# kwea123/nerf_pl

Hardware: AMD Instinct MI355X
Metric: rays/sec (64+128 samples), full training step: render_rays fwd + MSE + bwd + grad all-reduce + Adam (higher is better)
Workload: dtype bf16

## Files before the change

include/nerfhip.h:

```cpp
#ifndef NERFHIP_H
#define NERFHIP_H

#include <stddef.h>
#include <stdint.h>

#ifdef __cplusplus
extern "C" {
#endif

#define NERFHIP_ABI_VERSION 3

#define NERFHIP_E_BADARG (-1)
#define NERFHIP_E_UNSUPPORTED (-2)
#define NERFHIP_E_ALIGN (-3)
#define NERFHIP_E_DATA (-4)

#define NERFHIP_F32 0
#define NERFHIP_BF16 1
#define NERFHIP_BF16_F8 2

typedef void* nerfhip_stream_t;

int nerfhip_abi_version(void);
const char* nerfhip_error_string(int code);

int nerfhip_posenc(const float* x, float* out, int64_t n, int C, int n_freqs, nerfhip_stream_t stream);
int nerfhip_posenc_bwd(const float* x, const float* gout, float* gx, int64_t n, int C, int n_freqs,
                       nerfhip_stream_t stream);

int nerfhip_posenc_bands(const float* x, const float* bands, float* out, int64_t n, int C, int n_freqs,
                         nerfhip_stream_t stream);
int nerfhip_posenc_bands_bwd(const float* x, const float* bands, const float* gout, float* gx, int64_t n, int C, int n_freqs,
                             nerfhip_stream_t stream);

int nerfhip_sample_coarse_z(const float* rays, const float* perturb_rand, float* z, int64_t B, int S,
                            int use_disp, float perturb, nerfhip_stream_t stream);

int nerfhip_searchsorted_right(const float* a, const float* v, int64_t* idx, int64_t B, int M, int K,
                               nerfhip_stream_t stream);
int nerfhip_searchsorted_left(const float* a, const float* v, int64_t* idx, int64_t B, int M, int K,
                              nerfhip_stream_t stream);

int nerfhip_sample_pdf(const float* bins, int64_t bins_stride, const float* weights, int64_t w_stride,
                       const float* u, int64_t u_stride, float* samples, int64_t B, int M, int K, float eps,
                       nerfhip_stream_t stream);

#define NERFHIP_ROW_TOTAL_EXACT 0
#define NERFHIP_ROW_TOTAL_ATEN 1

int nerfhip_sample_pdf_ex(const float* bins, int64_t bins_stride, const float* weights, int64_t w_stride,
                          const float* u, int64_t u_stride, float* samples, int64_t B, int M, int K, float eps,
                          float* cdf_out, int64_t* inds_out, int row_total, nerfhip_stream_t stream);

int nerfhip_fine_z(const float* z_coarse, const float* w_coarse, const float* u, int64_t u_stride,
                   float* z_fine, float* z_new, int64_t B, int S_c, int N_i, float eps,
                   nerfhip_stream_t stream);

int nerfhip_fine_z_ex(const float* z_coarse, const float* w_coarse, const float* u, int64_t u_stride, float* z_fine,
                      float* z_new, int64_t B, int S_c, int N_i, float eps, float* cdf_out, int64_t* inds_out,
                      int row_total, nerfhip_stream_t stream);

int nerfhip_composite_fwd(const float* raw, int raw_ch, const float* z, const float* rays,
                          const float* noise, float noise_std, int white_back, float* weights, float* rgb,
                          float* depth, float* opacity, int64_t B, int S, nerfhip_stream_t stream);
int nerfhip_composite_bwd(const float* raw, int raw_ch, const float* z, const float* rays,
                          const float* noise, float noise_std, int white_back, const float* g_rgb,
                          const float* g_depth, const float* g_opacity, const float* g_weights,
                          float* g_raw, int64_t B, int S, nerfhip_stream_t stream);

int nerfhip_composite_train(const float* raw, const float* z, const float* rays, const float* noise, float noise_std,
                            int white_back, const float* target, float grad_scale, float* weights, float* rgb, float* depth,
                            float* opacity, float* g_raw, int64_t B, int S, nerfhip_stream_t stream);

int nerfhip_composite_train_fine_z(const float* raw, const float* z, const float* rays, const float* noise, float noise_std,
                                   int white_back, const float* target, float grad_scale, float* weights, float* rgb, float* depth,
                                   float* opacity, float* g_raw, int64_t B, int S, const float* u, int64_t u_stride, int N_i,
                                   float eps, float* z_fine, int row_total, nerfhip_stream_t stream);
int nerfhip_composite_train_loss(const float* raw, const float* z, const float* rays, const float* noise, float noise_std,
                                 int white_back, const float* target, float grad_scale, float* weights, float* rgb, float* depth,
                                 float* opacity, float* g_raw, int64_t B, int S, const float* rgb_coarse, float* out3,
                                 uint32_t* ticket, nerfhip_stream_t stream);

size_t nerfhip_mlp_packed_bytes(int dtype);
int nerfhip_mlp_pack_weights(const float* const* weights_host, const float* const* biases_host, void* packed,
                             int dtype, nerfhip_stream_t stream);

size_t nerfhip_mlp_act_bytes(int64_t n_points, int dtype);

int nerfhip_mlp_fwd_embedded(const float* x, int64_t x_stride, int64_t n, const void* packed, float* out,
                             int sigma_only, int dtype, void* save_acts, nerfhip_stream_t stream);

int nerfhip_mlp_fwd_rays(const float* rays, const float* z, int64_t B, int S, const void* packed, float* out,
                         int sigma_only, int dtype, void* save_acts, nerfhip_stream_t stream);

int nerfhip_mlp_fwd_rays_coarse(const float* rays, const float* perturb_rand, float* z, int64_t B, int S, int use_disp,
                                float perturb, const void* packed, float* out, int sigma_only, int dtype, void* save_acts,
                                nerfhip_stream_t stream);

size_t nerfhip_mlp_packed_bwd_bytes(int dtype);
int nerfhip_mlp_pack_weights_bwd(const float* const* weights_host, const float* const* biases_host, void* packed_bwd, int dtype,
                                 nerfhip_stream_t stream);
int nerfhip_mlp_pack_weights_train(const float* const* weights_host, const float* const* biases_host, void* packed,
                                   void* packed_bwd, int dtype, nerfhip_stream_t stream);
int nerfhip_mlp_pack_weights_train_multi(const float* const* weights_host, const float* const* biases_host,
                                         void* const* packed_host, void* const* packed_bwd_host, int n_models, int dtype,
                                         nerfhip_stream_t stream);
size_t nerfhip_mlp_dy_bytes(int64_t n_points, int dtype);
int nerfhip_mlp_dw_splits(int64_t n_points, int dtype);
size_t nerfhip_mlp_dw_workspace_bytes(int64_t n_points, int dtype);
int nerfhip_mlp_bwd(const float* g_out, const float* out, int64_t n, const void* packed_bwd, const void* acts,
                    void* dys, void* dw_workspace, float* const* grad_w_host, float* const* grad_b_host,
                    int accumulate, int dtype, nerfhip_stream_t stream);

int nerfhip_mlp_bwd_phases(const float* g_out, const float* out, int64_t n, const void* packed_bwd, const void* acts,
                           void* dys, void* dw_workspace, float* const* grad_w_host, float* const* grad_b_host,
                           int accumulate, int dtype, int phases, nerfhip_stream_t stream);

typedef struct nerfhip_adam_fused {
    int n_models;
    float* param[2];
    float* exp_avg[2];
    float* exp_avg_sq[2];
    const float* grad_flat[2];
    float* state;
    float lr, beta1, beta2, eps, weight_decay;
} nerfhip_adam_fused;
size_t nerfhip_mlp_dw_workspace_bytes_multi(const int64_t* n_points_host, int n_models, int dtype);
int nerfhip_mlp_dw_plan(const int64_t* n_points_host, int n_models, int dtype, int* splits_out, int* stage_kib_out);
int nerfhip_mlp_bwd_multi(int n_models, const float* const* g_out_host, const float* const* out_host, const int64_t* n_host,
                          const void* const* packed_bwd_host, const void* const* acts_host, void* const* dys_host,
                          void* dw_workspace, float* const* grad_w_host, float* const* grad_b_host, int accumulate, int dtype,
                          int phases, const float* g_scale, const nerfhip_adam_fused* adam, nerfhip_stream_t stream);

typedef struct nerfhip_enc_source {
    const float* rays[2];
    const float* z[2];
    int S[2];
} nerfhip_enc_source;
int nerfhip_mlp_bwd_multi_rays(int n_models, const float* const* g_out_host, const float* const* out_host, const int64_t* n_host,
                               const void* const* packed_bwd_host, const void* const* acts_host, void* const* dys_host,
                               void* dw_workspace, float* const* grad_w_host, float* const* grad_b_host, int accumulate, int dtype,
                               int phases, const float* g_scale, const nerfhip_adam_fused* adam, const nerfhip_enc_source* enc,
                               nerfhip_stream_t stream);

int nerfhip_mlp_dx_embedded(const void* dys, int64_t n, const float* w_xyz1, const float* w_xyz5, const float* w_dir,
                            float* gx, int64_t gx_stride, int dtype, nerfhip_stream_t stream);

#define NERFHIP_ACT_NONE 0
#define NERFHIP_ACT_RELU 1
#define NERFHIP_ACT_SIGMOID 2
int nerfhip_linear_fwd(const float* x, int64_t ldx, const float* w, int64_t ldw, const float* bias, float* y, int64_t ldy,
                       int64_t n, int n_in, int n_out, int act, int accumulate, int dtype, nerfhip_stream_t stream);
int nerfhip_linear_bwd_input(const float* gy, int64_t ldgy, const float* y, int64_t ldy, int act, const float* w, int64_t ldw,
                             float* gx, int64_t ldgx, int64_t n, int n_in, int n_out, int accumulate, int dtype,
                             nerfhip_stream_t stream);
size_t nerfhip_linear_bwd_weight_workspace_bytes(int64_t n, int n_in, int n_out);
int nerfhip_linear_bwd_weight(const float* gy, int64_t ldgy, const float* y, int64_t ldy, int act, const float* x, int64_t ldx,
                              float* gw, int64_t ldgw, float* gb, void* workspace, int64_t n, int n_in, int n_out,
                              int accumulate, int dtype, nerfhip_stream_t stream);

int nerfhip_mse_psnr(const float* rgb_coarse, const float* rgb_fine, const float* target, int64_t n, float* out3,
                     float* g_coarse, float* g_fine, nerfhip_stream_t stream);

int nerfhip_adam_step(float* const* params_host, const float* const* grads_host, float* const* exp_avg_host,
                      float* const* exp_avg_sq_host, const int64_t* numel_host, int n_tensors, float* state, float lr,
                      float beta1, float beta2, float eps, float weight_decay, nerfhip_stream_t stream);

int nerfhip_radam_step(float* const* params_host, const float* const* grads_host, float* const* exp_avg_host,
                       float* const* exp_avg_sq_host, const int64_t* numel_host, int n_tensors, float* state, double lr,
                       double beta1, double beta2, double eps, double weight_decay, int degenerated_to_sgd,
                       nerfhip_stream_t stream);
int nerfhip_ranger_step(float* const* params_host, const float* const* grads_host, float* const* exp_avg_host,
                        float* const* exp_avg_sq_host, const int64_t* numel_host, int n_tensors, float* state,
                        float* const* slow_host, double alpha, int k, double n_sma_threshold, double lr, double beta1,
                        double beta2, double eps, double weight_decay, nerfhip_stream_t stream);

int nerfhip_ray_directions(float* dirs, int H, int W, double focal, nerfhip_stream_t stream);
int nerfhip_get_rays(const float* directions, const float* c2w, float* rays_o, float* rays_d, int64_t n,
                     nerfhip_stream_t stream);
int nerfhip_ndc_rays(int H, int W, double focal, float near, const float* rays_o, const float* rays_d, float* out_o,
                     float* out_d, int64_t n, nerfhip_stream_t stream);
int nerfhip_gen_rays(const float* c2w, const int64_t* pixel_ids, int64_t first_pixel, int64_t n, int H, int W,
                     double focal, float near, float far, int use_ndc, float ndc_near_plane, float* rays,
                     nerfhip_stream_t stream);
int nerfhip_sample_batch(const float* c2w, const int64_t* pixel_ids, const float* rgbs_all, int64_t n, int H, int W,
                         double focal, float near, float far, int use_ndc, float ndc_near_plane, float* rays, float* rgbs,
                         nerfhip_stream_t stream);

#define NERFHIP_DRAW_UNIFORM 0
#define NERFHIP_DRAW_NORMAL 1
#define NERFHIP_DRAW_RANDINT 2
typedef struct nerfhip_draw {
    int kind;
    int64_t numel;
    void* out;
    uint64_t range;
} nerfhip_draw;
typedef struct nerfhip_ray_batch {
    const float* c2w;
    const float* rgbs_all;
    float* rays;
    float* rgbs;
    int H, W;
    double focal;
    float near, far;
    int use_ndc;
    float ndc_near_plane;
} nerfhip_ray_batch;
uint64_t nerfhip_torch_draw_increment(int64_t numel, int max_blocks);
int nerfhip_torch_draws(const nerfhip_draw* draws_host, int n_draws, const nerfhip_ray_batch* batch_host, uint64_t seed,
                        uint64_t offset, uint64_t* state, int max_blocks, uint64_t* increment_host, nerfhip_stream_t stream);

int nerfhip_train_prologue(const nerfhip_draw* draws_host, int n_draws, const nerfhip_ray_batch* batch_host, uint64_t seed,
                           uint64_t offset, uint64_t* state, int max_blocks, uint64_t* increment_host,
                           const float* const* weights_host, const float* const* biases_host, void* const* packed_host,
                           void* const* packed_bwd_host, int n_models, int dtype, nerfhip_stream_t stream);

typedef struct nerfhip_render_args {
    const float* rays;
    int64_t B;
    int S_c, N_i;
    const void* packed_coarse;
    const void* packed_fine;
    float* z_coarse;
    float* raw_coarse;
    float* z_fine;
    float* raw_fine;
    void* save_coarse;
    void* save_fine;
    const float* perturb_rand;
    float perturb;
    int use_disp;
    const float* noise_coarse;
    const float* noise_fine;
    float noise_std;
    int white_back;
    const float* u;
    int64_t u_stride;
    float eps;
    int row_total;
    float* rgb_coarse;
    float* depth_coarse;
    float* opacity_coarse;
    float* rgb_fine;
    float* depth_fine;
    float* opacity_fine;
    const float* target;
    float grad_scale;
    float* g_raw_coarse;
    float* g_raw_fine;
    float* out3;
    uint32_t* ticket;
    int regen_enc;
} nerfhip_render_args;
int nerfhip_render_supported(int64_t B, int S_c, int N_i, int dtype);
int nerfhip_render_fwd(const nerfhip_render_args* args_host, int dtype, nerfhip_stream_t stream);
int nerfhip_render_test_fwd(const nerfhip_render_args* args_host, int dtype, nerfhip_stream_t stream);
int nerfhip_render_train_fwd(const nerfhip_render_args* args_host, int dtype, nerfhip_stream_t stream);

size_t nerfhip_marching_cubes_workspace_bytes(int64_t n0, int64_t n1, int64_t n2);
int nerfhip_marching_cubes_count(const float* volume, int64_t n0, int64_t n1, int64_t n2, double iso, void* workspace,
                                 int64_t* totals, nerfhip_stream_t stream);
int nerfhip_marching_cubes_emit(const float* volume, int64_t n0, int64_t n1, int64_t n2, double iso, void* workspace,
                                const int64_t* totals, double* vertices, int32_t* triangles, nerfhip_stream_t stream);

int nerfhip_mesh_edge_keys(const int32_t* triangles, int64_t T, int64_t* keys, nerfhip_stream_t stream);
size_t nerfhip_mesh_cluster_workspace_bytes(int64_t V, int64_t T);
int nerfhip_mesh_largest_cluster(const int32_t* triangles, int64_t V, int64_t T, const int64_t* sorted_keys, const int64_t* order,
                                 void* workspace, int64_t* totals, nerfhip_stream_t stream);
int nerfhip_mesh_cluster_compact(const int32_t* triangles, int64_t V, int64_t T, void* workspace, int64_t* kept_vertex_ids,
                                 int32_t* kept_triangles, nerfhip_stream_t stream);

int nerfhip_mesh_vertex_normals(const float* vertices, int64_t V, const int32_t* triangles, int64_t T, double* normals,
                                nerfhip_stream_t stream);
int nerfhip_mesh_normal_rays(const float* vertices, const double* normals, int64_t V, float near, float far, float near_t,
                             float* rays, nerfhip_stream_t stream);
int nerfhip_mesh_view_rays(const float* vertices, int64_t V, const float* w2c_host, const float* origin_host, float focal, int W,
                           int H, const uint8_t* image, float near, uint8_t* colors, double* depth, float* rays,
                           nerfhip_stream_t stream);
int nerfhip_mesh_color_accumulate(const uint8_t* colors, const double* depth, const float* opacity, int64_t V,
                                  float occ_threshold, double* accum, nerfhip_stream_t stream);
int nerfhip_mesh_color_finish(const double* accum, int64_t V, uint8_t* out, nerfhip_stream_t stream);
int nerfhip_mesh_rgb_to_u8(const float* rgb, int64_t n, uint8_t* out, nerfhip_stream_t stream);

size_t nerfhip_vol_workspace_bytes(int64_t n);
int nerfhip_vol_pack(const float* rgbsigma, int64_t n, int64_t first_index, float neg_cell, void* workspace, uint32_t* records,
                     int64_t capacity, int64_t* cursor, nerfhip_stream_t stream);

int nerfhip_png_unfilter(const uint8_t* streams, uint8_t* out, int32_t* error_flags, int n_images, int H, int W, int ch,
                         nerfhip_stream_t stream);
int nerfhip_resize_rgba_lanczos(const uint8_t* in, uint8_t* out, uint8_t* workspace, int n_images, int in_h, int in_w, int out_h,
                                int out_w, const int32_t* xmin_h, const int32_t* count_h, const int32_t* taps_h, int ksize_h,
                                const int32_t* xmin_v, const int32_t* count_v, const int32_t* taps_v, int ksize_v,
                                nerfhip_stream_t stream);
int nerfhip_rgba_to_rgb_white(const uint8_t* rgba, float* rgb, uint8_t* valid_mask, int64_t n, nerfhip_stream_t stream);

int nerfhip_jpeg_entropy_decode(const uint8_t* scan, int64_t scan_bytes, int n_comp, const int32_t* comp, const uint8_t* huffman,
                                int huffman_mask, int mcus_x, int mcus_y, int restart_interval, int16_t* const* coef,
                                const int64_t* coef_blocks);
size_t nerfhip_jpeg_planes_bytes(int H, int W, int n_comp, int hs, int vs);
int nerfhip_jpeg_decode(const int16_t* coef_y, const int16_t* coef_cb, const int16_t* coef_cr, const uint16_t* quant,
                        uint8_t* planes, uint8_t* out, int n_images, int H, int W, int n_comp, int hs, int vs,
                        nerfhip_stream_t stream);

#define NERFHIP_IMAGE_PLANAR 0
#define NERFHIP_IMAGE_INTERLEAVED 1
size_t nerfhip_ssim_workspace_bytes(int B, int C, int H, int W);
int nerfhip_ssim(const float* img1, const float* img2, int B, int C, int H, int W, int window_size, int layout, float* map,
                 float* mean, void* workspace, nerfhip_stream_t stream);
size_t nerfhip_depth_colormap_workspace_bytes(int64_t n);
int nerfhip_depth_colormap(const float* depth, int64_t n, const uint8_t* table, float* out_chw, uint8_t* out_hwc, void* workspace,
                           nerfhip_stream_t stream);

#define NERFHIP_GIF_STRIP 3838
size_t nerfhip_gif_workspace_bytes(int F, int H, int W);
size_t nerfhip_gif_data_stride(int H, int W);
int nerfhip_gif_quantize(const uint8_t* frames, int F, int H, int W, uint8_t* indices, uint8_t* palettes, int32_t* box_counts,
                         void* workspace, nerfhip_stream_t stream);
int nerfhip_gif_lzw(const uint8_t* indices, int F, int H, int W, uint8_t* data, int32_t* lengths, void* workspace,
                    nerfhip_stream_t stream);

#ifdef __cplusplus
}
#endif
#endif
```

nerf_pl_amd/_lib.py:

```python
import ctypes
import functools
import os

import torch

_PKG = os.path.dirname(os.path.abspath(__file__))
LIB_PATH = os.environ.get("NERFHIP_LIB_PATH") or os.path.join(_PKG, "libnerfhip.so")

F32, BF16, BF16_F8 = 0, 1, 2

_c_void_p = ctypes.c_void_p
_i64 = ctypes.c_int64
_int = ctypes.c_int
_f32 = ctypes.c_float
_f64 = ctypes.c_double

SIGNATURES = {
    "nerfhip_abi_version": [],
    "nerfhip_error_string": [_int],
    "nerfhip_posenc": [_c_void_p, _c_void_p, _i64, _int, _int, _c_void_p],
    "nerfhip_posenc_bwd": [_c_void_p, _c_void_p, _c_void_p, _i64, _int, _int, _c_void_p],
    "nerfhip_posenc_bands": [_c_void_p, _c_void_p, _c_void_p, _i64, _int, _int, _c_void_p],
    "nerfhip_posenc_bands_bwd": [_c_void_p, _c_void_p, _c_void_p, _c_void_p, _i64, _int, _int, _c_void_p],
    "nerfhip_sample_coarse_z": [_c_void_p, _c_void_p, _c_void_p, _i64, _int, _int, _f32, _c_void_p],
    "nerfhip_searchsorted_right": [_c_void_p, _c_void_p, _c_void_p, _i64, _int, _int, _c_void_p],
    "nerfhip_searchsorted_left": [_c_void_p, _c_void_p, _c_void_p, _i64, _int, _int, _c_void_p],
    "nerfhip_sample_pdf": [_c_void_p, _i64, _c_void_p, _i64, _c_void_p, _i64, _c_void_p, _i64, _int, _int, _f32,
                           _c_void_p],
    "nerfhip_sample_pdf_ex": [_c_void_p, _i64, _c_void_p, _i64, _c_void_p, _i64, _c_void_p, _i64, _int, _int, _f32,
                              _c_void_p, _c_void_p, _int, _c_void_p],
    "nerfhip_fine_z_ex": [_c_void_p, _c_void_p, _c_void_p, _i64, _c_void_p, _c_void_p, _i64, _int, _int, _f32,
                          _c_void_p, _c_void_p, _int, _c_void_p],
    "nerfhip_fine_z": [_c_void_p, _c_void_p, _c_void_p, _i64, _c_void_p, _c_void_p, _i64, _int, _int, _f32,
                       _c_void_p],
    "nerfhip_composite_fwd": [_c_void_p, _int, _c_void_p, _c_void_p, _c_void_p, _f32, _int, _c_void_p, _c_void_p,
                              _c_void_p, _c_void_p, _i64, _int, _c_void_p],
    "nerfhip_composite_bwd": [_c_void_p, _int, _c_void_p, _c_void_p, _c_void_p, _f32, _int, _c_void_p, _c_void_p,
                              _c_void_p, _c_void_p, _c_void_p, _i64, _int, _c_void_p],
    "nerfhip_mlp_packed_bytes": [_int],
    "nerfhip_mlp_pack_weights": [ctypes.POINTER(_c_void_p), ctypes.POINTER(_c_void_p), _c_void_p, _int, _c_void_p],
    "nerfhip_mlp_act_bytes": [_i64, _int],
    "nerfhip_mlp_fwd_embedded": [_c_void_p, _i64, _i64, _c_void_p, _c_void_p, _int, _int, _c_void_p, _c_void_p],
    "nerfhip_mlp_fwd_rays": [_c_void_p, _c_void_p, _i64, _int, _c_void_p, _c_void_p, _int, _int, _c_void_p, _c_void_p],
    "nerfhip_mlp_packed_bwd_bytes": [_int],
    "nerfhip_mlp_pack_weights_bwd": [ctypes.POINTER(_c_void_p), ctypes.POINTER(_c_void_p), _c_void_p, _int, _c_void_p],
    "nerfhip_mlp_pack_weights_train": [ctypes.POINTER(_c_void_p), ctypes.POINTER(_c_void_p), _c_void_p, _c_void_p, _int, _c_void_p],
    "nerfhip_mlp_dy_bytes": [_i64, _int],
    "nerfhip_mlp_dw_splits": [_i64, _int],
    "nerfhip_mlp_dw_workspace_bytes": [_i64, _int],
    "nerfhip_ray_directions": [_c_void_p, _int, _int, ctypes.c_double, _c_void_p],
    "nerfhip_get_rays": [_c_void_p, _c_void_p, _c_void_p, _c_void_p, _i64, _c_void_p],
    "nerfhip_ndc_rays": [_int, _int, ctypes.c_double, _f32, _c_void_p, _c_void_p, _c_void_p, _c_void_p, _i64, _c_void_p],
    "nerfhip_gen_rays": [_c_void_p, _c_void_p, _i64, _i64, _int, _int, ctypes.c_double, _f32, _f32, _int, _f32, _c_void_p,
                         _c_void_p],
    "nerfhip_mse_psnr": [_c_void_p, _c_void_p, _c_void_p, _i64, _c_void_p, _c_void_p, _c_void_p, _c_void_p],
    "nerfhip_mlp_bwd_phases": [_c_void_p, _c_void_p, _i64, _c_void_p, _c_void_p, _c_void_p, _c_void_p,
                               ctypes.POINTER(_c_void_p), ctypes.POINTER(_c_void_p), _int, _int, _int, _c_void_p],
    "nerfhip_mlp_dx_embedded": [_c_void_p, _i64, _c_void_p, _c_void_p, _c_void_p, _c_void_p, _i64, _int, _c_void_p],
    "nerfhip_adam_step": [ctypes.POINTER(_c_void_p), ctypes.POINTER(_c_void_p), ctypes.POINTER(_c_void_p),
                          ctypes.POINTER(_c_void_p), ctypes.POINTER(_i64), _int, _c_void_p, _f32, _f32, _f32, _f32, _f32, _c_void_p],
    "nerfhip_radam_step": [ctypes.POINTER(_c_void_p), ctypes.POINTER(_c_void_p), ctypes.POINTER(_c_void_p),
                           ctypes.POINTER(_c_void_p), ctypes.POINTER(_i64), _int, _c_void_p, _f64, _f64, _f64, _f64, _f64, _int, _c_void_p],
    "nerfhip_ranger_step": [ctypes.POINTER(_c_void_p), ctypes.POINTER(_c_void_p), ctypes.POINTER(_c_void_p),
                            ctypes.POINTER(_c_void_p), ctypes.POINTER(_i64), _int, _c_void_p, ctypes.POINTER(_c_void_p), _f64, _int,
                            _f64, _f64, _f64, _f64, _f64, _f64, _c_void_p],
    "nerfhip_mlp_bwd": [_c_void_p, _c_void_p, _i64, _c_void_p, _c_void_p, _c_void_p, _c_void_p,
                        ctypes.POINTER(_c_void_p), ctypes.POINTER(_c_void_p), _int, _int, _c_void_p],
    "nerfhip_sample_batch": [_c_void_p, _c_void_p, _c_void_p, _i64, _int, _int, ctypes.c_double, _f32, _f32, _int, _f32, _c_void_p,
                             _c_void_p, _c_void_p],
    "nerfhip_mlp_pack_weights_train_multi": [ctypes.POINTER(_c_void_p), ctypes.POINTER(_c_void_p), ctypes.POINTER(_c_void_p),
                                             ctypes.POINTER(_c_void_p), _int, _int, _c_void_p],
    "nerfhip_render_supported": [_i64, _int, _int, _int],
    "nerfhip_render_test_fwd": [_c_void_p, _int, _c_void_p],
    "nerfhip_render_fwd": [_c_void_p, _int, _c_void_p],
    "nerfhip_render_train_fwd": [_c_void_p, _int, _c_void_p],
    "nerfhip_composite_train": [_c_void_p, _c_void_p, _c_void_p, _c_void_p, _f32, _int, _c_void_p, _f32, _c_void_p, _c_void_p,
                                _c_void_p, _c_void_p, _c_void_p, _i64, _int, _c_void_p],
    "nerfhip_composite_train_fine_z": [_c_void_p, _c_void_p, _c_void_p, _c_void_p, _f32, _int, _c_void_p, _f32, _c_void_p, _c_void_p,
                                       _c_void_p, _c_void_p, _c_void_p, _i64, _int, _c_void_p, _i64, _int, _f32, _c_void_p, _int, _c_void_p],
    "nerfhip_composite_train_loss": [_c_void_p, _c_void_p, _c_void_p, _c_void_p, _f32, _int, _c_void_p, _f32, _c_void_p, _c_void_p,
                                     _c_void_p, _c_void_p, _c_void_p, _i64, _int, _c_void_p, _c_void_p, _c_void_p, _c_void_p],
    "nerfhip_mlp_fwd_rays_coarse": [_c_void_p, _c_void_p, _c_void_p, _i64, _int, _int, _f32, _c_void_p, _c_void_p, _int, _int,
                                    _c_void_p, _c_void_p],
    "nerfhip_torch_draw_increment": [_i64, _int],
    "nerfhip_torch_draws": [_c_void_p, _int, _c_void_p, ctypes.c_uint64, ctypes.c_uint64, _c_void_p, _int,
                            ctypes.POINTER(ctypes.c_uint64), _c_void_p],
    "nerfhip_train_prologue": [_c_void_p, _int, _c_void_p, ctypes.c_uint64, ctypes.c_uint64, _c_void_p, _int,
                               ctypes.POINTER(ctypes.c_uint64), ctypes.POINTER(_c_void_p), ctypes.POINTER(_c_void_p),
                               ctypes.POINTER(_c_void_p), ctypes.POINTER(_c_void_p), _int, _int, _c_void_p],
    "nerfhip_mlp_dw_workspace_bytes_multi": [ctypes.POINTER(_i64), _int, _int],
    "nerfhip_mlp_dw_plan": [ctypes.POINTER(_i64), _int, _int, ctypes.POINTER(_int), ctypes.POINTER(_int)],
    "nerfhip_mlp_bwd_multi": [_int, ctypes.POINTER(_c_void_p), ctypes.POINTER(_c_void_p), ctypes.POINTER(_i64),
                              ctypes.POINTER(_c_void_p), ctypes.POINTER(_c_void_p), ctypes.POINTER(_c_void_p), _c_void_p,
                              ctypes.POINTER(_c_void_p), ctypes.POINTER(_c_void_p), _int, _int, _int, _c_void_p, _c_void_p, _c_void_p],
    "nerfhip_mlp_bwd_multi_rays": [_int, ctypes.POINTER(_c_void_p), ctypes.POINTER(_c_void_p), ctypes.POINTER(_i64),
                                   ctypes.POINTER(_c_void_p), ctypes.POINTER(_c_void_p), ctypes.POINTER(_c_void_p), _c_void_p,
                                   ctypes.POINTER(_c_void_p), ctypes.POINTER(_c_void_p), _int, _int, _int, _c_void_p, _c_void_p, _c_void_p,
                                   _c_void_p],
    "nerfhip_linear_fwd": [_c_void_p, _i64, _c_void_p, _i64, _c_void_p, _c_void_p, _i64, _i64, _int, _int, _int, _int, _int, _c_void_p],
    "nerfhip_linear_bwd_input": [_c_void_p, _i64, _c_void_p, _i64, _int, _c_void_p, _i64, _c_void_p, _i64, _i64, _int, _int, _int,
                                 _int, _c_void_p],
    "nerfhip_linear_bwd_weight_workspace_bytes": [_i64, _int, _int],
    "nerfhip_linear_bwd_weight": [_c_void_p, _i64, _c_void_p, _i64, _int, _c_void_p, _i64, _c_void_p, _i64, _c_void_p, _c_void_p,
                                  _i64, _int, _int, _int, _int, _c_void_p],
    "nerfhip_marching_cubes_workspace_bytes": [_i64, _i64, _i64],
    "nerfhip_marching_cubes_count": [_c_void_p, _i64, _i64, _i64, ctypes.c_double, _c_void_p, _c_void_p, _c_void_p],
    "nerfhip_marching_cubes_emit": [_c_void_p, _i64, _i64, _i64, ctypes.c_double, _c_void_p, _c_void_p, _c_void_p, _c_void_p,
                                    _c_void_p],
    "nerfhip_mesh_edge_keys": [_c_void_p, _i64, _c_void_p, _c_void_p],
    "nerfhip_mesh_cluster_workspace_bytes": [_i64, _i64],
    "nerfhip_mesh_largest_cluster": [_c_void_p, _i64, _i64, _c_void_p, _c_void_p, _c_void_p, _c_void_p, _c_void_p],
    "nerfhip_mesh_cluster_compact": [_c_void_p, _i64, _i64, _c_void_p, _c_void_p, _c_void_p, _c_void_p],
    "nerfhip_mesh_vertex_normals": [_c_void_p, _i64, _c_void_p, _i64, _c_void_p, _c_void_p],
    "nerfhip_mesh_normal_rays": [_c_void_p, _c_void_p, _i64, _f32, _f32, _f32, _c_void_p, _c_void_p],
    "nerfhip_mesh_view_rays": [_c_void_p, _i64, ctypes.POINTER(_f32), ctypes.POINTER(_f32), _f32, _int, _int, _c_void_p, _f32,
                               _c_void_p, _c_void_p, _c_void_p, _c_void_p],
    "nerfhip_mesh_color_accumulate": [_c_void_p, _c_void_p, _c_void_p, _i64, _f32, _c_void_p, _c_void_p],
    "nerfhip_mesh_color_finish": [_c_void_p, _i64, _c_void_p, _c_void_p],
    "nerfhip_mesh_rgb_to_u8": [_c_void_p, _i64, _c_void_p, _c_void_p],
    "nerfhip_vol_workspace_bytes": [_i64],
    "nerfhip_vol_pack": [_c_void_p, _i64, _i64, _f32, _c_void_p, _c_void_p, _i64, _c_void_p, _c_void_p],
    "nerfhip_png_unfilter": [_c_void_p, _c_void_p, _c_void_p, _int, _int, _int, _int, _c_void_p],
    "nerfhip_resize_rgba_lanczos": [_c_void_p, _c_void_p, _c_void_p, _int, _int, _int, _int, _int, _c_void_p, _c_void_p, _c_void_p,
                                    _int, _c_void_p, _c_void_p, _c_void_p, _int, _c_void_p],
    "nerfhip_rgba_to_rgb_white": [_c_void_p, _c_void_p, _c_void_p, _i64, _c_void_p],
    "nerfhip_jpeg_entropy_decode": [_c_void_p, _i64, _int, _c_void_p, _c_void_p, _int, _int, _int, _int, ctypes.POINTER(_c_void_p),
                                    ctypes.POINTER(_i64)],
    "nerfhip_jpeg_planes_bytes": [_int, _int, _int, _int, _int],
    "nerfhip_jpeg_decode": [_c_void_p, _c_void_p, _c_void_p, _c_void_p, _c_void_p, _c_void_p, _int, _int, _int, _int, _int, _int,
                            _c_void_p],
    "nerfhip_ssim_workspace_bytes": [_int, _int, _int, _int],
    "nerfhip_ssim": [_c_void_p, _c_void_p, _int, _int, _int, _int, _int, _int, _c_void_p, _c_void_p, _c_void_p, _c_void_p],
    "nerfhip_depth_colormap_workspace_bytes": [_i64],
    "nerfhip_depth_colormap": [_c_void_p, _i64, _c_void_p, _c_void_p, _c_void_p, _c_void_p, _c_void_p],
    "nerfhip_gif_workspace_bytes": [_int, _int, _int],
    "nerfhip_gif_data_stride": [_int, _int],
    "nerfhip_gif_quantize": [_c_void_p, _int, _int, _int, _c_void_p, _c_void_p, _c_void_p, _c_void_p, _c_void_p],
    "nerfhip_gif_lzw": [_c_void_p, _int, _int, _int, _c_void_p, _c_void_p, _c_void_p, _c_void_p],
}


class AdamFused(ctypes.Structure):
    _fields_ = [("n_models", _int), ("param", _c_void_p * 2), ("exp_avg", _c_void_p * 2), ("exp_avg_sq", _c_void_p * 2),
                ("grad_flat", _c_void_p * 2), ("state", _c_void_p), ("lr", _f32), ("beta1", _f32), ("beta2", _f32), ("eps", _f32),
                ("weight_decay", _f32)]

class Draw(ctypes.Structure):
    _fields_ = [("kind", _int), ("numel", _i64), ("out", _c_void_p), ("range", ctypes.c_uint64)]


class RayBatch(ctypes.Structure):
    _fields_ = [("c2w", _c_void_p), ("rgbs_all", _c_void_p), ("rays", _c_void_p), ("rgbs", _c_void_p), ("H", _int), ("W", _int),
                ("focal", ctypes.c_double), ("near", _f32), ("far", _f32), ("use_ndc", _int), ("ndc_near_plane", _f32)]


class RenderArgs(ctypes.Structure):
    _fields_ = [("rays", _c_void_p), ("B", _i64), ("S_c", _int), ("N_i", _int), ("packed_coarse", _c_void_p), ("packed_fine", _c_void_p),
                ("z_coarse", _c_void_p), ("raw_coarse", _c_void_p), ("z_fine", _c_void_p), ("raw_fine", _c_void_p),
                ("save_coarse", _c_void_p), ("save_fine", _c_void_p), ("perturb_rand", _c_void_p), ("perturb", _f32), ("use_disp", _int),
                ("noise_coarse", _c_void_p), ("noise_fine", _c_void_p), ("noise_std", _f32), ("white_back", _int), ("u", _c_void_p),
                ("u_stride", _i64), ("eps", _f32), ("row_total", _int), ("rgb_coarse", _c_void_p), ("depth_coarse", _c_void_p),
                ("opacity_coarse", _c_void_p), ("rgb_fine", _c_void_p), ("depth_fine", _c_void_p), ("opacity_fine", _c_void_p),
                ("target", _c_void_p), ("grad_scale", _f32), ("g_raw_coarse", _c_void_p), ("g_raw_fine", _c_void_p), ("out3", _c_void_p),
                ("ticket", _c_void_p), ("regen_enc", _int)]


class EncSource(ctypes.Structure):
    _fields_ = [("rays", _c_void_p * 2), ("z", _c_void_p * 2), ("S", _int * 2)]


DRAW_UNIFORM, DRAW_NORMAL, DRAW_RANDINT = 0, 1, 2

_RESTYPES = {"nerfhip_error_string": ctypes.c_char_p, "nerfhip_torch_draw_increment": ctypes.c_uint64, "nerfhip_mlp_packed_bytes": ctypes.c_size_t,
             "nerfhip_mlp_act_bytes": ctypes.c_size_t, "nerfhip_mlp_packed_bwd_bytes": ctypes.c_size_t,
             "nerfhip_mlp_dy_bytes": ctypes.c_size_t, "nerfhip_mlp_dw_workspace_bytes": ctypes.c_size_t,
             "nerfhip_mlp_dw_workspace_bytes_multi": ctypes.c_size_t,
             "nerfhip_linear_bwd_weight_workspace_bytes": ctypes.c_size_t,
             "nerfhip_marching_cubes_workspace_bytes": ctypes.c_size_t, "nerfhip_mesh_cluster_workspace_bytes": ctypes.c_size_t,
             "nerfhip_jpeg_planes_bytes": ctypes.c_size_t, "nerfhip_ssim_workspace_bytes": ctypes.c_size_t,
             "nerfhip_depth_colormap_workspace_bytes": ctypes.c_size_t, "nerfhip_gif_workspace_bytes": ctypes.c_size_t,
             "nerfhip_gif_data_stride": ctypes.c_size_t, "nerfhip_vol_workspace_bytes": ctypes.c_size_t}

_lib = None


class NerfHipError(RuntimeError):
    pass


def load():
    global _lib
    if _lib is not None:
        return _lib
    if not os.path.exists(LIB_PATH):
        raise NerfHipError(
            "libnerfhip.so not built: run `python -m nerf_pl_amd.build` (needs hipcc, gfx950). "
            "There is no CPU/eager fallback for the hot path.")
    lib = ctypes.CDLL(LIB_PATH, mode=ctypes.RTLD_GLOBAL)
    for name, argtypes in SIGNATURES.items():
        fn = getattr(lib, name)
        fn.argtypes = argtypes
        fn.restype = _RESTYPES.get(name, ctypes.c_int)
    if lib.nerfhip_abi_version() != 3:
        raise NerfHipError("libnerfhip ABI version mismatch")
    _lib = lib
    return lib


def check(code, what):
    if code != 0:
        msg = load().nerfhip_error_string(code)
        raise NerfHipError("%s failed: %s (code %d)" % (what, msg.decode() if msg else "?", code))


def stream_ptr():
    return ctypes.c_void_p(torch.cuda.current_stream().cuda_stream)


def _first_cuda_tensor(args):
    for a in args:
        if torch.is_tensor(a) and a.is_cuda:
            return a
        if isinstance(a, (list, tuple)):
            t = _first_cuda_tensor(a)
            if t is not None:
                return t
    return None


def device_guard(fn):
    @functools.wraps(fn)
    def wrapped(*args, **kw):
        t = _first_cuda_tensor(args)
        if t is None:
            t = _first_cuda_tensor(tuple(kw.values()))
        if t is None or t.device.index == torch.cuda.current_device():
            return fn(*args, **kw)
        with torch.cuda.device(t.device):
            return fn(*args, **kw)
    return wrapped


def ptr(t):
    if t is None:
        return None
    return ctypes.c_void_p(t.data_ptr())


def require_gpu(*tensors):
    dev = None
    for t in tensors:
        if t is None:
            continue
        if not t.is_cuda:
            raise NerfHipError("nerf_pl_amd runs on MI355X only: got a %s tensor (no CPU fallback)" % t.device)
        if t.dtype != torch.float32:
            raise NerfHipError("expected float32 tensor, got %s" % t.dtype)
        if dev is None:
            dev = t.device
        elif t.device != dev:
            raise NerfHipError("tensors of one call live on different GPUs (%s vs %s)" % (dev, t.device))
    if dev is not None and dev.index != torch.cuda.current_device():
        raise NerfHipError("launch on %s while the current device is cuda:%d (operator missing its device_guard)"
                           % (dev, torch.cuda.current_device()))
```

nerf_pl_amd/csrc/mlp_bwd.hip:

```cpp
#include "common.h"
#include "mlp_layout.h"
#include "mlp_bwd_chain.h"
#include "mlp_bwd_dw.h"
#include "mlp_dw_plan.h"

static_assert(kPlanF32 == NERFHIP_F32 && kPlanBf16 == NERFHIP_BF16 && kPlanBf16F8 == NERFHIP_BF16_F8, "mlp_dw_plan.h dtype codes");
static inline bool valid_dtype(int dtype) { return dtype == NERFHIP_F32 || dtype == NERFHIP_BF16 || dtype == NERFHIP_BF16_F8; }
static inline int compute_prec(int dtype) { return dtype == NERFHIP_F32 ? NERFHIP_F32 : NERFHIP_BF16; }
#if NERFHIP_DW_PROBE
static bool g_probe_f8 = false;
#endif

extern "C" size_t nerfhip_mlp_dy_bytes(int64_t n_points, int dtype) {
    if (n_points < 0 || !valid_dtype(dtype)) return 0;
    if (dtype == NERFHIP_BF16_F8) return (size_t)act_tiles(n_points, dtype) * nerfhip::mlp::f8_dy_tile_bytes();
    return (size_t)act_tiles(n_points, dtype) * nerfhip::mlp::kDySlabs * 64 * (dtype == NERFHIP_BF16 ? 16 : 32);
}

extern "C" int nerfhip_mlp_dw_splits(int64_t n_points, int dtype) {
    if (n_points <= 0 || !valid_dtype(dtype)) return 0;
    return dw_plan(&n_points, 1, dtype, nullptr);
}
static size_t dw_workspace_bytes(int nwg, int n_models) {
    return ((size_t)nwg * nerfhip::mlp::kDwSlabFloats + (size_t)n_models * nerfhip::mlp::kFoldScratchFloats) * sizeof(float);
}
extern "C" size_t nerfhip_mlp_dw_workspace_bytes(int64_t n_points, int dtype) {
    const int nwg = nerfhip_mlp_dw_splits(n_points, dtype);
    return nwg > 0 ? dw_workspace_bytes(nwg, 1) : 0;
}
extern "C" size_t nerfhip_mlp_dw_workspace_bytes_multi(const int64_t* n_points_host, int n_models, int dtype) {
    if (!n_points_host || n_models < 1 || n_models > nerfhip::kDwMaxModels || !valid_dtype(dtype)) return 0;
    for (int m = 0; m < n_models; ++m)
        if (n_points_host[m] <= 0) return 0;
    return dw_workspace_bytes(dw_plan(n_points_host, n_models, dtype, nullptr), n_models);
}

extern "C" int nerfhip_mlp_dw_plan(const int64_t* n_points_host, int n_models, int dtype, int* splits_out, int* stage_kib_out) {
    if (!n_points_host || !splits_out || n_models < 1 || n_models > nerfhip::kDwMaxModels || !valid_dtype(dtype)) return NERFHIP_E_BADARG;
    for (int m = 0; m < n_models; ++m)
        if (n_points_host[m] <= 0) return NERFHIP_E_BADARG;
    nerfhip::DwJobTable jt;
    const int total = dw_plan(n_points_host, n_models, dtype, &jt);
    for (int j = 0; j < n_models * nerfhip::mlp::kNumDwJobs; ++j) {
        splits_out[j] = jt.nsplit[j];
        if (stage_kib_out) {
            int slabs = jt.job[j].dy_slabs + jt.job[j].x1_slabs + jt.job[j].x2_slabs;
            if (jt.fold_of[j] >= 0 || jt.nsplit[j] == 0) slabs = 0;
            for (int k = 0; k < n_models * nerfhip::mlp::kNumDwJobs; ++k)
                if (jt.fold_of[k] == j) slabs += jt.job[k].dy_slabs;
            stage_kib_out[j] = dtype == NERFHIP_F32 ? 2 * slabs : slabs;
        }
    }
    return total;
}

extern "C" int nerfhip_mlp_bwd_multi(int n_models, const float* const* g_out_host, const float* const* out_host,
                                     const int64_t* n_host, const void* const* packed_bwd_host, const void* const* acts_host,
                                     void* const* dys_host, void* dw_workspace, float* const* grad_w_host,
                                     float* const* grad_b_host, int accumulate, int dtype, int phases, const float* g_scale,
                                     const nerfhip_adam_fused* adam, nerfhip_stream_t stream) {
    return nerfhip_mlp_bwd_multi_rays(n_models, g_out_host, out_host, n_host, packed_bwd_host, acts_host, dys_host, dw_workspace, grad_w_host,
                                      grad_b_host, accumulate, dtype, phases, g_scale, adam, nullptr, stream);
}

extern "C" int nerfhip_mlp_bwd_multi_rays(int n_models, const float* const* g_out_host, const float* const* out_host,
                                          const int64_t* n_host, const void* const* packed_bwd_host, const void* const* acts_host,
                                          void* const* dys_host, void* dw_workspace, float* const* grad_w_host,
                                          float* const* grad_b_host, int accumulate, int dtype, int phases, const float* g_scale,
                                          const nerfhip_adam_fused* adam, const nerfhip_enc_source* enc, nerfhip_stream_t stream) {
    NERFHIP_CHECK_ARG(n_models >= 1 && n_models <= nerfhip::kDwMaxModels);
    if (!valid_dtype(dtype)) return NERFHIP_E_UNSUPPORTED;
    bool regen[nerfhip::kDwMaxModels] = {false, false};
    if (enc) {
        if (dtype != NERFHIP_BF16) return NERFHIP_E_UNSUPPORTED;
        for (int m = 0; m < n_models; ++m) {
            if (!enc->rays[m]) continue;
            NERFHIP_CHECK_ARG(enc->z[m] && enc->S[m] > 0 && enc->S[m] % 32 == 0 && n_host[m] % 256 == 0 && n_host[m] % enc->S[m] == 0);
            NERFHIP_CHECK_ARG(n_host[m] / 32 < (int64_t)1 << 31);
            if ((((uintptr_t)enc->rays[m]) | ((uintptr_t)enc->z[m])) & 15) return NERFHIP_E_ALIGN;
            regen[m] = true;
        }
    }
    NERFHIP_CHECK_ARG(g_out_host && out_host && n_host && packed_bwd_host && acts_host && dys_host && grad_w_host && grad_b_host);
    NERFHIP_CHECK_ARG(!(adam && accumulate));
    nerfhip::GradTable G;
    nerfhip::DwJobTable jt;
    for (int m = 0; m < n_models; ++m) {
        NERFHIP_CHECK_ARG(n_host[m] > 0);
        NERFHIP_CHECK_ARG(g_out_host[m] && out_host[m] && packed_bwd_host[m] && acts_host[m] && dys_host[m] && dw_workspace);
        if ((((uintptr_t)g_out_host[m]) | ((uintptr_t)out_host[m]) | ((uintptr_t)packed_bwd_host[m]) | ((uintptr_t)acts_host[m]) |
             ((uintptr_t)dys_host[m])) & 15)
            return NERFHIP_E_ALIGN;
    }
    const int nwg = dw_plan(n_host, n_models, dtype, &jt);
    for (int m = 0; m < nerfhip::kDwMaxModels; ++m) {
        const bool on = m < n_models && regen[m];
        jt.enc_rays[m] = on ? enc->rays[m] : nullptr;
        jt.enc_z[m] = on ? enc->z[m] : nullptr;
        jt.enc_tpr[m] = on ? enc->S[m] / 32 : 1;
    }
    float* const fold_scratch = (float*)dw_workspace + (size_t)nwg * nerfhip::mlp::kDwSlabFloats;
    nerfhip::FoldArgs F;
    for (int m = 0; m < nerfhip::kDwMaxModels; ++m) {
        const int mm = m < n_models ? m : 0;
        F.image[m] = reinterpret_cast<const float*>((const uint8_t*)packed_bwd_host[mm] +
                                                    (size_t)nerfhip::mlp::bwd_padded_pieces(compute_prec(dtype)) * nerfhip::mlp::kPieceBytes);
        F.gw_final[m] = grad_w_host[12 * mm + 8];
        F.gb_final[m] = grad_b_host[12 * mm + 8];
        F.gw_dir[m] = grad_w_host[12 * mm + 9];
    }
    for (int j = 0; j < nerfhip::kDwMaxJobs; ++j) {
        const int jj = j < jt.njobs ? j : 0, m = jj / nerfhip::mlp::kNumDwJobs, prm = nerfhip::mlp::kDwJobs[jj % nerfhip::mlp::kNumDwJobs].param;
        NERFHIP_CHECK_ARG(grad_w_host[12 * m + prm] && grad_b_host[12 * m + prm]);
        G.w[j] = grad_w_host[12 * m + prm];
        G.b[j] = grad_b_host[12 * m + prm];
        jt.acts[j] = (const uint8_t*)acts_host[m];
        jt.dys[j] = (const uint8_t*)dys_host[m];
    }
    nerfhip::AdamFused A;
    A.state = nullptr;
    A.lr = A.beta1 = A.beta2 = A.eps = A.wd = 0.f;
    for (int m = 0; m < nerfhip::kDwMaxModels; ++m) { A.param[m] = A.m[m] = A.v[m] = nullptr; A.grad0[m] = nullptr; }
    if (adam) {
        NERFHIP_CHECK_ARG(adam->state && adam->n_models == n_models);
        for (int m = 0; m < n_models; ++m) {
            NERFHIP_CHECK_ARG(adam->param[m] && adam->exp_avg[m] && adam->exp_avg_sq[m] && adam->grad_flat[m]);
            A.param[m] = adam->param[m]; A.m[m] = adam->exp_avg[m]; A.v[m] = adam->exp_avg_sq[m]; A.grad0[m] = adam->grad_flat[m];
        }
        A.state = adam->state; A.lr = adam->lr; A.beta1 = adam->beta1; A.beta2 = adam->beta2; A.eps = adam->eps; A.wd = adam->weight_decay;
    }
    hipStream_t s = (hipStream_t)stream;
    const bool do_chain = phases & 1, do_dw = phases & 2, do_reduce = phases & 4;
    if (do_chain) {
        int64_t tiles[nerfhip::kDwMaxModels];
        for (int m = 0; m < n_models; ++m) tiles[m] = act_tiles(n_host[m], dtype);
        nerfhip::launch_bwd_chain(n_models, g_out_host, g_scale, out_host, n_host, packed_bwd_host, acts_host, dys_host, dtype, tiles, s);
    }
    if (do_dw) {
        if (dtype == NERFHIP_BF16_F8) nerfhip::launch_dw_f8(jt, (float*)dw_workspace, nwg, s);
        else nerfhip::launch_dw(dtype, jt, (float*)dw_workspace, nwg, s);
#if NERFHIP_DW_PROBE
        g_probe_f8 = dtype == NERFHIP_BF16_F8;
#endif
    }
    if (do_reduce) {
        nerfhip::launch_reduce(dtype == NERFHIP_BF16_F8, jt, (const float*)dw_workspace, G, fold_scratch, accumulate, A, s);
        nerfhip::launch_fold(F, (const float*)fold_scratch, n_models, accumulate, A, s);
    }
    return nerfhip_launch_status();
}

#if NERFHIP_DW_PROBE
extern "C" int nerfhip_debug_dw_probe(unsigned* host_dst, int n_words) {
    if (!host_dst || n_words < 0 || n_words > 1024 * 8 * 8) return NERFHIP_E_BADARG;
    return g_probe_f8 ? nerfhip::read_dw_f8_probe(host_dst, n_words) : nerfhip::read_dw_probe(host_dst, n_words);
}
#endif

extern "C" int nerfhip_mlp_bwd_phases(const float* g_out, const float* out, int64_t n, const void* packed_bwd, const void* acts,
                                      void* dys, void* dw_workspace, float* const* grad_w_host, float* const* grad_b_host,
                                      int accumulate, int dtype, int phases, nerfhip_stream_t stream) {
    NERFHIP_CHECK_ARG(n >= 0);
    if (!valid_dtype(dtype)) return NERFHIP_E_UNSUPPORTED;
    NERFHIP_CHECK_ARG(grad_w_host && grad_b_host);
    for (int i = 0; i < 12; ++i) NERFHIP_CHECK_ARG(grad_w_host[i] && grad_b_host[i]);
    if (n == 0) return 0;
    return nerfhip_mlp_bwd_multi(1, &g_out, &out, &n, &packed_bwd, &acts, &dys, dw_workspace, grad_w_host, grad_b_host, accumulate,
                                 dtype, phases, nullptr, nullptr, stream);
}

extern "C" int nerfhip_mlp_bwd(const float* g_out, const float* out, int64_t n, const void* packed_bwd, const void* acts,
                               void* dys, void* dw_workspace, float* const* grad_w_host, float* const* grad_b_host,
                               int accumulate, int dtype, nerfhip_stream_t stream) {
    return nerfhip_mlp_bwd_phases(g_out, out, n, packed_bwd, acts, dys, dw_workspace, grad_w_host, grad_b_host, accumulate, dtype, 7,
                                  stream);
}
```

nerf_pl_amd/csrc/mlp_bwd_chain.h:

```cpp
#pragma once
#include <hip/hip_runtime.h>
#include <stdint.h>

namespace nerfhip {
struct BwdChainArgs {
    const float* g_out[2];
    const float* out[2];
    int64_t n[2];
    const uint8_t* packed_bwd[2];
    const uint8_t* acts[2];
    uint8_t* dys[2];
    int blocks0;
};
void launch_bwd_chain(int n_models, const float* const* g_out, const float* g_scale, const float* const* out, const int64_t* n,
                      const void* const* packed_bwd, const void* const* acts, void* const* dys, int dtype, const int64_t* tiles,
                      hipStream_t s);
}
```

nerf_pl_amd/csrc/mlp_bwd_chain.hip:

```cpp
#include "mlp_device.h"
#include "f8_store.h"
#include "mlp_bwd_chain.h"

namespace nerfhip {

__device__ __forceinline__ float slab_absmax8(const bf16x8& s) {
    float m = 0.0f;
#pragma unroll
    for (int j = 0; j < 8; ++j) m = fmaxf(m, fabsf((float)s[j]));
    return m;
}
__device__ __forceinline__ float slab_absmax8(const f32x8& s) { return 0.0f; }

constexpr int kChainDepthBf16 = 2, kChainDepthF8 = 0;
constexpr int kChainBurst = 2;
template <int PREC> using BwdStream = RingStream<PrecTraits<PREC>::NW, bwd_chunks(PREC), true>;

template <typename Slab>
__device__ __forceinline__ Slab load_slab(__amdgpu_buffer_rsrc_t rsrc, int sec, int lane) {
    Slab s;
    u32x4* dst = reinterpret_cast<u32x4*>(&s);
    const unsigned voff = (unsigned)lane * (unsigned)sizeof(Slab);
    const unsigned soff = (unsigned)(sec * 64 * sizeof(Slab));
#pragma unroll
    for (int q = 0; q < (int)(sizeof(Slab) / 16); ++q) dst[q] = __builtin_amdgcn_raw_buffer_load_b128(rsrc, voff + 16 * q, soff, 0);
    return s;
}
template <int PREC, typename Slab>
__device__ __forceinline__ void store_slab(int& pending, __amdgpu_buffer_rsrc_t rsrc, int sec, const Slab& s, int lane) {
    const unsigned voff = (unsigned)lane * (unsigned)sizeof(Slab);
    const unsigned soff = (unsigned)(sec * 64 * sizeof(Slab) * act_il(PREC));
    store_slab_b128(pending, rsrc, s, voff + soff);
}

__device__ __forceinline__ void save_dy_pair(int& pending, uint8_t* dy_tile, int pair, const bf16x8& s0, const bf16x8& s1, int sb, int lane) {
    save_pair_bf8(pending, dy_tile, pair, s0, s1, sb, lane);
}
__device__ __forceinline__ void save_dy_pair(int&, uint8_t*, int, const f32x8&, const f32x8&, int, int) {}
__device__ __forceinline__ int dy_block_scale(float lane_max) { return bf8_block_scale(lane_max); }

template <int BIT>
__device__ __forceinline__ unsigned gate_mask(unsigned word) {
    unsigned m;
    asm("v_bfe_i32 %0, %1, %2, 1" : "=v"(m) : "v"(word), "n"(BIT));
    return m;
}

template <int PREC, int L, int NT, int NKS, bool MASK, bool F8, int IN_PAIRS, typename Slab>
__device__ __forceinline__ int run_bwd_layer_tm(BwdStream<PREC>& st, const unsigned lds_lo, const unsigned lds_hi, const unsigned sig_lds,
                                                const Slab (&gin)[NKS - kBwdLayers[L].sigma_slab], Slab* out,
                                                __amdgpu_buffer_rsrc_t acts, int gate_off, int mask_piece,
                                                __amdgpu_buffer_rsrc_t dys, uint8_t* dy_tile, int dy_sec, int dy_scale_idx, int in_sec,
                                                int in_sb, int lane) {
    constexpr int G0 = bwd_layer_start(L, PREC);
    constexpr int PPF = ppf(PREC);
    static_assert(kBwdLayers[L].nt == NT && kBwdLayers[L].nks == NKS, "bwd layer shape mismatch");
    auto piece_off = [](int g) { return ((g / kChunkPieces) % kSlots) * kChunkBytes + (g % kChunkPieces) * kPieceBytes; };
    typedef __attribute__((address_space(3))) const char* lds_cptr;
    auto piece_ptr = [&](int g) { return piece_off(g) < 65536 ? (lds_cptr)(lds_lo + (unsigned)piece_off(g)) : (lds_cptr)(lds_hi + (unsigned)(piece_off(g) - 65536)); };
    constexpr bool SIG = kBwdLayers[L].sigma_slab != 0;
    constexpr int NIN = NKS - (SIG ? 1 : 0);
    auto bslab = [&](int ks) -> Slab {
        if constexpr (SIG) {
            if (ks == NIN) return *reinterpret_cast<__attribute__((address_space(3))) const Slab*>(sig_lds);
        }
        return gin[ks < NIN ? ks : 0];
    };
    u32x4 gates = {0u, 0u, 0u, 0u};
    if (MASK)
        gates = __builtin_amdgcn_raw_buffer_load_b128(acts, (unsigned)lane * 16u, (unsigned)((gate_off + mask_piece * kPieceBytes) * act_il(PREC, F8)), 0);
    float mx = 0.0f;
    f32x16 acc2[2];
    constexpr int NFR = NT * NKS;
    constexpr int kChainDepth = F8 ? kChainDepthF8 : kChainDepthBf16;
    [[maybe_unused]] bf16x8 afr[kChainDepth > 0 ? kChainDepth : 1];
    [[maybe_unused]] auto frag_read = [&](auto ic) -> bf16x8 {
        constexpr int g = G0 + decltype(ic)::value * PPF;
        if constexpr (g % kChunkPieces == 0) st.boundary(g / kChunkPieces);
        return *reinterpret_cast<__attribute__((address_space(3))) const bf16x8*>(piece_ptr(g));
    };
    if constexpr (PREC == NERFHIP_BF16 && kChainDepth > 0) {
        static_for<0, (kChainDepth < NFR ? kChainDepth : NFR)>([&](auto jc) { afr[decltype(jc)::value] = frag_read(jc); });
    }
    static_for<0, NT>([&](auto tc) {
        constexpr int t = decltype(tc)::value;
        f32x16& acc = acc2[t & 1];
#pragma unroll
        for (int r = 0; r < 16; ++r) acc[r] = 0.0f;
        if constexpr (PREC == NERFHIP_BF16 && kChainDepth > 0) {
            static_for<0, NKS>([&](auto kc) {
                constexpr int ks = decltype(kc)::value;
                constexpr int i = t * NKS + ks;
                acc = __builtin_amdgcn_mfma_f32_32x32x16_bf16(afr[i % (kChainDepth > 0 ? kChainDepth : 1)], bslab(ks), acc, 0, 0, 0);
                if constexpr (i + kChainDepth < NFR) afr[i % (kChainDepth > 0 ? kChainDepth : 1)] = frag_read(std::integral_constant<int, i + kChainDepth>{});
                __builtin_amdgcn_sched_barrier(0);
            });
        } else {
#pragma unroll
        for (int ks = 0; ks < NKS; ++ks) {
            const int g = G0 + (t * NKS + ks) * PPF;
            if (g % kChunkPieces == 0) st.boundary(g / kChunkPieces);
            if constexpr (PREC == NERFHIP_BF16) {
                const bf16x8 a = *reinterpret_cast<__attribute__((address_space(3))) const bf16x8*>(piece_ptr(g));
                acc = __builtin_amdgcn_mfma_f32_32x32x16_bf16(a, bslab(ks), acc, 0, 0, 0);
            } else {
                const f32x4 a0 = *reinterpret_cast<__attribute__((address_space(3))) const f32x4*>(piece_ptr(g));
                if ((g + 1) % kChunkPieces == 0) st.boundary((g + 1) / kChunkPieces);
                const f32x4 a1 = *reinterpret_cast<__attribute__((address_space(3))) const f32x4*>(piece_ptr(g + 1));
                const Slab bs = bslab(ks);
#pragma unroll
                for (int j = 0; j < 4; ++j) acc = __builtin_amdgcn_mfma_f32_32x32x2f32(a0[j], bs[j], acc, 0, 0, 0);
#pragma unroll
                for (int j = 0; j < 4; ++j) acc = __builtin_amdgcn_mfma_f32_32x32x2f32(a1[j], bs[4 + j], acc, 0, 0, 0);
            }
        }
        }
        if constexpr (F8 && PREC == NERFHIP_BF16) {
            if constexpr (IN_PAIRS > 0) {
#pragma unroll
                for (int q = 0; q < IN_PAIRS; ++q)
                    if (q >= t * IN_PAIRS / NT && q < (t + 1) * IN_PAIRS / NT)
                        save_dy_pair(st.pending, dy_tile, in_sec / 2 + q, gin[2 * q], gin[2 * q + 1], in_sb, lane);
            }
        }
        if constexpr (PREC == NERFHIP_BF16 && MASK) {
            static_for<0, 8>([&](auto pc) {
                constexpr int p = decltype(pc)::value;
                constexpr int idx = 8 * (2 * t) + 2 * p;
                typedef __attribute__((ext_vector_type(2))) float f32x2v;
                typedef __attribute__((ext_vector_type(2))) __bf16 bf16x2q;
                typedef __attribute__((ext_vector_type(2))) short s16x2q;
                const f32x2v xv = {acc[2 * p], acc[2 * p + 1]};
                if (F8) mx = fmaxf(fmaxf(mx, fabsf(xv[0])), fabsf(xv[1]));
                const bf16x2q pk = __builtin_convertvector(xv, bf16x2q);
                const unsigned gword = gates[gate_word(idx)];
                s16x2q gm = __builtin_bit_cast(s16x2q, gword);
                gm = (gm << (short)((idx & 31) >> 1)) >> (short)15;
                const unsigned d = __builtin_bit_cast(unsigned, pk) & __builtin_bit_cast(unsigned, gm);
                const bf16x2q gated = __builtin_bit_cast(bf16x2q, d);
                out[2 * t + (p >> 2)][2 * (p & 3)] = gated[0];
                out[2 * t + (p >> 2)][2 * (p & 3) + 1] = gated[1];
            });
        } else {
        float v[16];
        static_for<0, 16>([&](auto rc) {
            constexpr int r = decltype(rc)::value;
            constexpr int idx = 8 * (2 * t) + r;
            const float gv = acc[r];
            if constexpr (MASK) v[r] = __uint_as_float(__float_as_uint(gv) & gate_mask<gate_bit(idx)>(gates[gate_word(idx)]));
            else v[r] = gv;
            if (F8) mx = fmaxf(mx, fabsf(v[r]));
        });
#pragma unroll
        for (int sl = 0; sl < 2; ++sl) {
            float v8[8];
#pragma unroll
            for (int j = 0; j < 8; ++j) v8[j] = v[8 * sl + j];
            make_slab(out[2 * t + sl], v8);
        }
        }
        if constexpr (!F8) {
            __amdgpu_buffer_rsrc_t dys_l = __builtin_amdgcn_make_buffer_rsrc(dy_tile + (size_t)dy_sec * 64 * sizeof(Slab) * act_il(PREC), 0,
                                                                              (int)(2 * NT * 64 * sizeof(Slab) * act_il(PREC)), 0x00020000);
            constexpr int TB = kChainBurst / 2 > 0 ? kChainBurst / 2 : 1;
            if constexpr ((t + 1) % TB == 0 || t == NT - 1) {
                constexpr int t0 = (t / TB) * TB;
#pragma unroll
                for (int sl = 2 * t0; sl < 2 * t + 2; ++sl) store_slab<PREC>(st.pending, dys_l, sl, out[sl], lane);
            }
        }
    });
    if constexpr (F8 && PREC == NERFHIP_BF16) {
        const int sb = dy_block_scale(mx);
        save_scale_f8(st.pending, dy_tile, f8_dy_scale_off(), dy_scale_idx, sb, lane);
        return sb;
    }
    return 127;
}

template <int PREC, bool F8>
__global__ __launch_bounds__(PrecTraits<PREC>::NW * 64, PrecTraits<PREC>::WPS)
void mlp_bwd_chain_kernel(BwdChainArgs A, const float* __restrict__ g_scale) {
    const int mdl = ((int)blockIdx.x >= A.blocks0) ? 1 : 0;
    const unsigned wg = blockIdx.x - (mdl ? (unsigned)A.blocks0 : 0u);
    const float* __restrict__ g_out = mdl ? A.g_out[1] : A.g_out[0];
    const float* __restrict__ out = mdl ? A.out[1] : A.out[0];
    const int64_t n = mdl ? A.n[1] : A.n[0];
    const uint8_t* __restrict__ packed_bwd = mdl ? A.packed_bwd[1] : A.packed_bwd[0];
    const uint8_t* __restrict__ acts_base = mdl ? A.acts[1] : A.acts[0];
    uint8_t* __restrict__ dys_base = mdl ? A.dys[1] : A.dys[0];
    static_assert(!F8 || PREC == NERFHIP_BF16, "fp8 storage is a bf16-compute mode");
    using Slab = typename PrecTraits<PREC>::Slab;
    constexpr int kActTile = F8 ? f8_act_tile_bytes() : act_tile_bytes(PREC);
    constexpr int kGateOff = F8 ? f8_act_gate_off() : act_mask_off(PREC);
    constexpr int kDyTile = F8 ? f8_dy_tile_bytes() : kDySlabs * 64 * (int)sizeof(Slab);
    constexpr int NW = PrecTraits<PREC>::NW;
    __shared__ __attribute__((aligned(1024))) char ring[kSlots * kChunkBytes + NW * 64 * (int)sizeof(Slab)];
#if NERFHIP_STREAM_PROBE
    const uint64_t probe_t0 = __builtin_amdgcn_s_memrealtime();
#endif
    const int lane = threadIdx.x & 63;
    const int wave = __builtin_amdgcn_readfirstlane((int)(threadIdx.x >> 6));
    const int h = lane >> 5;
    const int64_t tile = (int64_t)wg * NW + wave;
    const int64_t p = tile * 32 + (lane & 31);
    const bool valid = p < n;
    const int64_t pc = valid ? p : n - 1;

    float4 g = reinterpret_cast<const float4*>(g_out)[pc];
    const float4 o = reinterpret_cast<const float4*>(out)[pc];
    if (!valid) g = make_float4(0.f, 0.f, 0.f, 0.f);
    if (g_scale) {
        const float sc = *g_scale;
        g.x *= sc; g.y *= sc; g.z *= sc; g.w *= sc;
    }

    constexpr int IL = act_il(PREC, F8);
    __amdgpu_buffer_rsrc_t acts = __builtin_amdgcn_make_buffer_rsrc(
        const_cast<uint8_t*>(acts_base) + tile_block_off(tile, kActTile, IL), 0, kActTile * IL, 0x00020000);
    uint8_t* dy_tile = dys_base + tile_block_off(tile, kDyTile, IL);
    __amdgpu_buffer_rsrc_t dys = __builtin_amdgcn_make_buffer_rsrc(dy_tile, 0, kDyTile * IL, 0x00020000);


    BwdStream<PREC> st;
    st.gsrc = packed_bwd;
    st.voff = (unsigned)lane * 16u;
    st.lds_base = (unsigned)(uintptr_t)ring;
    st.wave = wave;
    st.pending = 0;
    st.pending_prev = 0;
    st.issue_chunk(0);
    st.issue_chunk(1);
    const unsigned lds_lo = (unsigned)(uintptr_t)ring + (unsigned)lane * 16u;
    unsigned lds_hi = lds_lo + 65536u;
    asm volatile("" : "+v"(lds_hi));
    const unsigned sig_lds = (unsigned)(uintptr_t)ring + (unsigned)(kSlots * kChunkBytes) + (unsigned)((wave * 64 + lane) * (int)sizeof(Slab));

    float v[8];
    Slab zero_slab;
#pragma unroll
    for (int j = 0; j < 8; ++j) v[j] = 0.0f;
    make_slab(zero_slab, v);
    Slab g_rgb, g_sig;
    {
        const float ga[3] = {g.x * o.x * (1.0f - o.x), g.y * o.y * (1.0f - o.y), g.z * o.z * (1.0f - o.z)};
#pragma unroll
        for (int j = 0; j < 8; ++j) v[j] = (h == 0 && j < 3) ? ga[j < 3 ? j : 0] : 0.0f;
        make_slab(g_rgb, v);
#pragma unroll
        for (int j = 0; j < 8; ++j) v[j] = (h == 0 && j == 0) ? g.w : 0.0f;
        make_slab(g_sig, v);
    }
    if constexpr (F8) {
        if constexpr (PREC == NERFHIP_BF16) {
            const int sb_rgb = bf8_block_scale(slab_absmax8(g_rgb)), sb_sig = bf8_block_scale(slab_absmax8(g_sig));
            save_pair_bf8(st.pending, dy_tile, kDyRgb / 2, g_rgb, zero_slab, sb_rgb, lane);
            save_pair_bf8(st.pending, dy_tile, kDySigma / 2, g_sig, zero_slab, sb_sig, lane);
            save_scale_f8(st.pending, dy_tile, f8_dy_scale_off(), f8_dy_section(kDyRgb), sb_rgb, lane);
            save_scale_f8(st.pending, dy_tile, f8_dy_scale_off(), f8_dy_section(kDySigma), sb_sig, lane);
        }
    } else {
        store_slab<PREC>(st.pending, dys, kDyRgb, g_rgb, lane);
        store_slab<PREC>(st.pending, dys, kDyRgb + 1, zero_slab, lane);
        store_slab<PREC>(st.pending, dys, kDySigma, g_sig, lane);
        store_slab<PREC>(st.pending, dys, kDySigma + 1, zero_slab, lane);
    }

    Slab gd[8];
    Slab ga[16], gb[16];
    Slab g_in0[1] = {g_rgb};
    int sb = run_bwd_layer_tm<PREC, 0, 4, 1, true, F8, 0>(st, lds_lo, lds_hi, sig_lds, g_in0, gd, acts, kGateOff, kMaskPieceT, dys, dy_tile, kDyDir,
                                                          f8_dy_section(kDyDir), -1, 127, lane);
    *reinterpret_cast<__attribute__((address_space(3))) Slab*>(sig_lds) = g_sig;
    static_assert(kBwdLayerFold == 1, "layer sequence below");
    sb = run_bwd_layer_tm<PREC, 1, 8, 9, true, F8, 4>(st, lds_lo, lds_hi, sig_lds, gd, gb, acts, kGateOff, mask_piece_h(8), dys, dy_tile, dy_h(8),
                                                      f8_dy_section(dy_h(8)), kDyDir, sb, lane);
    static_assert(bwd_layer_pieces(2, PREC) * 3 % (kChunkPieces * kSlots) == 0, "three looped layers = a whole number of ring turns");
#define NH_BWD(L, IN, OUT, D)                                                                                                \
    sb = run_bwd_layer_tm<PREC, L, 8, 16, true, F8, 8>(st, lds_lo, lds_hi, sig_lds, reinterpret_cast<const Slab(&)[16]>(IN), OUT, acts, kGateOff, \
                                                       mask_piece_h(9 - L) - (D), dys, dy_tile, dy_h(9 - L) + 16 * (D),              \
                                                       f8_dy_section(dy_h(9 - L)) + (D), dy_h(10 - L) + 16 * (D), sb, lane);
    if constexpr (PREC != NERFHIP_BF16) {
        NH_BWD(2, gb, ga, 0) NH_BWD(3, ga, gb, 0) NH_BWD(4, gb, ga, 0) NH_BWD(5, ga, gb, 0) NH_BWD(6, gb, ga, 0) NH_BWD(7, ga, gb, 0)
    } else {
        const uint8_t* const gsrc0 = st.gsrc;
        int n_pass;
        asm volatile("s_mov_b32 %0, 2" : "=s"(n_pass));
#pragma clang loop unroll(disable)
        for (int pass = 0; pass < n_pass; ++pass) {
            st.pending = 0;
            st.pending_prev = 0;
            const int d = 3 * pass;
            NH_BWD(2, gb, ga, d) NH_BWD(3, ga, gb, d) NH_BWD(4, gb, ga, d)
#pragma unroll
            for (int i = 0; i < 16; ++i) gb[i] = ga[i];
            st.gsrc += (size_t)(3 * bwd_layer_pieces(2, PREC)) * kPieceBytes;
        }
        st.pending = 0;
        st.pending_prev = 0;
        st.gsrc = gsrc0;
    }
    NH_BWD(8, gb, ga, 0)
#undef NH_BWD
    if constexpr (F8 && PREC == NERFHIP_BF16) {
#pragma unroll
        for (int q = 0; q < 8; ++q) save_dy_pair(st.pending, dy_tile, dy_h(1) / 2 + q, ga[2 * q], ga[2 * q + 1], sb, lane);
    }
#if NERFHIP_STREAM_PROBE
    if (lane == 0) {
        unsigned* pr = reinterpret_cast<unsigned*>(dy_tile);
        pr[0] = st.pr_wait; pr[1] = st.pr_bar; pr[2] = st.pr_n;
        pr[3] = (unsigned)(__builtin_amdgcn_s_memrealtime() - probe_t0);
    }
#endif
}


}

namespace nerfhip {
void launch_bwd_chain(int n_models, const float* const* g_out, const float* g_scale, const float* const* out, const int64_t* n,
                      const void* const* packed_bwd, const void* const* acts, void* const* dys, int dtype, const int64_t* tiles,
                      hipStream_t s) {
    const int wpw = (dtype == NERFHIP_F32) ? 4 : 8;
    BwdChainArgs A;
    unsigned blocks = 0;
    for (int m = 0; m < 2; ++m) {
        const int mm = m < n_models ? m : 0;
        A.g_out[m] = g_out[mm]; A.out[m] = out[mm]; A.n[m] = n[mm];
        A.packed_bwd[m] = (const uint8_t*)packed_bwd[mm]; A.acts[m] = (const uint8_t*)acts[mm]; A.dys[m] = (uint8_t*)dys[mm];
        if (m == 0) A.blocks0 = (int)(tiles[0] / wpw);
        if (m < n_models) blocks += (unsigned)(tiles[m] / wpw);
    }
    if (dtype == NERFHIP_BF16_F8)
        hipLaunchKernelGGL((mlp_bwd_chain_kernel<NERFHIP_BF16, true>), dim3(blocks), dim3(512), 0, s, A, g_scale);
    else if (dtype == NERFHIP_BF16)
        hipLaunchKernelGGL((mlp_bwd_chain_kernel<NERFHIP_BF16, false>), dim3(blocks), dim3(512), 0, s, A, g_scale);
    else
        hipLaunchKernelGGL((mlp_bwd_chain_kernel<NERFHIP_F32, false>), dim3(blocks), dim3(256), 0, s, A, g_scale);
}
}
```

nerf_pl_amd/csrc/mlp_bwd_dw.h:

```cpp
#pragma once
#include <stdint.h>

#include "mlp_layout.h"

typedef struct ihipStream_t* hipStream_t;

#ifndef NERFHIP_DW_PROBE
#define NERFHIP_DW_PROBE 0
#endif

namespace nerfhip {
using namespace mlp;

constexpr int kDwMaxModels = 2;
constexpr int kDwMaxJobs = kDwMaxModels * kNumDwJobs;
struct DwJobTable {
    DwJob job[kDwMaxJobs];
    int nsplit[kDwMaxJobs];
    int soff[kDwMaxJobs + 1];
    const uint8_t* acts[kDwMaxJobs];
    const uint8_t* dys[kDwMaxJobs];
    int64_t ntiles[kDwMaxJobs];
    int njobs;
    int fold_of[kDwMaxJobs];
    const float* enc_rays[kDwMaxModels];
    const float* enc_z[kDwMaxModels];
    int enc_tpr[kDwMaxModels];
};
static_assert(kDwJobs[kDwJobDir].x2_off == kDwJobs[kDwJobSigma].x1_off && kDwJobs[kDwJobDir].x2_slabs == 16 && kDwJobs[kDwJobDir].x1_slabs == 2 &&
              kDwJobs[kDwJobSigma].x1_slabs == 16 && kDwJobs[kDwJobSigma].dy_slabs == 2 && kDwJobs[kDwJobDir].dy_slabs == 8 &&
              kDwJobs[kDwJobSigma].x2_slabs == 0, "the sigma head and the dir layer read the same h8 section");
constexpr int kDwFoldRow0 = 4;
NH_HD constexpr int dw_fold_block(int xt) { return (kDwFoldRow0 + xt / 2) * kDwMaxXTiles + (xt & 1); }
constexpr int kDwFoldStageSlabs = 28;
constexpr int kDwFoldSigmaSlab = 26;

struct GradTable {
    float* w[kDwMaxJobs];
    float* b[kDwMaxJobs];
};

struct AdamFused {
    float* param[kDwMaxModels];
    float* m[kDwMaxModels];
    float* v[kDwMaxModels];
    const float* grad0[kDwMaxModels];
    float* state;
    float lr, beta1, beta2, eps, wd;
};

struct FoldArgs {
    const float* image[kDwMaxModels];
    float* gw_final[kDwMaxModels];
    float* gb_final[kDwMaxModels];
    float* gw_dir[kDwMaxModels];
};

void launch_dw(int prec, const DwJobTable& jt, float* slabs, int nwg, hipStream_t s);
void launch_dw_f8(const DwJobTable& jt, float* slabs, int nwg, hipStream_t s);
void launch_reduce(bool f8, const DwJobTable& jt, const float* slabs, const GradTable& G, float* fold_scratch, int accumulate,
                   const AdamFused& A, hipStream_t s);
void launch_fold(const FoldArgs& F, const float* fold_scratch, int n_models, int accumulate, const AdamFused& A, hipStream_t s);
#if NERFHIP_DW_PROBE
int read_dw_probe(unsigned* host_dst, int n_words);
int read_dw_f8_probe(unsigned* host_dst, int n_words);
#endif
}
```

nerf_pl_amd/csrc/mlp_bwd_dw.hip:

```cpp
#include "mlp_device.h"
#include "mlp_bwd_dw.h"

namespace nerfhip {

#if NERFHIP_DW_PROBE
__device__ unsigned g_dw_probe[1024 * 8 * 8];
#endif

constexpr int kDwRingKiB = 160, kDwMaxDepth = 12;
constexpr int kDwFragRing = 5, kDwFragRing2D = 4;

template <int PREC> struct DwTraits;
template <> struct DwTraits<NERFHIP_BF16> {
    static constexpr int SPP = 1;
    static constexpr int RING_BYTES = kDwRingKiB * 1024;
    static constexpr int DEPTH = 0, STAGE_BYTES = 0;
};
template <> struct DwTraits<NERFHIP_F32> {
    static constexpr int SPP = 2;
    static constexpr int DEPTH = 2;
    static constexpr int MAXP = 72;
    static constexpr int STAGE_BYTES = MAXP * kPieceBytes;
    static constexpr int RING_BYTES = DEPTH * STAGE_BYTES;
};

template <int PREC> NH_HD constexpr int dw_depth(int pieces) {
    if (PREC != NERFHIP_BF16) return DwTraits<PREC>::DEPTH;
    const int d = DwTraits<PREC>::RING_BYTES / (pieces * kPieceBytes);
    return d > kDwMaxDepth ? kDwMaxDepth : d;
}

__device__ __forceinline__ void dw_bias_sum(const bf16x8& a, float& s0, float& s1) {
    const bf16x2 one = {(__bf16)1.0f, (__bf16)1.0f};
    s0 = __builtin_amdgcn_fdot2_f32_bf16(bf16x2{a[0], a[1]}, one, s0, false);
    s1 = __builtin_amdgcn_fdot2_f32_bf16(bf16x2{a[2], a[3]}, one, s1, false);
    s0 = __builtin_amdgcn_fdot2_f32_bf16(bf16x2{a[4], a[5]}, one, s0, false);
    s1 = __builtin_amdgcn_fdot2_f32_bf16(bf16x2{a[6], a[7]}, one, s1, false);
}

template <int F, int SLABS>
__device__ __forceinline__ bf16x8 dw_encode_slab(const float (&v)[3], int h, int ks) {
    constexpr int NPAIR = 3 * (F / 2);
    constexpr float kInv2PiHi = 0.15915494f, kInv2PiLo = 6.4206297e-9f;
    float rh[3], rl[3];
#pragma unroll
    for (int c = 0; c < 3; ++c) {
        const float vs = h ? 2.0f * v[c] : v[c];
        rh[c] = vs * kInv2PiHi;
        rl[c] = __builtin_fmaf(vs, kInv2PiHi, -rh[c]) + vs * kInv2PiLo;
    }
    bf16x8 out;
#pragma unroll
    for (int q = 0; q < 4; ++q) {
        const int p = 4 * ks + q;
        float s, co;
        if (p < NPAIR) {
            const int i = p / 3, c = p - 3 * i;
            const float sc = (float)(1 << (2 * i));
            const float rhc = c == 0 ? rh[0] : (c == 1 ? rh[1] : rh[2]), rlc = c == 0 ? rl[0] : (c == 1 ? rl[1] : rl[2]);
            const float t = __builtin_amdgcn_fractf(rhc * sc) + rlc * sc;
            s = __builtin_amdgcn_sinf(t);
            co = __builtin_amdgcn_cosf(t);
        } else {
            const int tail = 2 * (p - NPAIR);
            s = (tail == 0) ? (h ? v[2] : v[0]) : 0.0f;
            co = (tail == 0) ? (h ? 0.0f : v[1]) : 0.0f;
        }
        out[2 * q] = (__bf16)s;
        out[2 * q + 1] = (__bf16)co;
    }
    return out;
}

template <int PREC>
__global__ __launch_bounds__(512, 2)
void mlp_bwd_dw_kernel(DwJobTable jobs, float* __restrict__ slabs) {
    constexpr int SPP = DwTraits<PREC>::SPP;
    constexpr int SLAB_BYTES = SPP * kPieceBytes;
    constexpr int IL = act_il(PREC);
    constexpr int RING_BYTES = DwTraits<PREC>::RING_BYTES;
    __shared__ __attribute__((aligned(1024))) char ring[RING_BYTES];

    const int lane = threadIdx.x & 63;
    const int wave = __builtin_amdgcn_readfirstlane((int)(threadIdx.x >> 6));
    int jid = 0;
#pragma unroll
    for (int j = 1; j < kDwMaxJobs; ++j) jid += ((int)blockIdx.x >= jobs.soff[j]) ? 1 : 0;
    const int nsplit = jobs.nsplit[jid], split = (int)blockIdx.x - jobs.soff[jid];
    const DwJob jb = jobs.job[jid];
    const int64_t ntiles = jobs.ntiles[jid];
    const uint8_t* __restrict__ acts_base = jobs.acts[jid];
    const uint8_t* __restrict__ dys_base = jobs.dys[jid];
    [[maybe_unused]] const float* __restrict__ enc_rays = jobs.enc_rays[jid / kNumDwJobs];
    [[maybe_unused]] const float* __restrict__ enc_z = jobs.enc_z[jid / kNumDwJobs];
    [[maybe_unused]] const int enc_tpr = jobs.enc_tpr[jid / kNumDwJobs];
    const int n_ot = jb.dy_slabs / 2;
    const int n_xs = jb.x1_slabs + jb.x2_slabs;
    const int n_xt = n_xs / 2;
    const int64_t per = (ntiles + nsplit - 1) / nsplit;
    const int64_t t_first = (int64_t)split * per;
    const int64_t my_tiles = (t_first >= ntiles) ? 0 : ((ntiles - t_first < per) ? ntiles - t_first : per);
    const unsigned lds_base = (unsigned)(uintptr_t)ring;

    const int dma_off_even = (PREC == NERFHIP_BF16) ? ((lane & 1) * 32 + (lane >> 1)) * 16 : lane * 16;
    const int dma_off_odd = (PREC == NERFHIP_BF16) ? ((lane & 1) * 32 + ((lane ^ 8) >> 1)) * 16 : lane * 16;

    f32x16 acc[kDwMaxXTiles];
#pragma unroll
    for (int x = 0; x < kDwMaxXTiles; ++x)
#pragma unroll
        for (int r = 0; r < 16; ++r) acc[x][r] = 0.0f;
    float dbacc = 0.0f;
    [[maybe_unused]] float dbacc2 = 0.0f;

    const int grp = lane >> 4, c = lane & 15;
    const int tr_off = (grp & 1) * SLAB_BYTES + (2 * (8 * (grp >> 1) + (c >> 2)) + ((c & 3) & 1)) * 16 + ((c & 3) >> 1) * 8;
    const int tr_s0 = (grp & 1) ? 128 : 0, tr_s1 = 128 - tr_s0;
    [[maybe_unused]] auto load_frag = [&](const char* pb, int q) { return load_frag_tr16(pb, tr_off, tr_s0, tr_s1, q); };
    const int m32 = lane & 31, kk = lane >> 5;
    const int f32_off = (m32 >> 4) * SLAB_BYTES + (slab_nat_h(m32 & 15) * 32) * 32 + slab_nat_j(m32 & 15) * 4;
#if NERFHIP_DW_PROBE
    unsigned pr_wait = 0, pr_bar = 0, pr_issue = 0, pr_comp = 0, pr_depth = 0;
    const uint64_t pr_t00 = __builtin_amdgcn_s_memrealtime();
#endif

    auto run = [&](auto nxt_c, auto nsl_c, auto regen_c) {
        constexpr int NXT = decltype(nxt_c)::value, NSL = decltype(nsl_c)::value;
        constexpr bool REGEN = decltype(regen_c)::value;
        static_assert(!REGEN || (PREC == NERFHIP_BF16 && (NXT == 2 || NXT == 9 || NXT == 10)), "classes with an encoding section");
        constexpr int ENC = REGEN ? (NXT == 9 ? kDirSlabs : kXyzSlabs) : 0;
        constexpr int DYS = NXT == 9 ? 8 : 16;
        constexpr bool FOLD = NXT == 9 && NSL == kDwFoldStageSlabs;
        constexpr bool SPLIT2D = (PREC == NERFHIP_BF16) && (NXT == 8 || NXT == 10) && (NSL - 2 * NXT >= 16);
        constexpr int NP = NSL * SPP;
        constexpr int NPD = NP - ENC;
        constexpr int LPWD = (NPD + 7) / 8;
        constexpr int LPW = LPWD + (REGEN ? 1 : 0);
        constexpr int STAGE = (PREC == NERFHIP_BF16) ? NP * kPieceBytes : DwTraits<PREC>::STAGE_BYTES;
        constexpr int ZSLOT = 256;
        constexpr int D0 = dw_depth<PREC>(NP);
        constexpr int D = (REGEN && D0 * (STAGE + ZSLOT) > RING_BYTES) ? D0 - 1 : D0;
        static_assert(D >= 2 && D * (STAGE + (REGEN ? ZSLOT : 0)) <= RING_BYTES, "ring stages of this job class");
        static_assert((D - 2) * LPW <= 63, "counted vmcnt");
#if NERFHIP_DW_PROBE
        pr_depth = D;
#endif
        int s_issue = 0, s_use = 0;
        const uint8_t* abase = nullptr;
        const uint8_t* dbase = nullptr;
        unsigned slot = 0;
        auto stage_tile = [&](int64_t it) {
            int64_t T = t_first + (it < my_tiles ? it : my_tiles - 1);
            if (T >= ntiles) T = ntiles - 1;
            return T;
        };
        const float* zsrc = nullptr;
        unsigned zslot = 0;
        int z_issue = 0, g_slot = 0;
        const unsigned lds_z = lds_base + (unsigned)(D * STAGE);
        auto next_z = [&](int64_t st) {
            zsrc = enc_z + stage_tile(st) * 32 + (lane & 31);
            zslot = (unsigned)__builtin_amdgcn_readfirstlane((int)(lds_z + (unsigned)(z_issue * ZSLOT)));
            z_issue = (z_issue + 1 == D) ? 0 : z_issue + 1;
        };
        auto next_stage = [&](int64_t it) {
            const int64_t T = stage_tile(it);
            abase = acts_base + tile_block_off(T, act_tile_bytes(PREC), IL);
            dbase = dys_base + tile_block_off(T, kDySlabs * 64 * (16 * SPP), IL);
            slot = lds_base + (unsigned)(s_issue * STAGE);
            s_issue = (s_issue + 1 == D) ? 0 : s_issue + 1;
            if constexpr (REGEN) next_z(it + 1);
        };
        float ray_next[6] = {0.f, 0.f, 0.f, 0.f, 0.f, 0.f};
        auto load_ray = [&](int64_t st) {
            if (wave < ENC) {
                const unsigned r = (unsigned)__builtin_amdgcn_readfirstlane((int)((unsigned)stage_tile(st) / (unsigned)enc_tpr));
                typedef const float __attribute__((address_space(4))) * ConstF;
                const ConstF rp = (ConstF)(uintptr_t)(enc_rays + (size_t)r * 8);
#pragma unroll
                for (int c = 0; c < 6; ++c) ray_next[c] = rp[c];
            }
        };
        auto gen_stage = [&](int64_t st) {
            if (wave < ENC) {
                const int n = lane & 31, h = lane >> 5;
                bf16x8 e;
                if constexpr (NXT == 9) {
                    const float dv[3] = {ray_next[3], ray_next[4], ray_next[5]};
                    e = dw_encode_slab<4, kDirSlabs>(dv, h, wave);
                } else {
                    const float zv = *reinterpret_cast<const float*>(ring + D * STAGE + g_slot * ZSLOT + n * 4);
                    float xv[3];
#pragma unroll
                    for (int c = 0; c < 3; ++c) xv[c] = nh_add(ray_next[c], nh_mul(ray_next[3 + c], zv));
                    e = dw_encode_slab<10, kXyzSlabs>(xv, h, wave);
                }
                const int unit = (2 * n + h) ^ ((wave & 1) ? 8 : 0);
                *reinterpret_cast<bf16x8*>(ring + g_slot * STAGE + (DYS + wave) * SLAB_BYTES + unit * 16) = e;
            }
            g_slot = (g_slot + 1 == D) ? 0 : g_slot + 1;
            load_ray(st + 1);
        };
        constexpr int REM = NPD % 8;
        constexpr bool SHARE_LAST = (PREC == NERFHIP_BF16) && (REM == 4 || REM == 2);
        const int share_piece = NPD - REM + (SHARE_LAST ? (wave * REM) / 8 : 0);
        const unsigned long long share_mask = REM == 4 ? (0xffffffffull << (32 * (wave & 1))) : (0xffffull << (16 * (wave & 3)));
        auto issue_piece = [&](int i) {
            if constexpr (REGEN) {
                if (i == LPW - 1) {
                    glds4(zsrc, zslot);
                    return;
                }
            }
            int pi = wave + 8 * i;
            const bool shared = SHARE_LAST && i == LPWD - 1;
            if (shared) pi = share_piece;
            if (pi >= NPD) pi = NPD - 1;
            if (REGEN && pi >= DYS) pi += ENC;
            const int sl = pi / SPP, sub = pi % SPP;
            const uint8_t* src;
            if (FOLD && sl >= kDwFoldSigmaSlab) src = dbase + (size_t)(kDySigma + sl - kDwFoldSigmaSlab) * 64 * (16 * SPP) * IL;
            else if (sl < jb.dy_slabs) src = dbase + (size_t)(jb.dy_off + sl) * 64 * (16 * SPP) * IL;
            else if (sl < jb.dy_slabs + jb.x1_slabs) src = abase + (size_t)(jb.x1_off + sl - jb.dy_slabs) * 64 * (16 * SPP) * IL;
            else src = abase + (size_t)(jb.x2_off + sl - jb.dy_slabs - jb.x1_slabs) * 64 * (16 * SPP) * IL;
            const uint8_t* g = src + (size_t)sub * kPieceBytes + ((sl & 1) ? dma_off_odd : dma_off_even);
            const unsigned dst = (unsigned)__builtin_amdgcn_readfirstlane((int)(slot + (unsigned)(pi * kPieceBytes)));
            if (shared) glds16_nt_masked(g, dst, share_mask);
            else glds16_nt(g, dst);
        };
        auto issue_stage = [&](int64_t it) {
            next_stage(it);
#pragma unroll
            for (int i = 0; i < LPW; ++i) issue_piece(i);
        };
        constexpr bool SPREAD = (PREC == NERFHIP_BF16);
        constexpr int DMA_STEP = (2 * NXT) / LPW > 0 ? (2 * NXT) / LPW : 1;
        if constexpr (REGEN) {
            next_z(0);
            glds4(zsrc, zslot);
            load_ray(0);
        }
#pragma unroll
        for (int s = 0; s < D - 1; ++s) issue_stage(s);
        if constexpr (REGEN) {
            wait_vm<(D - 1) * LPW>();
            gen_stage(0);
        }
        for (int64_t it = 0; it < my_tiles; ++it) {
#if NERFHIP_DW_PROBE
            const unsigned t0 = shader_cycles();
            wait_vm<(PREC == NERFHIP_BF16) ? (D - 2) * LPW : 0>();
            const unsigned t1 = shader_cycles();
            asm volatile("s_barrier" ::: "memory");
            const unsigned t2 = shader_cycles();
            pr_wait += (t1 - t0) & 0xffffffffu;
            pr_bar += (t2 - t1) & 0xffffffffu;
#else
            wait_vm_barrier<(PREC == NERFHIP_BF16) ? (D - 2) * LPW : 0>();
#endif
            if (SPREAD && (SPLIT2D || wave < n_ot)) next_stage(it + D - 1);
            else issue_stage(it + D - 1);
#if NERFHIP_DW_PROBE
            const unsigned t3 = shader_cycles();
            pr_issue += (t3 - t2) & 0xffffffffu;
#endif
            const char* st_base = ring + s_use * STAGE;
            s_use = (s_use + 1 == D) ? 0 : s_use + 1;
            if constexpr (SPLIT2D) {
                constexpr int XW = NXT / 2, NF = 2 * XW, RD = kDwFragRing2D;
                static_assert(RD >= 2 && RD <= NF, "B fragment ring");
                const int wi = wave >> 1, wj = wave & 1;
                const char* dyb = st_base + (4 * wi) * SLAB_BYTES;
                const char* x_all = st_base + 16 * SLAB_BYTES;
                const char* xb = x_all + (2 * XW * wj) * SLAB_BYTES;
                auto dma_after = [](int k) constexpr { return ((k + 1) * NF) / LPW - 1; };
                bf16x8 a[2][2], b[RD];
                a[0][0] = load_frag(dyb, 0);
                a[0][1] = load_frag(dyb + 2 * SLAB_BYTES, 0);
#pragma unroll
                for (int f = 0; f < RD - 1; ++f) b[f] = load_frag(xb + 2 * (f % XW) * SLAB_BYTES, f / XW);
                a[1][0] = load_frag(dyb, 1);
                a[1][1] = load_frag(dyb + 2 * SLAB_BYTES, 1);
                __builtin_amdgcn_sched_barrier(0);
#pragma unroll
                for (int f = 0; f < NF; ++f) {
                    if (f + RD - 1 < NF) b[(f + RD - 1) % RD] = load_frag(xb + 2 * ((f + RD - 1) % XW) * SLAB_BYTES, (f + RD - 1) / XW);
                    __builtin_amdgcn_sched_barrier(0);
                    acc[2 * (f % XW)] = __builtin_amdgcn_mfma_f32_32x32x16_bf16(a[f / XW][0], b[f % RD], acc[2 * (f % XW)], 0, 0, 0);
                    acc[2 * (f % XW) + 1] = __builtin_amdgcn_mfma_f32_32x32x16_bf16(a[f / XW][1], b[f % RD], acc[2 * (f % XW) + 1], 0, 0, 0);
                    __builtin_amdgcn_sched_barrier(0);
                    if (f == 0 || f == XW) {
                        const bf16x8 ab = wj ? a[f / XW][1] : a[f / XW][0];
                        dw_bias_sum(ab, dbacc, dbacc2);
                    }
                    if constexpr (SPREAD) {
#pragma unroll
                        for (int k = 0; k < LPW; ++k)
                            if (dma_after(k) == f) {
                                issue_piece(k);
                                __builtin_amdgcn_sched_barrier(0);
                            }
                    }
                }
            } else if (wave < n_ot) {
                const char* dy_base = st_base + (2 * wave) * SLAB_BYTES;
                const char* x_base = st_base + jb.dy_slabs * SLAB_BYTES;
                if constexpr (PREC == NERFHIP_BF16) {
                    constexpr int RD = kDwFragRing, NM = 2 * NXT;
                    const bf16x8 a0 = load_frag(dy_base, 0);
                    bf16x8 b[RD];
#pragma unroll
                    for (int m = 0; m < RD - 1; ++m)
                        if (m < NM) b[m] = load_frag(x_base + 2 * (m % NXT) * SLAB_BYTES, m / NXT);
                    const bf16x8 a1 = load_frag(dy_base, 1);
                    __builtin_amdgcn_sched_barrier(0);
#pragma unroll
                    for (int m = 0; m < NM; ++m) {
                        const int x = m % NXT;
                        if (m + RD - 1 < NM) b[(m + RD - 1) % RD] = load_frag(x_base + 2 * ((m + RD - 1) % NXT) * SLAB_BYTES, (m + RD - 1) / NXT);
                        __builtin_amdgcn_sched_barrier(0);
                        acc[x] = __builtin_amdgcn_mfma_f32_32x32x16_bf16(m < NXT ? a0 : a1, b[m % RD], acc[x], 0, 0, 0);
                        __builtin_amdgcn_sched_barrier(0);
                        if (m == 1) dw_bias_sum(a0, dbacc, dbacc2);
                        if (m == NXT + 1 || (NXT == 1 && m == 1)) dw_bias_sum(a1, dbacc, dbacc2);
                        if constexpr (SPREAD) {
                            if (m % DMA_STEP == DMA_STEP - 1 && m / DMA_STEP < LPW) {
                                issue_piece(m / DMA_STEP);
                                __builtin_amdgcn_sched_barrier(0);
                            }
                        }
                    }
                    if constexpr (SPREAD) {
#pragma unroll
                        for (int i = (2 * NXT) / DMA_STEP; i < LPW; ++i) issue_piece(i);
                    }
                } else {
#pragma unroll 4
                    for (int ks = 0; ks < 16; ++ks) {
                        const int pt = 2 * ks + kk;
                        const float a = *reinterpret_cast<const float*>(dy_base + f32_off + pt * 32);
                        dbacc += a;
#pragma unroll
                        for (int x = 0; x < NXT; ++x) {
                            const float b = *reinterpret_cast<const float*>(x_base + 2 * x * SLAB_BYTES + f32_off + pt * 32);
                            acc[x] = __builtin_amdgcn_mfma_f32_32x32x2f32(a, b, acc[x], 0, 0, 0);
                        }
                    }
                }
            } else if constexpr (FOLD) {
                const char* sg = st_base + kDwFoldSigmaSlab * SLAB_BYTES;
                const char* xs = st_base + (jb.dy_slabs + 2 * (1 + 2 * (wave - kDwFoldRow0))) * SLAB_BYTES;
                if constexpr (PREC == NERFHIP_BF16) {
                    const bf16x8 a0 = load_frag(sg, 0), b00 = load_frag(xs, 0), b10 = load_frag(xs + 2 * SLAB_BYTES, 0);
                    const bf16x8 a1 = load_frag(sg, 1), b01 = load_frag(xs, 1), b11 = load_frag(xs + 2 * SLAB_BYTES, 1);
                    acc[0] = __builtin_amdgcn_mfma_f32_32x32x16_bf16(a0, b00, acc[0], 0, 0, 0);
                    acc[1] = __builtin_amdgcn_mfma_f32_32x32x16_bf16(a0, b10, acc[1], 0, 0, 0);
                    acc[0] = __builtin_amdgcn_mfma_f32_32x32x16_bf16(a1, b01, acc[0], 0, 0, 0);
                    acc[1] = __builtin_amdgcn_mfma_f32_32x32x16_bf16(a1, b11, acc[1], 0, 0, 0);
                    if (wave == kDwFoldRow0) {
                        dw_bias_sum(a0, dbacc, dbacc2);
                        dw_bias_sum(a1, dbacc, dbacc2);
                    }
                } else {
#pragma unroll 4
                    for (int ks = 0; ks < 16; ++ks) {
                        const int pt = 2 * ks + kk;
                        const float a = *reinterpret_cast<const float*>(sg + f32_off + pt * 32);
                        dbacc += a;
                        const float b0 = *reinterpret_cast<const float*>(xs + f32_off + pt * 32);
                        const float b1 = *reinterpret_cast<const float*>(xs + 2 * SLAB_BYTES + f32_off + pt * 32);
                        acc[0] = __builtin_amdgcn_mfma_f32_32x32x2f32(a, b0, acc[0], 0, 0, 0);
                        acc[1] = __builtin_amdgcn_mfma_f32_32x32x2f32(a, b1, acc[1], 0, 0, 0);
                    }
                }
            }
            if constexpr (REGEN) gen_stage(it + 1);
#if NERFHIP_DW_PROBE
            pr_comp += (shader_cycles() - t3) & 0xffffffffu;
#endif
        }
        asm volatile("s_waitcnt vmcnt(0)" ::: "memory");
        float* sl = slabs + (size_t)blockIdx.x * kDwSlabFloats;
        dbacc += dbacc2;
        if constexpr (SPLIT2D) {
            constexpr int XW = NXT / 2;
            const int wi = wave >> 1, wj = wave & 1;
#pragma unroll
            for (int xl = 0; xl < XW; ++xl)
#pragma unroll
                for (int d = 0; d < 2; ++d)
                    dw_store_block(sl + (size_t)((2 * wi + d) * kDwMaxXTiles + XW * wj + xl) * 1024, acc[2 * xl + d], lane);
            sl[8 * kDwMaxXTiles * 64 * 16 + (2 * wi + wj) * 64 + lane] = dbacc;
        } else if (wave < n_ot) {
#pragma unroll
            for (int x = 0; x < NXT; ++x) dw_store_block(sl + (size_t)(wave * kDwMaxXTiles + x) * 1024, acc[x], lane);
            sl[8 * kDwMaxXTiles * 64 * 16 + wave * 64 + lane] = dbacc;
        } else if constexpr (FOLD) {
            dw_store_block(sl + (size_t)dw_fold_block(2 * (wave - kDwFoldRow0)) * 1024, acc[0], lane);
            dw_store_block(sl + (size_t)dw_fold_block(2 * (wave - kDwFoldRow0) + 1) * 1024, acc[1], lane);
            if (wave == kDwFoldRow0) sl[8 * kDwMaxXTiles * 64 * 16 + kDwFoldRow0 * 64 + lane] = dbacc;
        }
    };
    using std::integral_constant;
    using std::false_type;
    using std::true_type;
    bool regen = false;
    if constexpr (PREC == NERFHIP_BF16) regen = enc_rays != nullptr;
    switch (n_xt) {
        case 2:
            if constexpr (PREC == NERFHIP_BF16) {
                if (regen) { run(integral_constant<int, 2>{}, integral_constant<int, 20>{}, true_type{}); break; }
            }
            run(integral_constant<int, 2>{}, integral_constant<int, 20>{}, false_type{});
            break;
        case 4: run(integral_constant<int, 4>{}, integral_constant<int, 10>{}, false_type{}); break;
        case 8:
            if (jb.dy_slabs == 16) run(integral_constant<int, 8>{}, integral_constant<int, 32>{}, false_type{});
            else run(integral_constant<int, 8>{}, integral_constant<int, 18>{}, false_type{});
            break;
        case 9:
            if (jobs.fold_of[(jid / kNumDwJobs) * kNumDwJobs + kDwJobSigma] == jid) {
                if constexpr (PREC == NERFHIP_BF16) {
                    if (regen) { run(integral_constant<int, 9>{}, integral_constant<int, kDwFoldStageSlabs>{}, true_type{}); break; }
                }
                run(integral_constant<int, 9>{}, integral_constant<int, kDwFoldStageSlabs>{}, false_type{});
            } else {
                run(integral_constant<int, 9>{}, integral_constant<int, 26>{}, false_type{});
            }
            break;
        default:
            if constexpr (PREC == NERFHIP_BF16) {
                if (regen) { run(integral_constant<int, 10>{}, integral_constant<int, 36>{}, true_type{}); break; }
            }
            run(integral_constant<int, 10>{}, integral_constant<int, 36>{}, false_type{});
            break;
    }
#if NERFHIP_DW_PROBE
    if (lane == 0 && blockIdx.x < 1024) {
        unsigned* pr = g_dw_probe + ((size_t)blockIdx.x * 8 + wave) * 8;
        pr[0] = (unsigned)my_tiles; pr[1] = pr_wait; pr[2] = pr_bar; pr[3] = pr_issue; pr[4] = pr_comp;
        pr[5] = (unsigned)(__builtin_amdgcn_s_memrealtime() - pr_t00);
        pr[6] = (unsigned)jid; pr[7] = pr_depth;
    }
#endif
}

NH_HD constexpr bool dw_job_has_class(const DwJob& j) {
    const int nxt = (j.x1_slabs + j.x2_slabs) / 2, nsl = j.dy_slabs + j.x1_slabs + j.x2_slabs;
    return (nxt == 2 && nsl == 20) || (nxt == 4 && nsl == 10) || (nxt == 8 && ((nsl == 32 && j.dy_slabs == 16) || (nsl == 18 && j.dy_slabs != 16))) ||
           (nxt == 9 && nsl == 26) || (nxt == 10 && nsl == 36);
}
NH_HD constexpr bool dw_jobs_have_classes() {
    for (int j = 0; j < kNumDwJobs; ++j)
        if (!dw_job_has_class(kDwJobs[j])) return false;
    return true;
}
static_assert(dw_jobs_have_classes(), "mlp_bwd_dw_kernel: a weight-gradient job without a compiled job class");

void launch_dw(int prec, const DwJobTable& jt, float* slabs, int nwg, hipStream_t s) {
    if (prec == NERFHIP_BF16) hipLaunchKernelGGL(mlp_bwd_dw_kernel<NERFHIP_BF16>, dim3(nwg), dim3(512), 0, s, jt, slabs);
    else hipLaunchKernelGGL(mlp_bwd_dw_kernel<NERFHIP_F32>, dim3(nwg), dim3(512), 0, s, jt, slabs);
}
#if NERFHIP_DW_PROBE
int read_dw_probe(unsigned* host_dst, int n_words) {
    return hipMemcpyFromSymbol(host_dst, HIP_SYMBOL(g_dw_probe), (size_t)n_words * 4, 0, hipMemcpyDeviceToHost) == hipSuccess ? 0 : -100;
}
#endif

}
```

nerf_pl_amd/csrc/mlp_dw_plan.h:

```cpp
#pragma once
#include "mlp_bwd_dw.h"

constexpr int kPlanF32 = 0, kPlanBf16 = 1, kPlanBf16F8 = 2;

constexpr int kDwWgsF32 = 512, kDwWgsBf16 = 256, kDwWgsF8 = 256;

static int64_t act_tiles(int64_t n_points, int dtype) {
    const int64_t ppw = 32 * (dtype == kPlanF32 ? 4 : 8);
    return (n_points + ppw - 1) / ppw * (ppw / 32);
}

constexpr int kDwCostA = 150, kDwCostB = 45;
constexpr int kDwMinIters = 48;
static int dw_target_wgs(int dtype) { return dtype == kPlanBf16F8 ? kDwWgsF8 : dtype == kPlanBf16 ? kDwWgsBf16 : kDwWgsF32; }
static int dw_plan(const int64_t* n_points, int n_models, int dtype, nerfhip::DwJobTable* jt) {
    using namespace nerfhip;
    using namespace nerfhip::mlp;
    const int njobs = n_models * kNumDwJobs;
    int64_t units[kDwMaxJobs];
    int64_t cap[kDwMaxJobs];
    int ns[kDwMaxJobs];
    int64_t cost[kDwMaxJobs];
    int total = 0;
    for (int j = 0; j < njobs; ++j) {
        const int64_t tiles = act_tiles(n_points[j / kNumDwJobs], dtype);
        const DwJob& jb = kDwJobs[j % kNumDwJobs];
        const int ca = dtype == kPlanBf16 ? kDwCostA : 1;
        const int cb = dtype == kPlanBf16 ? kDwCostB : 0;
        cost[j] = ca + (int64_t)cb * (jb.dy_slabs + jb.x1_slabs + jb.x2_slabs + (j % kNumDwJobs == kDwJobDir ? 2 : 0));
        units[j] = tiles / (dtype == kPlanBf16F8 ? 2 : 1);
        cap[j] = units[j] / kDwMinIters;
        if (cap[j] < 1) cap[j] = 1;
        if (j % kNumDwJobs == kDwJobFinal || j % kNumDwJobs == kDwJobSigma) {
            cap[j] = 0;
            ns[j] = 0;
            continue;
        }
        ns[j] = 1;
        ++total;
    }
    const int target = dw_target_wgs(dtype);
    while (total < target) {
        int best = -1;
        for (int j = 0; j < njobs; ++j) {
            if (ns[j] >= cap[j]) continue;
            if (best < 0) { best = j; continue; }
            const int64_t a = units[j] * cost[j] * ns[best], b = units[best] * cost[best] * ns[j];
            const int jj = j % kNumDwJobs, bb = best % kNumDwJobs;
            const bool j_big = jj >= 1 && jj <= 7, b_big = bb >= 1 && bb <= 7;
            if (a > b || (a == b && j_big && !b_big)) best = j;
        }
        if (best < 0) break;
        ++ns[best];
        ++total;
    }
    if (jt) {
        int off = 0;
        for (int j = 0; j < kDwMaxJobs; ++j) {
            const int jj = j < njobs ? j : 0;
            jt->job[j] = kDwJobs[jj % kNumDwJobs];
            jt->nsplit[j] = j < njobs ? ns[j] : 0;
            jt->soff[j] = off;
            jt->ntiles[j] = act_tiles(n_points[jj / kNumDwJobs], dtype);
            jt->fold_of[j] = (j < njobs && ns[j] == 0 && j % kNumDwJobs == kDwJobSigma) ? j - kDwJobSigma + kDwJobDir : -1;
            if (j < njobs) off += ns[j];
        }
        jt->soff[kDwMaxJobs] = off;
        jt->njobs = njobs;
    }
    return total;
}
```

nerf_pl_amd/models/train_step.py:

```python
import os

import numpy as np
import torch

from .. import ops
from .mlp_autograd import grad_hooks, grads_ready
from .nerf import ticket_fresh


def fusable(models, embeddings, loss_mod):
    from ..losses import MSELoss
    from .rendering import _fusable
    return (isinstance(loss_mod, MSELoss) and _fusable(models, embeddings)
            and len({m.mlp_dtype for m in models}) == 1
            and all(p.requires_grad for m in models for p in m.parameters()))


def _forward_launches(models, rays, rgbs, S, N, dtype, use_disp, perturb, perturb_rand, noise_c, noise_f, noise_std, white_back, u, gscale,
                      packs, acts_c, dev):
    z, raw_c = ops.mlp_fwd_rays_coarse(rays, S, packs[0][0], False, dtype, use_disp, perturb, perturb_rand, save=acts_c)
    if N > 0:
        _, opac_c, rgb_c, depth_c, g_raw_c, zf = ops.composite_train_fine_z(raw_c, z, rays, noise_c, noise_std, white_back, rgbs,
                                                                            gscale, N, u=u)
        acts_f = ops.alloc_acts(zf.numel(), dtype, dev)
        raw_f = ops.mlp_fwd_rays(rays, zf, packs[1][0], False, dtype, save=acts_f)
        opac_f, rgb_f, depth_f, g_raw_f, out3 = ops.composite_train_loss(raw_f, zf, rays, noise_f, noise_std, white_back, rgbs,
                                                                        gscale, rgb_coarse=rgb_c)
        entries = [(g_raw_f, raw_f, packs[1][1], acts_f), (g_raw_c, raw_c, packs[0][1], acts_c)]
        outs = [rgb_c, depth_c, opac_c, rgb_f, depth_f, opac_f]
    else:
        opac_c, rgb_c, depth_c, g_raw_c, out3 = ops.composite_train_loss(raw_c, z, rays, noise_c, noise_std, white_back, rgbs, gscale)
        entries = [(g_raw_c, raw_c, packs[0][1], acts_c)]
        outs = [rgb_c, depth_c, opac_c]
    return outs, entries, out3


_regen_enc = os.environ.get("NERFHIP_REGEN_ENC", "0") == "1"


def regen_enc_enabled():
    return _regen_enc


def set_regen_enc(on):
    global _regen_enc
    prev, _regen_enc = _regen_enc, bool(on)
    return prev


class _TrainRender(torch.autograd.Function):
    @staticmethod
    def forward(ctx, cfg, rays, rgbs, *params):
        models, S, use_disp, perturb, noise_std, N, white_back, adam, draws, packed = cfg
        rays = rays.float().contiguous()
        rgbs = rgbs.float().contiguous()
        B = rays.shape[0]
        dev = rays.device
        dtype = models[0].mlp_dtype
        if draws is None:
            from .. import draws as D
            draws = D.step_draws(B, S, N, perturb, noise_std, dev)
        perturb_rand = draws.get("perturb_rand") if perturb > 0 else None
        noise_c, noise_f = draws.get("noise_coarse"), draws.get("noise_fine")
        u = draws.get("u") if (N > 0 and perturb != 0) else None
        if noise_std != 0 and (noise_c is None or (N > 0 and noise_f is None)):
            raise ValueError("render_rays_train: noise_std != 0 needs the noise draws")
        packs = ([m.train_buffers(dtype, dev) for m in models] if ticket_fresh(packed, models, dtype)
                 else ops.pack_models_train(models, dtype))
        gscale = float(np.float32(2.0) / np.float32(3 * B))
        acts_c = ops.alloc_acts(B * S, dtype, dev)
        if ops.render_supported(B, S, N, dtype):
            acts_f = ops.alloc_acts(B * (S + N), dtype, dev) if N > 0 else None
            regen = regen_enc_enabled() and ops.mlp_dtype_code(dtype) == ops.BF16 and S % 32 == 0 and (S + N) % 32 == 0
            o = ops.render_train_fwd(rays, rgbs, gscale, S, N, packs[0][0], packs[1][0] if N > 0 else None, dtype, acts_c, acts_f,
                                     use_disp, perturb, perturb_rand, noise_c, noise_f, noise_std, white_back, u, regen_enc=regen)
            out3 = o["out3"]
            outs = [o["rgb_coarse"], o["depth_coarse"], o["opacity_coarse"]]
            entries = [(o["g_raw_coarse"], o["raw_coarse"], packs[0][1], acts_c) + ((rays, o["z_coarse"]) if regen else ())]
            if N > 0:
                outs += [o["rgb_fine"], o["depth_fine"], o["opacity_fine"]]
                entries.insert(0, (o["g_raw_fine"], o["raw_fine"], packs[1][1], acts_f) + ((rays, o["z_fine"]) if regen else ()))
        else:
            outs, entries, out3 = _forward_launches(models, rays, rgbs, S, N, dtype, use_disp, perturb, perturb_rand, noise_c, noise_f, noise_std,
                                                    white_back, u, gscale, packs, acts_c, dev)
        ctx.models = [models[1], models[0]] if N > 0 else [models[0]]
        ctx.entries, ctx.dtype, ctx.adam = entries, dtype, adam
        ctx.n_params = [len(m.flat_params()) for m in models]
        ctx.serials = [m.pack_serial() for m in ctx.models]
        ctx.mark_non_differentiable(out3, *outs)
        ctx.set_materialize_grads(False)
        return (out3[0], out3) + tuple(outs)

    @staticmethod
    def backward(ctx, g_loss, *_unused):
        n_models = len(ctx.n_params)
        if g_loss is None:
            return (None, None, None) + (None,) * sum(ctx.n_params)
        entries = ctx.entries
        g_scale = None if ops.is_unit_seed(g_loss) else g_loss.reshape(1).float().contiguous()
        models, dtype = ctx.models, ctx.dtype
        for m, serial in zip(models, ctx.serials):
            m.check_pack_serial(serial)
        hooked, joint_hook = grad_hooks(models)
        adam = None
        if not hooked:
            if ctx.adam is not None and any(p.grad is not None for m in models for p in m.flat_params()):
                ctx.adam = None
            adam = ctx.adam.handle(models) if ctx.adam is not None else None
        groups = [[k] for k in range(n_models)] if hooked and joint_hook is None else [list(range(n_models))]
        grads = []
        for group in groups:
            got = ops.mlp_bwd_multi([entries[k] for k in group], dtype, adam=adam, g_scale=g_scale)
            grads_ready([models[k] for k in group], [g[2] for g in got])
            grads += got
        if adam is not None:
            ctx.adam.applied_in_backward(models)
        ctx.entries = None
        by_model = {id(m): g for m, g in zip(models, grads)}
        out = []
        order = [models[-1]] + models[:-1] if n_models == 2 else models
        for m in order:
            gw, gb, _ = by_model[id(m)]
            out += gw + gb
        return (None, None, None) + tuple(out)


def render_rays_train(models, embeddings, rays, rgbs, N_samples=64, use_disp=False, perturb=0, noise_std=1, N_importance=0,
                      white_back=False, adam=None, draws=None, packed=None):
    N = int(N_importance)
    use = list(models[:2]) if N > 0 else [models[0]]
    params = [p for m in use for p in m.flat_params()]
    cfg = (use, int(N_samples), bool(use_disp), float(perturb), float(noise_std), N, bool(white_back), adam, draws, packed)
    res = _TrainRender.apply(cfg, rays, rgbs, *params)
    loss, out3 = res[0], res[1]
    results = {'rgb_coarse': res[2], 'depth_coarse': res[3], 'opacity_coarse': res[4]}
    if N > 0:
        results.update(rgb_fine=res[5], depth_fine=res[6], opacity_fine=res[7])
    return results, loss, out3
```

nerf_pl_amd/ops.py:

```python
import ctypes
import os

import torch

from . import _lib
from ._lib import BF16, BF16_F8, F32, NerfHipError, check, device_guard, ptr, require_gpu, stream_ptr

_DTYPES = {"fp32": F32, "f32": F32, "float32": F32, torch.float32: F32, F32: F32,
           "bf16": BF16, "bfloat16": BF16, torch.bfloat16: BF16, "bf16_f8": BF16_F8}


def mlp_dtype_code(d):
    if isinstance(d, bool) or d not in _DTYPES:
        raise ValueError("mlp dtype must be 'fp32', 'bf16' or 'bf16_f8', got %r" % (d,))
    return _DTYPES[d]


def _c(t):
    return t if t.is_contiguous() else t.contiguous()


def _check_draw(op, name, t, numel):
    if t is not None and (t.numel() != numel or t.dtype != torch.float32):
        raise ValueError("%s: %s must hold %d fp32 draws, got %s %s" % (op, name, numel, tuple(t.shape), t.dtype))


def _noise_arg(op, name, noise, noise_std, numel):
    if noise_std == 0 or noise is None:
        return None
    noise = _c(noise)
    _check_draw(op, name, noise, numel)
    return noise


def _u_arg(op, u, B, K):
    if u is None:
        return None, 0
    if tuple(u.shape) not in ((B, K), (K,)) or u.dtype != torch.float32:
        raise ValueError("%s: u must be (N_importance,) or (B, N_importance) = (%d, %d) fp32, got %s %s"
                         % (op, B, K, tuple(u.shape), u.dtype))
    return _c(u), (K if u.dim() == 2 else 0)


def _perturb_arg(op, perturb, perturb_rand, numel):
    if not perturb > 0:
        return None
    if perturb_rand is None:
        raise ValueError("%s: perturb>0 needs perturb_rand" % op)
    perturb_rand = _c(perturb_rand)
    _check_draw(op, "perturb_rand", perturb_rand, numel)
    return perturb_rand


def _train_composite_args(op, raw, z, rays, target):
    raw, z, rays, target = _c(raw), _c(z), _c(rays), _c(target)
    B, S = z.shape
    if raw.numel() != B * S * 4 or target.numel() != B * 3:
        raise ValueError("%s: raw must be (B,S,4) and target (B,3)" % op)
    return raw, z, rays, target, B, S


def _train_composite_outs(B, S, dev):
    f32 = dict(device=dev, dtype=torch.float32)
    return torch.empty(B, **f32), torch.empty(B, 3, **f32), torch.empty(B, **f32), torch.empty(B, S, 4, **f32)


_TICKETS = {}
_CAPTURES = {}
_EAGER_SLOTS = {}
_TICKET_WORDS = 1024


def _ticket(device):
    st = torch.cuda.current_stream(device)
    capturing = torch.cuda.is_current_stream_capturing()
    rec = _CAPTURES.setdefault((device.index, st.stream_id), [False, 0])
    if capturing and not rec[0]:
        rec[1] += 1
    rec[0] = capturing
    pool = _TICKETS.get(device.index)
    if pool is None:
        if capturing:
            raise NerfHipError("the ticket words of this GPU must exist before a capture: run the step once eagerly first")
        pool = _TICKETS[device.index] = torch.zeros(_TICKET_WORDS * 4, device=device, dtype=torch.int32)
    if capturing:
        slot = 32 + rec[1] % (_TICKET_WORDS - 32)
    else:
        slot = _EAGER_SLOTS.setdefault((device.index, st.stream_id), len([k for k in _EAGER_SLOTS if k[0] == device.index]) % 32)
    return pool[4 * slot:4 * slot + 4]


class _PosEnc(torch.autograd.Function):
    @staticmethod
    def forward(ctx, x, n_freqs, bands):
        require_gpu(x, bands)
        x = _c(x)
        n, C = x.shape
        out = torch.empty(n, C * (2 * n_freqs + 1), device=x.device, dtype=torch.float32)
        check(_lib.load().nerfhip_posenc_bands(ptr(x), ptr(bands), ptr(out), n, C, n_freqs, stream_ptr()), "nerfhip_posenc")
        ctx.save_for_backward(x)
        ctx.n_freqs, ctx.bands = n_freqs, bands
        return out

    @staticmethod
    def backward(ctx, gout):
        (x,) = ctx.saved_tensors
        gout = _c(gout.float())
        gx = torch.empty_like(x)
        n, C = x.shape
        check(_lib.load().nerfhip_posenc_bands_bwd(ptr(x), ptr(ctx.bands), ptr(gout), ptr(gx), n, C, ctx.n_freqs, stream_ptr()),
              "nerfhip_posenc_bwd")
        return gx, None, None


@device_guard
def posenc(x, n_freqs, bands=None):
    if x.dim() != 2:
        raise ValueError("posenc expects (n, C)")
    if bands is not None:
        if bands.numel() != int(n_freqs):
            raise ValueError("posenc: need one band per frequency")
        bands = bands.to(x.device, torch.float32).contiguous()
    return _PosEnc.apply(x, int(n_freqs), bands)


@device_guard
def sample_coarse_z(rays, n_samples, use_disp=False, perturb=0.0, perturb_rand=None):
    require_gpu(rays, perturb_rand)
    rays = _c(rays)
    B = rays.shape[0]
    perturb_rand = _perturb_arg("sample_coarse_z", perturb, perturb_rand, B * n_samples)
    z = torch.empty(B, n_samples, device=rays.device, dtype=torch.float32)
    check(_lib.load().nerfhip_sample_coarse_z(ptr(rays), ptr(perturb_rand), ptr(z), B, n_samples, int(bool(use_disp)),
                                              float(perturb), stream_ptr()), "nerfhip_sample_coarse_z")
    return z


@device_guard
def searchsorted(a, v, out=None, side="left"):
    require_gpu(a, v)
    if side not in ("left", "right"):
        raise ValueError("side must be 'left' or 'right'")
    if a.dim() != 2 or v.dim() != 2 or not (a.shape[0] == v.shape[0] or a.shape[0] == 1 or v.shape[0] == 1):
        raise ValueError("searchsorted expects a (B,M) and v (B,K), or one of them with a single row")
    rows = max(a.shape[0], v.shape[0])
    a, v = _c(a.expand(rows, a.shape[1])), _c(v.expand(rows, v.shape[1]))
    B, M = a.shape
    K = v.shape[1]
    if out is None:
        out = torch.empty(B, K, device=a.device, dtype=torch.int64)
    elif out.dtype != torch.int64 or not out.is_contiguous() or tuple(out.shape) != (B, K):
        raise ValueError("out must be a contiguous int64 (B,K) tensor")
    fn = _lib.load().nerfhip_searchsorted_right if side == "right" else _lib.load().nerfhip_searchsorted_left
    check(fn(ptr(a), ptr(v), ptr(out), B, M, K, stream_ptr()), "nerfhip_searchsorted_" + side)
    return out


_ROW_TOTAL_MODES = {"exact": 0, "aten": 1}
_row_total = _ROW_TOTAL_MODES[os.environ.get("NERFHIP_ROW_TOTAL", "aten")]


def set_row_total(mode):
    global _row_total
    prev = [k for k, v in _ROW_TOTAL_MODES.items() if v == _row_total][0]
    _row_total = _ROW_TOTAL_MODES[mode]
    return prev


@device_guard
def sample_pdf_u(bins, weights, n_importance, u=None, eps=1e-5, return_cdf_inds=False):
    require_gpu(bins, weights, u)
    if bins.stride(-1) != 1:
        bins = bins.contiguous()
    if weights.stride(-1) != 1:
        weights = weights.contiguous()
    B, M = weights.shape
    if bins.shape != (B, M + 1):
        raise ValueError("bins must be (N_rays, N_samples_+1)")
    u, u_stride = _u_arg("sample_pdf", u, B, n_importance)
    samples = torch.empty(B, n_importance, device=bins.device, dtype=torch.float32)
    cdf = torch.empty(B, M + 1, device=bins.device, dtype=torch.float32) if return_cdf_inds else None
    inds = torch.empty(B, n_importance, device=bins.device, dtype=torch.int64) if return_cdf_inds else None
    check(_lib.load().nerfhip_sample_pdf_ex(ptr(bins), bins.stride(0), ptr(weights), weights.stride(0), ptr(u), u_stride,
                                            ptr(samples), B, M, n_importance, float(eps), ptr(cdf), ptr(inds), _row_total,
                                            stream_ptr()),
          "nerfhip_sample_pdf")
    return (samples, cdf, inds) if return_cdf_inds else samples


@device_guard
def fine_z(z_coarse, w_coarse, n_importance, u=None, eps=1e-5, return_new=False, return_cdf_inds=False):
    require_gpu(z_coarse, w_coarse, u)
    z_coarse, w_coarse = _c(z_coarse), _c(w_coarse)
    B, S = z_coarse.shape
    u, u_stride = _u_arg("fine_z", u, B, n_importance)
    zf = torch.empty(B, S + n_importance, device=z_coarse.device, dtype=torch.float32)
    zn = torch.empty(B, n_importance, device=z_coarse.device, dtype=torch.float32) if return_new else None
    cdf = torch.empty(B, S - 1, device=z_coarse.device, dtype=torch.float32) if return_cdf_inds else None
    inds = torch.empty(B, n_importance, device=z_coarse.device, dtype=torch.int64) if return_cdf_inds else None
    check(_lib.load().nerfhip_fine_z_ex(ptr(z_coarse), ptr(w_coarse), ptr(u), u_stride, ptr(zf), ptr(zn), B, S,
                                        n_importance, float(eps), ptr(cdf), ptr(inds), _row_total, stream_ptr()), "nerfhip_fine_z")
    out = (zf, zn) if return_new else (zf,)
    if return_cdf_inds:
        out = out + (cdf, inds)
    return out if len(out) > 1 else out[0]


class _Composite(torch.autograd.Function):
    @staticmethod
    def forward(ctx, raw, z, rays, noise, noise_std, white_back):
        require_gpu(raw, z, rays, noise)
        raw, z, rays = _c(raw), _c(z), _c(rays)
        B, S = z.shape
        raw_ch = 4 if raw.dim() == 3 else 1
        if raw.numel() != B * S * raw_ch:
            raise ValueError("raw must be (B,S,4) or (B,S)")
        if noise is not None:
            noise = _c(noise)
        dev = z.device
        weights = torch.empty(B, S, device=dev, dtype=torch.float32)
        opacity = torch.empty(B, device=dev, dtype=torch.float32)
        rgb = torch.empty(B, 3, device=dev, dtype=torch.float32) if raw_ch == 4 else None
        depth = torch.empty(B, device=dev, dtype=torch.float32) if raw_ch == 4 else None
        check(_lib.load().nerfhip_composite_fwd(ptr(raw), raw_ch, ptr(z), ptr(rays), ptr(noise), float(noise_std),
                                                int(bool(white_back)), ptr(weights), ptr(rgb), ptr(depth),
                                                ptr(opacity), B, S, stream_ptr()), "nerfhip_composite_fwd")
        ctx.save_for_backward(raw, z, rays, noise)
        ctx.cfg = (raw_ch, float(noise_std), int(bool(white_back)))
        ctx.set_materialize_grads(False)
        if raw_ch == 4:
            return weights, opacity, rgb, depth
        return weights, opacity

    @staticmethod
    def backward(ctx, g_weights, g_opacity, g_rgb=None, g_depth=None):
        raw, z, rays, noise = ctx.saved_tensors
        raw_ch, noise_std, white_back = ctx.cfg
        B, S = z.shape

        def prep(g):
            return None if g is None else _c(g.float())

        g_raw = torch.empty_like(raw)
        check(_lib.load().nerfhip_composite_bwd(ptr(raw), raw_ch, ptr(z), ptr(rays), ptr(noise), noise_std, white_back,
                                                ptr(prep(g_rgb)), ptr(prep(g_depth)), ptr(prep(g_opacity)),
                                                ptr(prep(g_weights)), ptr(g_raw), B, S, stream_ptr()),
              "nerfhip_composite_bwd")
        return g_raw, None, None, None, None, None


@device_guard
def composite(raw, z, rays, noise=None, noise_std=0.0, white_back=False):
    if noise_std == 0:
        noise = None
    return _Composite.apply(raw, z, rays, noise, float(noise_std), bool(white_back))


@device_guard
def composite_train(raw, z, rays, noise, noise_std, white_back, target, grad_scale, want_weights=True):
    require_gpu(raw, z, rays, noise, target)
    raw, z, rays, target, B, S = _train_composite_args("composite_train", raw, z, rays, target)
    noise = _noise_arg("composite_train", "noise", noise, noise_std, B * S)
    weights = torch.empty(B, S, device=z.device, dtype=torch.float32) if want_weights else None
    opacity, rgb, depth, g_raw = _train_composite_outs(B, S, z.device)
    check(_lib.load().nerfhip_composite_train(ptr(raw), ptr(z), ptr(rays), ptr(noise), float(noise_std), int(bool(white_back)),
                                              ptr(target), float(grad_scale), ptr(weights), ptr(rgb), ptr(depth), ptr(opacity),
                                              ptr(g_raw), B, S, stream_ptr()), "nerfhip_composite_train")
    return weights, opacity, rgb, depth, g_raw


@device_guard
def composite_train_fine_z(raw, z, rays, noise, noise_std, white_back, target, grad_scale, n_importance, u=None, eps=1e-5,
                           want_weights=False):
    require_gpu(raw, z, rays, noise, target, u)
    raw, z, rays, target, B, S = _train_composite_args("composite_train_fine_z", raw, z, rays, target)
    noise = _noise_arg("composite_train_fine_z", "noise", noise, noise_std, B * S)
    u, u_stride = _u_arg("composite_train_fine_z", u, B, n_importance)
    dev = z.device
    weights = torch.empty(B, S, device=dev, dtype=torch.float32) if want_weights else None
    opacity, rgb, depth, g_raw = _train_composite_outs(B, S, dev)
    zf = torch.empty(B, S + n_importance, device=dev, dtype=torch.float32)
    check(_lib.load().nerfhip_composite_train_fine_z(ptr(raw), ptr(z), ptr(rays), ptr(noise), float(noise_std), int(bool(white_back)),
                                                     ptr(target), float(grad_scale), ptr(weights), ptr(rgb), ptr(depth), ptr(opacity),
                                                     ptr(g_raw), B, S, ptr(u), u_stride, int(n_importance), float(eps), ptr(zf),
                                                     _row_total, stream_ptr()), "nerfhip_composite_train_fine_z")
    return weights, opacity, rgb, depth, g_raw, zf


@device_guard
def composite_train_loss(raw, z, rays, noise, noise_std, white_back, target, grad_scale, rgb_coarse=None):
    require_gpu(raw, z, rays, noise, target, rgb_coarse)
    raw, z, rays, target, B, S = _train_composite_args("composite_train_loss", raw, z, rays, target)
    if rgb_coarse is not None:
        rgb_coarse = _c(rgb_coarse)
        if rgb_coarse.numel() != B * 3:
            raise ValueError("composite_train_loss: rgb_coarse must be (B,3)")
    noise = _noise_arg("composite_train_loss", "noise", noise, noise_std, B * S)
    dev = z.device
    opacity, rgb, depth, g_raw = _train_composite_outs(B, S, dev)
    out3 = torch.empty(3, device=dev, dtype=torch.float32)
    check(_lib.load().nerfhip_composite_train_loss(ptr(raw), ptr(z), ptr(rays), ptr(noise), float(noise_std), int(bool(white_back)),
                                                   ptr(target), float(grad_scale), None, ptr(rgb), ptr(depth), ptr(opacity), ptr(g_raw),
                                                   B, S, ptr(rgb_coarse), ptr(out3), ptr(_ticket(dev)), stream_ptr()),
          "nerfhip_composite_train_loss")
    return opacity, rgb, depth, g_raw, out3


class _MsePsnr(torch.autograd.Function):
    @staticmethod
    def forward(ctx, rgb_c, rgb_f, target):
        require_gpu(rgb_c, rgb_f, target)
        rgb_c, target = _c(rgb_c), _c(target)
        rgb_f = _c(rgb_f) if rgb_f is not None else None
        n = target.numel()
        if rgb_c.numel() != n or (rgb_f is not None and rgb_f.numel() != n):
            raise ValueError("mse_psnr: shape mismatch")
        out3 = torch.empty(3, device=target.device, dtype=torch.float32)
        g_c = torch.empty_like(rgb_c)
        g_f = torch.empty_like(rgb_f) if rgb_f is not None else None
        check(_lib.load().nerfhip_mse_psnr(ptr(rgb_c), ptr(rgb_f), ptr(target), n, ptr(out3), ptr(g_c), ptr(g_f), stream_ptr()),
              "nerfhip_mse_psnr")
        ctx.save_for_backward(g_c, g_f)
        ctx.mark_non_differentiable(out3)
        ctx.set_materialize_grads(False)
        return out3[0], out3

    @staticmethod
    def backward(ctx, g_loss, _g_out3):
        g_c, g_f = ctx.saved_tensors
        if g_loss is None:
            return None, None, None
        if is_unit_seed(g_loss):
            return g_c, g_f, None
        if g_f is None:
            return g_c * g_loss, None, None
        g_c, g_f = torch._foreach_mul([g_c, g_f], g_loss)
        return g_c, g_f, None


_UNIT_SEEDS = {}


def unit_seed(like):
    key = (like.device.type, like.device.index)
    t = _UNIT_SEEDS.get(key)
    if t is None:
        t = _UNIT_SEEDS[key] = torch.ones((), device=like.device, dtype=torch.float32)
    return t


def is_unit_seed(g):
    t = _UNIT_SEEDS.get((g.device.type, g.device.index))
    return t is not None and g.data_ptr() == t.data_ptr() and g.numel() == 1


@device_guard
def mse_psnr_values(rgb_coarse, rgb_fine, target):
    require_gpu(rgb_coarse, rgb_fine, target)
    rgb_coarse, target = _c(rgb_coarse), _c(target)
    rgb_fine = _c(rgb_fine) if rgb_fine is not None else None
    out3 = torch.empty(3, device=target.device, dtype=torch.float32)
    check(_lib.load().nerfhip_mse_psnr(ptr(rgb_coarse), ptr(rgb_fine), ptr(target), target.numel(), ptr(out3), None, None, stream_ptr()),
          "nerfhip_mse_psnr")
    return out3


@device_guard
def mse_psnr(rgb_coarse, rgb_fine, target):
    return _MsePsnr.apply(rgb_coarse, rgb_fine, target)


PARAM_ORDER = ["xyz_encoding_1.0", "xyz_encoding_2.0", "xyz_encoding_3.0", "xyz_encoding_4.0",
               "xyz_encoding_5.0", "xyz_encoding_6.0", "xyz_encoding_7.0", "xyz_encoding_8.0",
               "xyz_encoding_final", "dir_encoding.0", "sigma", "rgb.0"]
PARAM_SHAPES = [(256, 63), (256, 256), (256, 256), (256, 256), (256, 319), (256, 256), (256, 256), (256, 256),
                (256, 256), (128, 283), (1, 256), (3, 128)]


DEFAULT_ARCH_ONLY = "the fused HIP MLP implements the reference's default architecture (D=8, W=256, skips=[4], 63/27 inputs) only"


def packed_bytes(dtype):
    return int(_lib.load().nerfhip_mlp_packed_bytes(mlp_dtype_code(dtype)))


def packed_bwd_bytes(dtype):
    return int(_lib.load().nerfhip_mlp_packed_bwd_bytes(mlp_dtype_code(dtype)))


def pack_arg_tables(weights, biases):
    if len(weights) != 12 or len(biases) != 12:
        raise ValueError("need 12 weights and 12 biases")
    for i, (w, b) in enumerate(zip(weights, biases)):
        require_gpu(w, b)
        if tuple(w.shape) != PARAM_SHAPES[i] or tuple(b.shape) != (PARAM_SHAPES[i][0],):
            raise NerfHipError("%s; got %s for %s" % (DEFAULT_ARCH_ONLY, tuple(w.shape), PARAM_ORDER[i]))
        if not (w.is_contiguous() and b.is_contiguous()):
            raise NerfHipError("NeRF parameters must be contiguous")
    wp = (ctypes.c_void_p * 12)(*[w.data_ptr() for w in weights])
    bp = (ctypes.c_void_p * 12)(*[b.data_ptr() for b in biases])
    return wp, bp


@device_guard
def pack_weights_raw(wp, bp, out, dtype):
    check(_lib.load().nerfhip_mlp_pack_weights(wp, bp, ptr(out), mlp_dtype_code(dtype), stream_ptr()), "nerfhip_mlp_pack_weights")


@device_guard
def pack_weights_bwd_raw(wp, bp, out, dtype):
    check(_lib.load().nerfhip_mlp_pack_weights_bwd(wp, bp, ptr(out), mlp_dtype_code(dtype), stream_ptr()),
          "nerfhip_mlp_pack_weights_bwd")


@device_guard
def pack_weights_train_raw(wp, bp, out, out_bwd, dtype):
    check(_lib.load().nerfhip_mlp_pack_weights_train(wp, bp, ptr(out), ptr(out_bwd), mlp_dtype_code(dtype), stream_ptr()),
          "nerfhip_mlp_pack_weights_train")


def alloc_acts(n_points, dtype, device):
    nbytes = int(_lib.load().nerfhip_mlp_act_bytes(int(n_points), mlp_dtype_code(dtype)))
    return torch.empty(nbytes, device=device, dtype=torch.uint8)


@device_guard
def mlp_fwd_embedded(x, packed, sigma_only, dtype, save=None):
    require_gpu(x)
    if x.dim() != 2 or x.stride(1) != 1:
        x = x.reshape(-1, x.shape[-1]).contiguous()
    n = x.shape[0]
    need = 63 if sigma_only else 90
    if x.shape[1] != need:
        raise ValueError("NeRF.forward expects %d input channels, got %d" % (need, x.shape[1]))
    out = torch.empty(n, 1 if sigma_only else 4, device=x.device, dtype=torch.float32)
    check(_lib.load().nerfhip_mlp_fwd_embedded(ptr(x), x.stride(0), n, ptr(packed), ptr(out), int(bool(sigma_only)),
                                               mlp_dtype_code(dtype), ptr(save), stream_ptr()),
          "nerfhip_mlp_fwd_embedded")
    return out


@device_guard
def mlp_fwd_rays(rays, z, packed, sigma_only, dtype, save=None):
    require_gpu(rays, z)
    rays, z = _c(rays), _c(z)
    B, S = z.shape
    out = torch.empty((B, S) if sigma_only else (B, S, 4), device=z.device, dtype=torch.float32)
    check(_lib.load().nerfhip_mlp_fwd_rays(ptr(rays), ptr(z), B, S, ptr(packed), ptr(out), int(bool(sigma_only)),
                                           mlp_dtype_code(dtype), ptr(save), stream_ptr()), "nerfhip_mlp_fwd_rays")
    return out


@device_guard
def mlp_fwd_rays_coarse(rays, n_samples, packed, sigma_only, dtype, use_disp=False, perturb=0.0, perturb_rand=None, save=None):
    require_gpu(rays, perturb_rand)
    rays = _c(rays)
    B, S = rays.shape[0], int(n_samples)
    perturb_rand = _perturb_arg("mlp_fwd_rays_coarse", perturb, perturb_rand, B * S)
    z = torch.empty(B, S, device=rays.device, dtype=torch.float32)
    out = torch.empty((B, S) if sigma_only else (B, S, 4), device=rays.device, dtype=torch.float32)
    check(_lib.load().nerfhip_mlp_fwd_rays_coarse(ptr(rays), ptr(perturb_rand), ptr(z), B, S,
                                                  int(bool(use_disp)), float(perturb), ptr(packed), ptr(out), int(bool(sigma_only)),
                                                  mlp_dtype_code(dtype), ptr(save), stream_ptr()), "nerfhip_mlp_fwd_rays_coarse")
    return z, out


_render_fused = os.environ.get("NERFHIP_RENDER_FUSED", "1") != "0"


def set_render_fused(on):
    global _render_fused
    prev, _render_fused = _render_fused, bool(on)
    return prev


def render_supported(B, S_c, N_i, dtype):
    if not _render_fused:
        return False
    return bool(_lib.load().nerfhip_render_supported(int(B), int(S_c), int(N_i), mlp_dtype_code(dtype)))


def _render_args(rays, S, N, packed_c, packed_f, use_disp, perturb, perturb_rand, noise_c, noise_f, noise_std, white_back, u, eps,
                 want_coarse, coarse_sigma_only=False):
    B = rays.shape[0]
    dev = rays.device
    f32 = dict(device=dev, dtype=torch.float32)
    a = _lib.RenderArgs()
    bufs = {"z_coarse": torch.empty(B, S, **f32), "opacity_coarse": torch.empty(B, **f32),
            "raw_coarse": torch.empty((B, S) if coarse_sigma_only else (B, S, 4), **f32)}
    if want_coarse:
        bufs.update(rgb_coarse=torch.empty(B, 3, **f32), depth_coarse=torch.empty(B, **f32))
    if N > 0:
        bufs.update(z_fine=torch.empty(B, S + N, **f32), raw_fine=torch.empty(B, S + N, 4, **f32), rgb_fine=torch.empty(B, 3, **f32),
                    depth_fine=torch.empty(B, **f32), opacity_fine=torch.empty(B, **f32))
    perturb_rand = _perturb_arg("render", perturb, perturb_rand, B * S)
    noise_c = _noise_arg("render", "noise_coarse", noise_c, noise_std, B * S)
    noise_f = _noise_arg("render", "noise_fine", noise_f if N > 0 else None, noise_std, B * (S + N))
    if noise_std != 0 and (noise_c is None or (N > 0 and noise_f is None)):
        raise ValueError("render: noise_std != 0 needs the noise draws")
    u, u_stride = _u_arg("render", u if N > 0 else None, B, N)
    a.rays, a.B, a.S_c, a.N_i = rays.data_ptr(), B, int(S), int(N)
    a.packed_coarse = packed_c.data_ptr()
    a.packed_fine = packed_f.data_ptr() if packed_f is not None else None
    for k, t in bufs.items():
        setattr(a, k, t.data_ptr())
    a.perturb_rand = perturb_rand.data_ptr() if perturb_rand is not None else None
    a.perturb, a.use_disp = float(perturb), int(bool(use_disp))
    a.noise_coarse = noise_c.data_ptr() if noise_c is not None else None
    a.noise_fine = noise_f.data_ptr() if noise_f is not None else None
    a.noise_std, a.white_back = float(noise_std), int(bool(white_back))
    a.u, a.u_stride, a.eps, a.row_total = (u.data_ptr() if u is not None else None), u_stride, float(eps), _row_total
    keep = (rays, packed_c, packed_f, perturb_rand, noise_c, noise_f, u)
    return a, bufs, keep


@device_guard
def render_fwd(rays, n_samples, n_importance, packed_coarse, packed_fine, dtype, use_disp=False, perturb=0.0, perturb_rand=None,
               noise_coarse=None, noise_fine=None, noise_std=0.0, white_back=False, u=None, eps=1e-5, want_coarse=True, test_time=False):
    require_gpu(rays, perturb_rand, noise_coarse, noise_fine, u)
    rays = _c(rays)
    tt = bool(test_time) and int(n_importance) > 0
    a, bufs, keep = _render_args(rays, n_samples, n_importance, packed_coarse, packed_fine, use_disp, perturb, perturb_rand,
                                 noise_coarse, noise_fine, noise_std, white_back, u, eps, want_coarse and not tt, coarse_sigma_only=tt)
    if tt:
        check(_lib.load().nerfhip_render_test_fwd(ctypes.addressof(a), mlp_dtype_code(dtype), stream_ptr()), "nerfhip_render_test_fwd")
    else:
        check(_lib.load().nerfhip_render_fwd(ctypes.addressof(a), mlp_dtype_code(dtype), stream_ptr()), "nerfhip_render_fwd")
    return bufs


@device_guard
def render_train_fwd(rays, target, grad_scale, n_samples, n_importance, packed_coarse, packed_fine, dtype, acts_coarse, acts_fine,
                     use_disp=False, perturb=0.0, perturb_rand=None, noise_coarse=None, noise_fine=None, noise_std=0.0,
                     white_back=False, u=None, eps=1e-5, regen_enc=False):
    require_gpu(rays, target, perturb_rand, noise_coarse, noise_fine, u)
    rays, target = _c(rays), _c(target)
    B, S, N = rays.shape[0], int(n_samples), int(n_importance)
    if target.numel() != 3 * B or target.dtype != torch.float32:
        raise ValueError("render_train_fwd: target must be (B,3) fp32")
    a, bufs, keep = _render_args(rays, S, N, packed_coarse, packed_fine, use_disp, perturb, perturb_rand, noise_coarse, noise_fine,
                                 noise_std, white_back, u, eps, True)
    dev = rays.device
    bufs["g_raw_coarse"] = torch.empty(B, S, 4, device=dev, dtype=torch.float32)
    if N > 0:
        bufs["g_raw_fine"] = torch.empty(B, S + N, 4, device=dev, dtype=torch.float32)
    bufs["out3"] = torch.empty(3, device=dev, dtype=torch.float32)
    a.g_raw_coarse = bufs["g_raw_coarse"].data_ptr()
    a.g_raw_fine = bufs["g_raw_fine"].data_ptr() if N > 0 else None
    a.out3 = bufs["out3"].data_ptr()
    a.save_coarse = acts_coarse.data_ptr()
    a.save_fine = acts_fine.data_ptr() if N > 0 else None
    a.target, a.grad_scale = target.data_ptr(), float(grad_scale)
    a.ticket = _ticket(dev).data_ptr()
    a.regen_enc = int(bool(regen_enc) and mlp_dtype_code(dtype) == BF16)
    check(_lib.load().nerfhip_render_train_fwd(ctypes.addressof(a), mlp_dtype_code(dtype), stream_ptr()), "nerfhip_render_train_fwd")
    return bufs


FLAT_GRAD_FLOATS = sum(s[0] * s[1] + s[0] for s in PARAM_SHAPES)


def flat_grad_views(n_points, device, shapes=PARAM_SHAPES, out=None):
    sizes = [s[0] * s[1] for s in shapes] + [s[0] for s in shapes]
    if out is not None:
        flat = out
        if n_points == 0:
            flat.zero_()
    else:
        flat = (torch.zeros if n_points == 0 else torch.empty)(sum(sizes), device=device, dtype=torch.float32)
    views, off = [], 0
    for sz in sizes:
        views.append(flat[off:off + sz])
        off += sz
    return [v.view(s) for v, s in zip(views[:12], shapes)], views[12:], flat


@device_guard
def mlp_bwd(g_out, out, packed_bwd, acts, dtype, shapes=PARAM_SHAPES, phases=7, workspace=None):
    require_gpu(g_out, out)
    code = mlp_dtype_code(dtype)
    g_out = _c(g_out.float()).reshape(-1, 4)
    out = _c(out).reshape(-1, 4)
    n = out.shape[0]
    dev = out.device
    lib = _lib.load()
    if workspace is not None and "dys" in workspace:
        dys, ws = workspace["dys"], workspace["ws"]
    else:
        dys = torch.empty(int(lib.nerfhip_mlp_dy_bytes(n, code)), device=dev, dtype=torch.uint8)
        ws = torch.empty(int(lib.nerfhip_mlp_dw_workspace_bytes(n, code)), device=dev, dtype=torch.uint8)
        if workspace is not None:
            workspace["dys"], workspace["ws"] = dys, ws
    gw, gb, flat = flat_grad_views(n, dev, shapes)
    gwp = (ctypes.c_void_p * 12)(*[t.data_ptr() for t in gw])
    gbp = (ctypes.c_void_p * 12)(*[t.data_ptr() for t in gb])
    check(lib.nerfhip_mlp_bwd_phases(ptr(g_out), ptr(out), n, ptr(packed_bwd), ptr(acts), ptr(dys), ptr(ws), gwp, gbp, 0, code,
                                     int(phases), stream_ptr()), "nerfhip_mlp_bwd")
    return gw, gb, flat


@device_guard
def mlp_dx_embedded(dys, n, w_xyz1, w_xyz5, w_dir, dtype):
    code = mlp_dtype_code(dtype)
    if code == BF16_F8:
        raise NotImplementedError("nerfhip_mlp_dx_embedded reads bf16 / fp32 dY slabs ('bf16_f8' keeps dY only as e5m2: NeRF.forward "
                                  "saves in bf16 for calls whose input requires grad, models/mlp_autograd.py)")
    require_gpu(w_xyz1, w_xyz5, w_dir)
    gx = torch.empty(n, 90, device=dys.device, dtype=torch.float32)
    check(_lib.load().nerfhip_mlp_dx_embedded(ptr(dys), n, ptr(_c(w_xyz1.detach())), ptr(_c(w_xyz5.detach())), ptr(_c(w_dir.detach())),
                                              ptr(gx), 90, code, stream_ptr()), "nerfhip_mlp_dx_embedded")
    return gx


def pack_tables(models, dtype):
    if not 1 <= len(models) <= 4:
        raise ValueError("pack_models_train packs 1..4 models")
    tabs, bufs = [], []
    for m in models:
        if not m.is_default_arch():
            raise NotImplementedError(DEFAULT_ARCH_ONLY)
        wp, bp, dev = m._pack_args()
        tabs.append((wp, bp))
        bufs.append(m.train_buffers(dtype, dev))
    n = len(models)
    W = (ctypes.c_void_p * (12 * n))(*[t[0][i] for t in tabs for i in range(12)])
    Bv = (ctypes.c_void_p * (12 * n))(*[t[1][i] for t in tabs for i in range(12)])
    P = (ctypes.c_void_p * n)(*[b[0].data_ptr() for b in bufs])
    Pb = (ctypes.c_void_p * n)(*[b[1].data_ptr() for b in bufs])
    return W, Bv, P, Pb, bufs


def pack_models_train(models, dtype):
    W, Bv, P, Pb, bufs = pack_tables(models, dtype)
    with torch.cuda.device(bufs[0][0].device):
        check(_lib.load().nerfhip_mlp_pack_weights_train_multi(W, Bv, P, Pb, len(models), mlp_dtype_code(dtype), stream_ptr()),
              "nerfhip_mlp_pack_weights_train_multi")
    for m in models:
        m.images_packed()
    return bufs


def mlp_bwd_multi(entries, dtype, adam=None, phases=7, workspace=None, g_scale=None):
    code = mlp_dtype_code(dtype)
    lib = _lib.load()
    M = len(entries)
    dev = entries[0][1].device
    gs, outs, ns, dys, grads = [], [], [], [], []
    enc, keep_enc = None, []
    for m, e in enumerate(entries):
        g_out, out = e[0], e[1]
        if len(e) > 4 and e[4] is not None:
            if enc is None:
                enc = _lib.EncSource()
            rays_e, z_e = _c(e[4]), _c(e[5])
            require_gpu(rays_e, z_e)
            if rays_e.dtype != torch.float32 or z_e.dtype != torch.float32 or z_e.dim() != 2 or rays_e.shape[0] != z_e.shape[0]:
                raise ValueError("mlp_bwd_multi: (rays (B,8), z (B,S)) fp32 expected")
            enc.rays[m], enc.z[m], enc.S[m] = rays_e.data_ptr(), z_e.data_ptr(), int(z_e.shape[1])
            keep_enc.append((rays_e, z_e))
        require_gpu(g_out, out)
        g_out = _c(g_out.float()).reshape(-1, 4)
        out = _c(out).reshape(-1, 4)
        gs.append(g_out)
        outs.append(out)
        ns.append(out.shape[0])
    with torch.cuda.device(dev):
        n_arr = (ctypes.c_int64 * M)(*ns)
        key = ("multi", tuple(ns), code)
        if workspace is not None and key in workspace:
            dys, ws = workspace[key]
        else:
            dys = [torch.empty(int(lib.nerfhip_mlp_dy_bytes(n, code)), device=dev, dtype=torch.uint8) for n in ns]
            ws = torch.empty(int(lib.nerfhip_mlp_dw_workspace_bytes_multi(n_arr, M, code)), device=dev, dtype=torch.uint8)
            if workspace is not None:
                workspace[key] = (dys, ws)
        joint = torch.empty(M * FLAT_GRAD_FLOATS, device=dev, dtype=torch.float32)
        for m, n in enumerate(ns):
            grads.append(flat_grad_views(n, dev, out=joint[m * FLAT_GRAD_FLOATS:(m + 1) * FLAT_GRAD_FLOATS]))
        vp = ctypes.c_void_p
        G = (vp * M)(*[t.data_ptr() for t in gs])
        O = (vp * M)(*[t.data_ptr() for t in outs])
        PB = (vp * M)(*[e[2].data_ptr() for e in entries])
        AC = (vp * M)(*[e[3].data_ptr() for e in entries])
        DY = (vp * M)(*[t.data_ptr() for t in dys])
        GW = (vp * (12 * M))(*[t.data_ptr() for g in grads for t in g[0]])
        GB = (vp * (12 * M))(*[t.data_ptr() for g in grads for t in g[1]])
        if adam is not None:
            for m in range(M):
                adam.grad_flat[m] = grads[m][2].data_ptr()
        if g_scale is not None:
            require_gpu(g_scale)
        check(lib.nerfhip_mlp_bwd_multi_rays(M, G, O, n_arr, PB, AC, DY, ptr(ws), GW, GB, 0, code, int(phases), ptr(g_scale),
                                             ctypes.addressof(adam) if adam is not None else None,
                                             ctypes.addressof(enc) if enc is not None else None, stream_ptr()), "nerfhip_mlp_bwd_multi_rays")
    return grads


ACT_NONE, ACT_RELU, ACT_SIGMOID = 0, 1, 2


def _rows(t):
    if t.dim() != 2:
        raise ValueError("expected a (n, channels) tensor")
    if t.stride(1) != 1 or t.stride(0) < t.shape[1]:
        t = t.contiguous()
    return t


def _off(t, col):
    return ctypes.c_void_p(t.data_ptr() + 4 * col)


class _LinearAct(torch.autograd.Function):

    @staticmethod
    def forward(ctx, act, dtype, w, b, *xs):
        xs = [_rows(x.float()) for x in xs]
        require_gpu(w, b, *xs)
        w, b = _c(w), _c(b)
        n, n_out, k_tot = xs[0].shape[0], w.shape[0], w.shape[1]
        if sum(x.shape[1] for x in xs) != k_tot or any(x.shape[0] != n for x in xs) or b.numel() != n_out:
            raise ValueError("linear: input segments %s do not match the weight %s" % ([tuple(x.shape) for x in xs], tuple(w.shape)))
        lib = _lib.load()
        code = mlp_dtype_code(dtype)
        y = torch.empty(n, n_out, device=w.device, dtype=torch.float32)
        col = 0
        for s, x in enumerate(xs):
            last = s == len(xs) - 1
            check(lib.nerfhip_linear_fwd(ptr(x), x.stride(0), _off(w, col), k_tot, ptr(b) if last else None, ptr(y), n_out, n,
                                         x.shape[1], n_out, act if last else ACT_NONE, int(s > 0), code, stream_ptr()),
                  "nerfhip_linear_fwd")
            col += x.shape[1]
        ctx.cfg = (act, code)
        ctx.save_for_backward(w, y, *xs)
        return y

    @staticmethod
    def backward(ctx, gy):
        w, y, *xs = ctx.saved_tensors
        act, code = ctx.cfg
        lib = _lib.load()
        gy = _c(gy.float())
        n, n_out, k_tot = y.shape[0], w.shape[0], w.shape[1]
        need_w, need_b = ctx.needs_input_grad[2], ctx.needs_input_grad[3]
        gw = gb = None
        gxs = []
        if (need_w or need_b) and n > 0:
            gw = torch.empty_like(w)
            gb = torch.empty(n_out, device=w.device, dtype=torch.float32)
            ws_bytes = max(lib.nerfhip_linear_bwd_weight_workspace_bytes(n, x.shape[1], n_out) for x in xs)
            ws = torch.empty(ws_bytes, device=w.device, dtype=torch.uint8)
        elif need_w or need_b:
            gw, gb = torch.zeros_like(w), torch.zeros(n_out, device=w.device, dtype=torch.float32)
        col = 0
        for s, x in enumerate(xs):
            if (need_w or need_b) and n > 0:
                check(lib.nerfhip_linear_bwd_weight(ptr(gy), n_out, ptr(y), n_out, act, ptr(x), x.stride(0), _off(gw, col), k_tot,
                                                    ptr(gb) if s == 0 else None, ptr(ws), n, x.shape[1], n_out, 0, code,
                                                    stream_ptr()), "nerfhip_linear_bwd_weight")
            gx = None
            if ctx.needs_input_grad[4 + s]:
                gx = torch.empty(n, x.shape[1], device=w.device, dtype=torch.float32)
                check(lib.nerfhip_linear_bwd_input(ptr(gy), n_out, ptr(y), n_out, act, _off(w, col), k_tot, ptr(gx), x.shape[1], n,
                                                   x.shape[1], n_out, 0, code, stream_ptr()), "nerfhip_linear_bwd_input")
            gxs.append(gx)
            col += x.shape[1]
        return (None, None, gw if need_w else None, gb if need_b else None) + tuple(gxs)


@device_guard
def linear_act(xs, weight, bias, act, dtype):
    return _LinearAct.apply(int(act), dtype, weight, bias, *xs)


_INT32_MAX = 2 ** 31 - 1


def _require_mesh(name, t, dtype, shape_len=None, cols=None):
    if not torch.is_tensor(t):
        raise NerfHipError("%s: expected a torch tensor, got %s" % (name, type(t).__name__))
    if not t.is_cuda:
        raise NerfHipError("nerf_pl_amd runs on MI355X only: %s is a %s tensor (no CPU fallback)" % (name, t.device))
    if t.dtype != dtype:
        raise NerfHipError("%s: expected %s, got %s" % (name, dtype, t.dtype))
    if shape_len is not None and t.dim() != shape_len:
        raise NerfHipError("%s: expected rank %d, got shape %s" % (name, shape_len, tuple(t.shape)))
    if cols is not None and t.shape[-1] != cols:
        raise NerfHipError("%s: expected %d columns, got shape %s" % (name, cols, tuple(t.shape)))
    return _c(t)


def _check_vertex_ids(triangles, V):
    if triangles.numel() and (int(triangles.min()) < 0 or int(triangles.max()) >= V):
        raise NerfHipError("triangles reference vertices outside [0, %d)" % V)


@device_guard
def marching_cubes(volume, iso):
    volume = _require_mesh("marching_cubes volume", volume, torch.float32, 3)
    n0, n1, n2 = volume.shape
    if min(n0, n1, n2) < 2:
        raise NerfHipError("marching_cubes: every dimension must be >= 2, got %s" % (tuple(volume.shape),))
    lib = _lib.load()
    ws_bytes = lib.nerfhip_marching_cubes_workspace_bytes(n0, n1, n2)
    if ws_bytes == 0:
        raise NerfHipError("marching_cubes: volume %s has 2^31 or more lattice points" % (tuple(volume.shape),))
    ws = torch.empty(ws_bytes, device=volume.device, dtype=torch.uint8)
    totals = torch.empty(2, device=volume.device, dtype=torch.int64)
    check(lib.nerfhip_marching_cubes_count(ptr(volume), n0, n1, n2, float(iso), ptr(ws), ptr(totals), stream_ptr()),
          "nerfhip_marching_cubes_count")
    V, T = (int(x) for x in totals.cpu())
    if V > _INT32_MAX or T > _INT32_MAX:
        raise NerfHipError("marching_cubes: %d vertices / %d triangles do not fit int32" % (V, T))
    verts = torch.empty(V, 3, device=volume.device, dtype=torch.float64)
    tris = torch.empty(T, 3, device=volume.device, dtype=torch.int32)
    if V or T:
        check(lib.nerfhip_marching_cubes_emit(ptr(volume), n0, n1, n2, float(iso), ptr(ws), ptr(totals), ptr(verts), ptr(tris),
                                              stream_ptr()), "nerfhip_marching_cubes_emit")
    return verts, tris


@device_guard
def largest_cluster(triangles, n_vertices):
    triangles = _require_mesh("triangles", triangles, torch.int32, 2, 3)
    T, V = triangles.shape[0], int(n_vertices)
    dev = triangles.device
    if T == 0 or V == 0:
        return torch.empty(0, device=dev, dtype=torch.int64), torch.empty(0, 3, device=dev, dtype=torch.int32)
    if V > _INT32_MAX or 3 * T > _INT32_MAX:
        raise NerfHipError("largest_cluster: mesh too large (V=%d, T=%d)" % (V, T))
    _check_vertex_ids(triangles, V)
    lib = _lib.load()
    keys = torch.empty(3 * T, device=dev, dtype=torch.int64)
    check(lib.nerfhip_mesh_edge_keys(ptr(triangles), T, ptr(keys), stream_ptr()), "nerfhip_mesh_edge_keys")
    sorted_keys, order = torch.sort(keys, stable=True)
    ws = torch.empty(lib.nerfhip_mesh_cluster_workspace_bytes(V, T), device=dev, dtype=torch.uint8)
    totals = torch.empty(3, device=dev, dtype=torch.int64)
    check(lib.nerfhip_mesh_largest_cluster(ptr(triangles), V, T, ptr(sorted_keys), ptr(order), ptr(ws), ptr(totals), stream_ptr()),
          "nerfhip_mesh_largest_cluster")
    t_kept, v_kept, status = (int(x) for x in totals.cpu())
    if status:
        raise NerfHipError("largest_cluster: the union-find gave up after its retry bound")
    kept_ids = torch.empty(v_kept, device=dev, dtype=torch.int64)
    kept_tris = torch.empty(t_kept, 3, device=dev, dtype=torch.int32)
    check(lib.nerfhip_mesh_cluster_compact(ptr(triangles), V, T, ptr(ws), ptr(kept_ids), ptr(kept_tris), stream_ptr()),
          "nerfhip_mesh_cluster_compact")
    return kept_ids, kept_tris


@device_guard
def vertex_normals(vertices, triangles):
    vertices = _require_mesh("vertices", vertices, torch.float32, 2, 3)
    triangles = _require_mesh("triangles", triangles, torch.int32, 2, 3)
    V, T = vertices.shape[0], triangles.shape[0]
    out = torch.empty(V, 3, device=vertices.device, dtype=torch.float64)
    if V == 0:
        return out
    _check_vertex_ids(triangles, V)
    check(_lib.load().nerfhip_mesh_vertex_normals(ptr(vertices), V, ptr(triangles), T, ptr(out), stream_ptr()),
          "nerfhip_mesh_vertex_normals")
    return out


@device_guard
def normal_rays(vertices, normals, near, far, near_t):
    vertices = _require_mesh("vertices", vertices, torch.float32, 2, 3)
    normals = _require_mesh("normals", normals, torch.float64, 2, 3)
    V = vertices.shape[0]
    rays = torch.empty(V, 8, device=vertices.device, dtype=torch.float32)
    if V:
        check(_lib.load().nerfhip_mesh_normal_rays(ptr(vertices), ptr(normals), V, float(near), float(far), float(near_t), ptr(rays),
                                                   stream_ptr()), "nerfhip_mesh_normal_rays")
    return rays


@device_guard
def view_rays(vertices, w2c, origin, focal, image, near):
    import numpy as np
    vertices = _require_mesh("vertices", vertices, torch.float32, 2, 3)
    image = _require_mesh("image", image, torch.uint8, 3, 3)
    H, W = image.shape[0], image.shape[1]
    V = vertices.shape[0]
    dev = vertices.device
    colors = torch.empty(V, 4, device=dev, dtype=torch.uint8)
    depth = torch.empty(V, device=dev, dtype=torch.float64)
    rays = torch.empty(V, 8, device=dev, dtype=torch.float32)
    if V:
        w = np.ascontiguousarray(np.asarray(w2c, np.float32).reshape(3, 4))
        o = np.ascontiguousarray(np.asarray(origin, np.float32).reshape(3))
        fp = ctypes.POINTER(ctypes.c_float)
        check(_lib.load().nerfhip_mesh_view_rays(ptr(vertices), V, w.ctypes.data_as(fp), o.ctypes.data_as(fp), float(np.float32(focal)),
                                                 W, H, ptr(image), float(near), ptr(colors), ptr(depth), ptr(rays), stream_ptr()),
              "nerfhip_mesh_view_rays")
    return colors, depth, rays


@device_guard
def color_accumulate(colors, depth, opacity, occ_threshold, accum):
    colors = _require_mesh("colors", colors, torch.uint8, 2, 4)
    depth = _require_mesh("depth", depth, torch.float64, 1)
    opacity = _require_mesh("opacity", opacity, torch.float32, 1)
    accum = _require_mesh("accum", accum, torch.float64, 2, 4)
    V = colors.shape[0]
    if V:
        check(_lib.load().nerfhip_mesh_color_accumulate(ptr(colors), ptr(depth), ptr(opacity), V, float(occ_threshold), ptr(accum),
                                                        stream_ptr()), "nerfhip_mesh_color_accumulate")
    return accum


@device_guard
def color_finish(accum):
    accum = _require_mesh("accum", accum, torch.float64, 2, 4)
    V = accum.shape[0]
    out = torch.empty(V, 3, device=accum.device, dtype=torch.uint8)
    if V:
        check(_lib.load().nerfhip_mesh_color_finish(ptr(accum), V, ptr(out), stream_ptr()), "nerfhip_mesh_color_finish")
    return out


@device_guard
def rgb_to_u8(rgb):
    rgb = _require_mesh("rgb", rgb, torch.float32)
    out = torch.empty(rgb.shape, device=rgb.device, dtype=torch.uint8)
    if rgb.numel():
        check(_lib.load().nerfhip_mesh_rgb_to_u8(ptr(rgb), rgb.numel(), ptr(out), stream_ptr()), "nerfhip_mesh_rgb_to_u8")
    return out


IMAGE_PLANAR, IMAGE_INTERLEAVED = 0, 1


@device_guard
def ssim(img1, img2, B, C, H, W, window_size=3, layout=IMAGE_PLANAR, want_map=False, want_mean=True):
    require_gpu(img1, img2)
    B, C, H, W, window_size = int(B), int(C), int(H), int(W), int(window_size)
    if min(B, C, H, W) < 0 or img1.numel() != B * C * H * W or img2.numel() != img1.numel():
        raise NerfHipError("ssim: images of %s and %s elements are not %d x %d x %d x %d" % (img1.numel(), img2.numel(), B, C, H, W))
    if window_size % 2 == 0 or not 3 <= window_size <= 11:
        raise NerfHipError("ssim: window_size must be odd and in 3..11, got %d" % window_size)
    img1, img2 = _c(img1), _c(img2)
    dev = img1.device
    lib = _lib.load()
    shape = (B, C, H, W) if layout == IMAGE_PLANAR else (B, H, W, C)
    out_map = torch.empty(shape, device=dev, dtype=torch.float32) if want_map else None
    mean = ws = None
    if want_mean:
        mean = torch.full((), float("nan"), device=dev, dtype=torch.float32) if img1.numel() == 0 else \
            torch.empty((), device=dev, dtype=torch.float32)
        ws = torch.empty(max(1, lib.nerfhip_ssim_workspace_bytes(B, C, H, W) // 8), device=dev, dtype=torch.float64)
    check(lib.nerfhip_ssim(ptr(img1), ptr(img2), B, C, H, W, window_size, int(layout), ptr(out_map), ptr(mean), ptr(ws), stream_ptr()),
          "nerfhip_ssim")
    return out_map, mean


def _require_depth_table(table, device):
    if not torch.is_tensor(table) or not table.is_cuda or table.dtype != torch.uint8 or tuple(table.shape) != (256, 3) \
            or table.device != device:
        raise NerfHipError("depth_colormap: the colour table must be a (256, 3) uint8 tensor on %s" % (device,))
    return _c(table)


@device_guard
def depth_colormap(depth, table, want_float=True, want_bytes=False):
    require_gpu(depth)
    table = _require_depth_table(table, depth.device)
    depth = _c(depth)
    n, dev = depth.numel(), depth.device
    lib = _lib.load()
    out_f = torch.empty((3,) + tuple(depth.shape), device=dev, dtype=torch.float32) if want_float else None
    out_b = torch.empty(tuple(depth.shape) + (3,), device=dev, dtype=torch.uint8) if want_bytes else None
    ws = torch.empty(max(1, lib.nerfhip_depth_colormap_workspace_bytes(n) // 4), device=dev, dtype=torch.float32)
    check(lib.nerfhip_depth_colormap(ptr(depth), n, ptr(table), ptr(out_f), ptr(out_b), ptr(ws), stream_ptr()),
          "nerfhip_depth_colormap")
    return out_f, out_b


GIF_STRIP = 3838


def gif_workspace(F, H, W, device):
    nbytes = _lib.load().nerfhip_gif_workspace_bytes(F, H, W)
    if F > 0 and nbytes == 0:
        raise NerfHipError("gif: %d frames of %d x %d are refused (1..65535 per side, at most 2^26 pixels, at most 65535 frames)"
                           % (F, H, W))
    return torch.empty(max(1, nbytes // 8), device=device, dtype=torch.int64)


@device_guard
def gif_quantize(frames, workspace=None):
    frames = _require_u8("gif_quantize: frames", frames)
    if frames.dim() != 4 or frames.shape[3] != 3:
        raise NerfHipError("gif_quantize: expected (F, H, W, 3), got %s" % (tuple(frames.shape),))
    F, H, W = frames.shape[:3]
    dev = frames.device
    lib = _lib.load()
    ws = workspace if workspace is not None else gif_workspace(F, H, W, dev)
    indices = torch.empty((F, H * W), device=dev, dtype=torch.uint8)
    palettes = torch.empty((F, 256, 3), device=dev, dtype=torch.uint8)
    boxes = torch.empty((F,), device=dev, dtype=torch.int32)
    check(lib.nerfhip_gif_quantize(ptr(frames), F, H, W, ptr(indices), ptr(palettes), ptr(boxes), ptr(ws), stream_ptr()),
          "nerfhip_gif_quantize")
    return indices, palettes, boxes


@device_guard
def gif_lzw(indices, H, W, workspace=None):
    indices = _require_u8("gif_lzw: indices", indices)
    if indices.dim() != 2 or indices.shape[1] != H * W:
        raise NerfHipError("gif_lzw: expected (F, %d) indices for %d x %d frames, got %s" % (H * W, H, W, tuple(indices.shape)))
    F = indices.shape[0]
    dev = indices.device
    lib = _lib.load()
    ws = workspace if workspace is not None else gif_workspace(F, H, W, dev)
    stride = lib.nerfhip_gif_data_stride(H, W)
    data = torch.empty((F, stride), device=dev, dtype=torch.uint8)
    lengths = torch.empty((F,), device=dev, dtype=torch.int32)
    check(lib.nerfhip_gif_lzw(ptr(indices), F, H, W, ptr(data), ptr(lengths), ptr(ws), stream_ptr()), "nerfhip_gif_lzw")
    return data, lengths


def _require_u8(name, t):
    if not torch.is_tensor(t):
        raise NerfHipError("%s: expected a torch tensor, got %s" % (name, type(t).__name__))
    if not t.is_cuda:
        raise NerfHipError("nerf_pl_amd runs on MI355X only: %s is a %s tensor (no CPU fallback)" % (name, t.device))
    if t.dtype != torch.uint8:
        raise NerfHipError("%s: expected uint8, got %s" % (name, t.dtype))
    return _c(t)


@device_guard
def decode_png_batch(streams, H, W, ch, return_flags=False):
    streams = _require_u8("decode_png_batch streams", streams)
    H, W, ch = int(H), int(W), int(ch)
    if ch not in (1, 3, 4) or H < 1 or W < 1:
        raise NerfHipError("decode_png_batch: H, W >= 1 and ch in (1, 3, 4), got %d x %d x %d" % (H, W, ch))
    if streams.dim() != 2 or streams.shape[1] != H * (1 + W * ch):
        raise NerfHipError("decode_png_batch: expected (n, %d) bytes per %d x %d x %d image, got %s"
                           % (H * (1 + W * ch), H, W, ch, tuple(streams.shape)))
    n = streams.shape[0]
    out = torch.empty(n, H, W, ch, device=streams.device, dtype=torch.uint8)
    flags = torch.empty(n, device=streams.device, dtype=torch.int32)
    check(_lib.load().nerfhip_png_unfilter(ptr(streams), ptr(out), ptr(flags), n, H, W, ch, stream_ptr()), "nerfhip_png_unfilter")
    if return_flags:
        return out, flags
    if n and bool(flags.any()):
        raise NerfHipError("decode_png_batch: image(s) %s hold a scanline filter type above 4" % flags.nonzero().flatten().tolist())
    return out


_TAPS = {}


def _lanczos_taps_device(in_size, out_size, device):
    key = (int(in_size), int(out_size), str(device))
    if key not in _TAPS:
        from .imageio_min import lanczos_taps
        if len(_TAPS) > 16:
            _TAPS.clear()
        _TAPS[key] = tuple(torch.from_numpy(a).to(device) for a in lanczos_taps(in_size, out_size))
    return _TAPS[key]


@device_guard
def resize_rgba_lanczos(u8, w, h):
    u8 = _require_u8("resize_rgba_lanczos image", u8)
    if u8.dim() not in (3, 4) or u8.shape[-1] != 4:
        raise NerfHipError("resize_rgba_lanczos: expected (n, H, W, 4) or (H, W, 4), got %s" % (tuple(u8.shape),))
    w, h = int(w), int(h)
    single = u8.dim() == 3
    n, H, W = (1,) + tuple(u8.shape[:2]) if single else tuple(u8.shape[:3])
    if min(w, h, H, W) < 1:
        raise NerfHipError("resize_rgba_lanczos: empty image")
    dev = u8.device
    out = torch.empty(n, h, w, 4, device=dev, dtype=torch.uint8)
    th = _lanczos_taps_device(W, w, dev) if W != w else (None, None, None)
    tv = _lanczos_taps_device(H, h, dev) if H != h else (None, None, None)
    ws = torch.empty(n, H, w, 4, device=dev, dtype=torch.uint8) if (W != w and H != h) else None
    check(_lib.load().nerfhip_resize_rgba_lanczos(ptr(u8), ptr(out), ptr(ws), n, H, W, h, w, ptr(th[0]), ptr(th[1]), ptr(th[2]),
                                                  th[2].shape[1] if th[2] is not None else 0, ptr(tv[0]), ptr(tv[1]), ptr(tv[2]),
                                                  tv[2].shape[1] if tv[2] is not None else 0, stream_ptr()),
          "nerfhip_resize_rgba_lanczos")
    return out[0] if single else out


@device_guard
def rgba_to_rgb_white(u8, out=None):
    u8 = _require_u8("rgba_to_rgb_white image", u8)
    if u8.dim() < 1 or u8.shape[-1] != 4:
        raise NerfHipError("rgba_to_rgb_white: expected (..., 4) uint8, got %s" % (tuple(u8.shape),))
    n = u8.numel() // 4
    if out is None:
        out = torch.empty(n, 3, device=u8.device, dtype=torch.float32)
    else:
        require_gpu(out)
        if out.device != u8.device or tuple(out.shape) != (n, 3) or not out.is_contiguous():
            raise NerfHipError("rgba_to_rgb_white: out must be a contiguous (%d, 3) float32 tensor on %s" % (n, u8.device))
    mask = torch.empty(n, device=u8.device, dtype=torch.uint8)
    check(_lib.load().nerfhip_rgba_to_rgb_white(ptr(u8), ptr(out), ptr(mask), n, stream_ptr()), "nerfhip_rgba_to_rgb_white")
    return out, mask.view(torch.bool)


def jpeg_entropy_decode(parsed):
    import numpy as np
    comps = parsed["components"]
    mx, my = int(parsed["mcus_x"]), int(parsed["mcus_y"])
    table = np.zeros((8, 272), np.uint8)
    mask = 0
    for (tc, th), (counts, symbols) in parsed["huffman"].items():
        table[4 * tc + th, :16] = counts
        table[4 * tc + th, 16:16 + len(symbols)] = symbols
        mask |= 1 << (4 * tc + th)
    comp = np.ascontiguousarray([[c[1], c[2], c[4], c[5]] for c in comps], dtype=np.int32)
    coef = [np.zeros((my * c[2], mx * c[1], 64), np.int16) for c in comps]
    scan = np.frombuffer(parsed["scan"], np.uint8)
    ptrs = (ctypes.c_void_p * len(comps))(*[a.ctypes.data for a in coef])
    caps = (ctypes.c_int64 * len(comps))(*[a.shape[0] * a.shape[1] for a in coef])
    code = _lib.load().nerfhip_jpeg_entropy_decode(scan.ctypes.data, len(scan), len(comps), comp.ctypes.data, table.ctypes.data, mask,
                                                   mx, my, int(parsed["restart_interval"]), ptrs, caps)
    if code != 0:
        msg = _lib.load().nerfhip_error_string(code).decode()
        raise NerfHipError("%s: nerfhip_jpeg_entropy_decode failed: %s (code %d)" % (parsed.get("name", "JPEG data"), msg, code))
    return coef


def _require_i16(name, t, device, shape):
    if not torch.is_tensor(t):
        raise NerfHipError("%s: expected a torch tensor, got %s" % (name, type(t).__name__))
    if not t.is_cuda:
        raise NerfHipError("nerf_pl_amd runs on MI355X only: %s is a %s tensor (no CPU fallback)" % (name, t.device))
    if t.dtype != torch.int16 or tuple(t.shape) != tuple(shape) or (device is not None and t.device != device):
        raise NerfHipError("%s: expected int16 %s on %s, got %s %s on %s" % (name, tuple(shape), device, t.dtype, tuple(t.shape), t.device))
    return _c(t)


@device_guard
def decode_jpeg_batch(coefs, quant, H, W, hs=1, vs=1):
    if torch.is_tensor(coefs):
        coefs = [coefs]
    coefs = list(coefs)
    H, W, hs, vs = int(H), int(W), int(hs), int(vs)
    n_comp = len(coefs)
    lib = _lib.load()
    plane_bytes = lib.nerfhip_jpeg_planes_bytes(H, W, n_comp, hs, vs) if n_comp in (1, 3) else 0
    if plane_bytes == 0:
        raise NerfHipError("decode_jpeg_batch: %d component(s) of %d x %d with luma sampling %dx%d is not supported (1 component, "
                           "or 3 with 1x1, 2x1 or 2x2)" % (n_comp, W, H, hs, vs))
    if not torch.is_tensor(coefs[0]) or coefs[0].dim() < 2:
        raise NerfHipError("decode_jpeg_batch: coefs must be (n, blocks, 64) int16 tensors")
    n, dev = coefs[0].shape[0], coefs[0].device
    mx, my = -(-W // (8 * hs)), -(-H // (8 * vs))
    flat = []
    for c, t in enumerate(coefs):
        blocks = mx * my * (hs * vs if c == 0 else 1)
        if torch.is_tensor(t) and t.dim() == 4:
            t = t.reshape(t.shape[0], -1, 64)
        flat.append(_require_i16("decode_jpeg_batch coefs[%d]" % c, t, dev, (n, blocks, 64)))
    quant = _require_i16("decode_jpeg_batch quant", quant, dev, (n, n_comp, 64))
    out = torch.empty(n, H, W, 4, device=dev, dtype=torch.uint8)
    planes = torch.empty(n * plane_bytes, device=dev, dtype=torch.uint8)
    check(lib.nerfhip_jpeg_decode(ptr(flat[0]), ptr(flat[1]) if n_comp == 3 else None, ptr(flat[2]) if n_comp == 3 else None,
                                  ptr(quant), ptr(planes), ptr(out), n, H, W, n_comp, hs, vs, stream_ptr()), "nerfhip_jpeg_decode")
    return out
```

Baseline: 1.081 million.

## Form first-layer dY inside the dW kernel instead of the backward chain

Adds a flag that stops the bf16 backward chain kernel at dY_2 and has the dW job for the first layer recompute dY_1 on the fly. That job uses the L2^T weights held in registers and streams dY_2 plus the activations through an LDS ring. This removes the chain's last layer pass and the write and re-read of dY_1 through global memory. The cost is extra MFMA work and a larger fetch in the dW job, which the planner accounts for with a new cost constant. The flag is on by default through an environment variable, applies only to bf16 without ray regeneration, and the change also adds an accumulate_into option.

```diff
diff --git a/include/nerfhip.h b/include/nerfhip.h
--- a/include/nerfhip.h
+++ b/include/nerfhip.h
@@ -142,6 +142,15 @@
                                void* dw_workspace, float* const* grad_w_host, float* const* grad_b_host, int accumulate, int dtype,
                                int phases, const float* g_scale, const nerfhip_adam_fused* adam, const nerfhip_enc_source* enc,
                                nerfhip_stream_t stream);
+
+#define NERFHIP_BWD_DY1_IN_DW 1
+size_t nerfhip_mlp_dw_workspace_bytes_multi_flags(const int64_t* n_points_host, int n_models, int dtype, int flags);
+int nerfhip_mlp_dw_plan_flags(const int64_t* n_points_host, int n_models, int dtype, int flags, int* splits_out, int* stage_kib_out);
+int nerfhip_mlp_bwd_multi_flags(int n_models, const float* const* g_out_host, const float* const* out_host, const int64_t* n_host,
+                                const void* const* packed_bwd_host, const void* const* acts_host, void* const* dys_host,
+                                void* dw_workspace, float* const* grad_w_host, float* const* grad_b_host, int accumulate, int dtype,
+                                int phases, const float* g_scale, const nerfhip_adam_fused* adam, const nerfhip_enc_source* enc,
+                                int flags, nerfhip_stream_t stream);
 
 int nerfhip_mlp_dx_embedded(const void* dys, int64_t n, const float* w_xyz1, const float* w_xyz5, const float* w_dir,
                             float* gx, int64_t gx_stride, int dtype, nerfhip_stream_t stream);
diff --git a/nerf_pl_amd/_lib.py b/nerf_pl_amd/_lib.py
--- a/nerf_pl_amd/_lib.py
+++ b/nerf_pl_amd/_lib.py
@@ -8,6 +8,7 @@
 LIB_PATH = os.environ.get("NERFHIP_LIB_PATH") or os.path.join(_PKG, "libnerfhip.so")
 
 F32, BF16, BF16_F8 = 0, 1, 2
+BWD_DY1_IN_DW = 1
 
 _c_void_p = ctypes.c_void_p
 _i64 = ctypes.c_int64
@@ -97,6 +98,12 @@
                                    ctypes.POINTER(_c_void_p), ctypes.POINTER(_c_void_p), ctypes.POINTER(_c_void_p), _c_void_p,
                                    ctypes.POINTER(_c_void_p), ctypes.POINTER(_c_void_p), _int, _int, _int, _c_void_p, _c_void_p, _c_void_p,
                                    _c_void_p],
+    "nerfhip_mlp_dw_workspace_bytes_multi_flags": [ctypes.POINTER(_i64), _int, _int, _int],
+    "nerfhip_mlp_dw_plan_flags": [ctypes.POINTER(_i64), _int, _int, _int, ctypes.POINTER(_int), ctypes.POINTER(_int)],
+    "nerfhip_mlp_bwd_multi_flags": [_int, ctypes.POINTER(_c_void_p), ctypes.POINTER(_c_void_p), ctypes.POINTER(_i64),
+                                    ctypes.POINTER(_c_void_p), ctypes.POINTER(_c_void_p), ctypes.POINTER(_c_void_p), _c_void_p,
+                                    ctypes.POINTER(_c_void_p), ctypes.POINTER(_c_void_p), _int, _int, _int, _c_void_p, _c_void_p, _c_void_p,
+                                    _int, _c_void_p],
     "nerfhip_linear_fwd": [_c_void_p, _i64, _c_void_p, _i64, _c_void_p, _c_void_p, _i64, _i64, _int, _int, _int, _int, _int, _c_void_p],
     "nerfhip_linear_bwd_input": [_c_void_p, _i64, _c_void_p, _i64, _int, _c_void_p, _i64, _c_void_p, _i64, _i64, _int, _int, _int,
                                  _int, _c_void_p],
@@ -175,6 +182,7 @@
              "nerfhip_mlp_act_bytes": ctypes.c_size_t, "nerfhip_mlp_packed_bwd_bytes": ctypes.c_size_t,
              "nerfhip_mlp_dy_bytes": ctypes.c_size_t, "nerfhip_mlp_dw_workspace_bytes": ctypes.c_size_t,
              "nerfhip_mlp_dw_workspace_bytes_multi": ctypes.c_size_t,
+             "nerfhip_mlp_dw_workspace_bytes_multi_flags": ctypes.c_size_t,
              "nerfhip_linear_bwd_weight_workspace_bytes": ctypes.c_size_t,
              "nerfhip_marching_cubes_workspace_bytes": ctypes.c_size_t, "nerfhip_mesh_cluster_workspace_bytes": ctypes.c_size_t,
              "nerfhip_jpeg_planes_bytes": ctypes.c_size_t, "nerfhip_ssim_workspace_bytes": ctypes.c_size_t,
diff --git a/nerf_pl_amd/csrc/mlp_bwd.hip b/nerf_pl_amd/csrc/mlp_bwd.hip
--- a/nerf_pl_amd/csrc/mlp_bwd.hip
+++ b/nerf_pl_amd/csrc/mlp_bwd.hip
@@ -28,19 +28,31 @@
     const int nwg = nerfhip_mlp_dw_splits(n_points, dtype);
     return nwg > 0 ? dw_workspace_bytes(nwg, 1) : 0;
 }
-extern "C" size_t nerfhip_mlp_dw_workspace_bytes_multi(const int64_t* n_points_host, int n_models, int dtype) {
-    if (!n_points_host || n_models < 1 || n_models > nerfhip::kDwMaxModels || !valid_dtype(dtype)) return 0;
+static_assert(kPlanDy1InDw == NERFHIP_BWD_DY1_IN_DW, "mlp_dw_plan.h flag codes");
+static inline bool valid_flags(int flags, int dtype) {
+    return (flags & ~NERFHIP_BWD_DY1_IN_DW) == 0 && (flags == 0 || dtype == NERFHIP_BF16);
+}
+extern "C" size_t nerfhip_mlp_dw_workspace_bytes_multi_flags(const int64_t* n_points_host, int n_models, int dtype, int flags) {
+    if (!n_points_host || n_models < 1 || n_models > nerfhip::kDwMaxModels || !valid_dtype(dtype) || !valid_flags(flags, dtype)) return 0;
     for (int m = 0; m < n_models; ++m)
         if (n_points_host[m] <= 0) return 0;
-    return dw_workspace_bytes(dw_plan(n_points_host, n_models, dtype, nullptr), n_models);
+    return dw_workspace_bytes(dw_plan(n_points_host, n_models, dtype, nullptr, flags), n_models);
+}
+extern "C" size_t nerfhip_mlp_dw_workspace_bytes_multi(const int64_t* n_points_host, int n_models, int dtype) {
+    return nerfhip_mlp_dw_workspace_bytes_multi_flags(n_points_host, n_models, dtype, 0);
 }
 
 extern "C" int nerfhip_mlp_dw_plan(const int64_t* n_points_host, int n_models, int dtype, int* splits_out, int* stage_kib_out) {
+    return nerfhip_mlp_dw_plan_flags(n_points_host, n_models, dtype, 0, splits_out, stage_kib_out);
+}
+extern "C" int nerfhip_mlp_dw_plan_flags(const int64_t* n_points_host, int n_models, int dtype, int flags, int* splits_out,
+                                         int* stage_kib_out) {
     if (!n_points_host || !splits_out || n_models < 1 || n_models > nerfhip::kDwMaxModels || !valid_dtype(dtype)) return NERFHIP_E_BADARG;
+    if (!valid_flags(flags, dtype)) return NERFHIP_E_UNSUPPORTED;
     for (int m = 0; m < n_models; ++m)
         if (n_points_host[m] <= 0) return NERFHIP_E_BADARG;
     nerfhip::DwJobTable jt;
-    const int total = dw_plan(n_points_host, n_models, dtype, &jt);
+    const int total = dw_plan(n_points_host, n_models, dtype, &jt, flags);
     for (int j = 0; j < n_models * nerfhip::mlp::kNumDwJobs; ++j) {
         splits_out[j] = jt.nsplit[j];
         if (stage_kib_out) {
@@ -48,6 +60,7 @@
             if (jt.fold_of[j] >= 0 || jt.nsplit[j] == 0) slabs = 0;
             for (int k = 0; k < n_models * nerfhip::mlp::kNumDwJobs; ++k)
                 if (jt.fold_of[k] == j) slabs += jt.job[k].dy_slabs;
+            if ((flags & NERFHIP_BWD_DY1_IN_DW) && j % nerfhip::mlp::kNumDwJobs == 0) slabs = nerfhip::kDwDy1FetchSlabs;
             stage_kib_out[j] = dtype == NERFHIP_F32 ? 2 * slabs : slabs;
         }
     }
@@ -59,8 +72,8 @@
                                      void* const* dys_host, void* dw_workspace, float* const* grad_w_host,
                                      float* const* grad_b_host, int accumulate, int dtype, int phases, const float* g_scale,
                                      const nerfhip_adam_fused* adam, nerfhip_stream_t stream) {
-    return nerfhip_mlp_bwd_multi_rays(n_models, g_out_host, out_host, n_host, packed_bwd_host, acts_host, dys_host, dw_workspace, grad_w_host,
-                                      grad_b_host, accumulate, dtype, phases, g_scale, adam, nullptr, stream);
+    return nerfhip_mlp_bwd_multi_flags(n_models, g_out_host, out_host, n_host, packed_bwd_host, acts_host, dys_host, dw_workspace, grad_w_host,
+                                       grad_b_host, accumulate, dtype, phases, g_scale, adam, nullptr, 0, stream);
 }
 
 extern "C" int nerfhip_mlp_bwd_multi_rays(int n_models, const float* const* g_out_host, const float* const* out_host,
@@ -68,8 +81,20 @@
                                           void* const* dys_host, void* dw_workspace, float* const* grad_w_host,
                                           float* const* grad_b_host, int accumulate, int dtype, int phases, const float* g_scale,
                                           const nerfhip_adam_fused* adam, const nerfhip_enc_source* enc, nerfhip_stream_t stream) {
+    return nerfhip_mlp_bwd_multi_flags(n_models, g_out_host, out_host, n_host, packed_bwd_host, acts_host, dys_host, dw_workspace, grad_w_host,
+                                       grad_b_host, accumulate, dtype, phases, g_scale, adam, enc, 0, stream);
+}
+
+extern "C" int nerfhip_mlp_bwd_multi_flags(int n_models, const float* const* g_out_host, const float* const* out_host,
+                                           const int64_t* n_host, const void* const* packed_bwd_host, const void* const* acts_host,
+                                           void* const* dys_host, void* dw_workspace, float* const* grad_w_host,
+                                           float* const* grad_b_host, int accumulate, int dtype, int phases, const float* g_scale,
+                                           const nerfhip_adam_fused* adam, const nerfhip_enc_source* enc, int flags,
+                                           nerfhip_stream_t stream) {
     NERFHIP_CHECK_ARG(n_models >= 1 && n_models <= nerfhip::kDwMaxModels);
-    if (!valid_dtype(dtype)) return NERFHIP_E_UNSUPPORTED;
+    if (!valid_dtype(dtype) || !valid_flags(flags, dtype)) return NERFHIP_E_UNSUPPORTED;
+    const bool dy1_in_dw = (flags & NERFHIP_BWD_DY1_IN_DW) != 0;
+    if (dy1_in_dw && enc) return NERFHIP_E_UNSUPPORTED;
     bool regen[nerfhip::kDwMaxModels] = {false, false};
     if (enc) {
         if (dtype != NERFHIP_BF16) return NERFHIP_E_UNSUPPORTED;
@@ -92,8 +117,9 @@
              ((uintptr_t)dys_host[m])) & 15)
             return NERFHIP_E_ALIGN;
     }
-    const int nwg = dw_plan(n_host, n_models, dtype, &jt);
+    const int nwg = dw_plan(n_host, n_models, dtype, &jt, flags);
     for (int m = 0; m < nerfhip::kDwMaxModels; ++m) {
+        jt.dy1_wt[m] = (dy1_in_dw && m < n_models) ? (const uint8_t*)packed_bwd_host[m] : nullptr;
         const bool on = m < n_models && regen[m];
         jt.enc_rays[m] = on ? enc->rays[m] : nullptr;
         jt.enc_z[m] = on ? enc->z[m] : nullptr;
@@ -134,7 +160,7 @@
     if (do_chain) {
         int64_t tiles[nerfhip::kDwMaxModels];
         for (int m = 0; m < n_models; ++m) tiles[m] = act_tiles(n_host[m], dtype);
-        nerfhip::launch_bwd_chain(n_models, g_out_host, g_scale, out_host, n_host, packed_bwd_host, acts_host, dys_host, dtype, tiles, s);
+        nerfhip::launch_bwd_chain(n_models, g_out_host, g_scale, out_host, n_host, packed_bwd_host, acts_host, dys_host, dtype, tiles, dy1_in_dw, s);
     }
     if (do_dw) {
         if (dtype == NERFHIP_BF16_F8) nerfhip::launch_dw_f8(jt, (float*)dw_workspace, nwg, s);
diff --git a/nerf_pl_amd/csrc/mlp_bwd_chain.h b/nerf_pl_amd/csrc/mlp_bwd_chain.h
--- a/nerf_pl_amd/csrc/mlp_bwd_chain.h
+++ b/nerf_pl_amd/csrc/mlp_bwd_chain.h
@@ -11,8 +11,9 @@
     const uint8_t* acts[2];
     uint8_t* dys[2];
     int blocks0;
+    int stop_at_dy2;
 };
 void launch_bwd_chain(int n_models, const float* const* g_out, const float* g_scale, const float* const* out, const int64_t* n,
                       const void* const* packed_bwd, const void* const* acts, void* const* dys, int dtype, const int64_t* tiles,
-                      hipStream_t s);
+                      bool stop_at_dy2, hipStream_t s);
 }
diff --git a/nerf_pl_amd/csrc/mlp_bwd_chain.hip b/nerf_pl_amd/csrc/mlp_bwd_chain.hip
--- a/nerf_pl_amd/csrc/mlp_bwd_chain.hip
+++ b/nerf_pl_amd/csrc/mlp_bwd_chain.hip
@@ -178,9 +178,10 @@
     return 127;
 }
 
-template <int PREC, bool F8>
+template <int PREC, bool F8, bool STOP2 = false>
 __global__ __launch_bounds__(PrecTraits<PREC>::NW * 64, PrecTraits<PREC>::WPS)
 void mlp_bwd_chain_kernel(BwdChainArgs A, const float* __restrict__ g_scale) {
+    static_assert(!STOP2 || (PREC == NERFHIP_BF16 && !F8), "the dW launch forms dY_1 from bf16 slabs only");
     const int mdl = ((int)blockIdx.x >= A.blocks0) ? 1 : 0;
     const unsigned wg = blockIdx.x - (mdl ? (unsigned)A.blocks0 : 0u);
     const float* __restrict__ g_out = mdl ? A.g_out[1] : A.g_out[0];
@@ -300,7 +301,11 @@
         st.pending_prev = 0;
         st.gsrc = gsrc0;
     }
-    NH_BWD(8, gb, ga, 0)
+    if constexpr (STOP2) {
+        asm volatile("s_waitcnt vmcnt(0)" ::: "memory");
+    } else {
+        NH_BWD(8, gb, ga, 0)
+    }
 #undef NH_BWD
     if constexpr (F8 && PREC == NERFHIP_BF16) {
 #pragma unroll
@@ -321,9 +326,10 @@
 namespace nerfhip {
 void launch_bwd_chain(int n_models, const float* const* g_out, const float* g_scale, const float* const* out, const int64_t* n,
                       const void* const* packed_bwd, const void* const* acts, void* const* dys, int dtype, const int64_t* tiles,
-                      hipStream_t s) {
+                      bool stop_at_dy2, hipStream_t s) {
     const int wpw = (dtype == NERFHIP_F32) ? 4 : 8;
     BwdChainArgs A;
+    A.stop_at_dy2 = (stop_at_dy2 && dtype == NERFHIP_BF16) ? 1 : 0;
     unsigned blocks = 0;
     for (int m = 0; m < 2; ++m) {
         const int mm = m < n_models ? m : 0;
@@ -334,6 +340,8 @@
     }
     if (dtype == NERFHIP_BF16_F8)
         hipLaunchKernelGGL((mlp_bwd_chain_kernel<NERFHIP_BF16, true>), dim3(blocks), dim3(512), 0, s, A, g_scale);
+    else if (dtype == NERFHIP_BF16 && A.stop_at_dy2)
+        hipLaunchKernelGGL((mlp_bwd_chain_kernel<NERFHIP_BF16, false, true>), dim3(blocks), dim3(512), 0, s, A, g_scale);
     else if (dtype == NERFHIP_BF16)
         hipLaunchKernelGGL((mlp_bwd_chain_kernel<NERFHIP_BF16, false>), dim3(blocks), dim3(512), 0, s, A, g_scale);
     else
diff --git a/nerf_pl_amd/csrc/mlp_bwd_dw.h b/nerf_pl_amd/csrc/mlp_bwd_dw.h
--- a/nerf_pl_amd/csrc/mlp_bwd_dw.h
+++ b/nerf_pl_amd/csrc/mlp_bwd_dw.h
@@ -26,7 +26,9 @@
     const float* enc_rays[kDwMaxModels];
     const float* enc_z[kDwMaxModels];
     int enc_tpr[kDwMaxModels];
+    const uint8_t* dy1_wt[kDwMaxModels];
 };
+constexpr int kDwDy1FetchSlabs = 21;
 static_assert(kDwJobs[kDwJobDir].x2_off == kDwJobs[kDwJobSigma].x1_off && kDwJobs[kDwJobDir].x2_slabs == 16 && kDwJobs[kDwJobDir].x1_slabs == 2 &&
               kDwJobs[kDwJobSigma].x1_slabs == 16 && kDwJobs[kDwJobSigma].dy_slabs == 2 && kDwJobs[kDwJobDir].dy_slabs == 8 &&
               kDwJobs[kDwJobSigma].x2_slabs == 0, "the sigma head and the dir layer read the same h8 section");
diff --git a/nerf_pl_amd/csrc/mlp_bwd_dw.hip b/nerf_pl_amd/csrc/mlp_bwd_dw.hip
--- a/nerf_pl_amd/csrc/mlp_bwd_dw.hip
+++ b/nerf_pl_amd/csrc/mlp_bwd_dw.hip
@@ -401,6 +401,140 @@
             if (wave == kDwFoldRow0) sl[8 * kDwMaxXTiles * 64 * 16 + kDwFoldRow0 * 64 + lane] = dbacc;
         }
     };
+    [[maybe_unused]] auto run_dy1 = [&](const uint8_t* __restrict__ wt) {
+        constexpr int D = 4, LPW = 3, STAGE = (16 + kDwDy1FetchSlabs) * kPieceBytes;
+        constexpr int O_ENC = 16, O_DY2 = 20, O_GATE = 36;
+        static_assert((PREC != NERFHIP_BF16 || D * STAGE <= RING_BYTES) && kDwDy1FetchSlabs == 16 + kXyzSlabs + 1 && 8 * LPW >= kDwDy1FetchSlabs, "class DY1 ring");
+        static_assert(kBwdLayers[kNumBwdLayers - 1].param == 1 && kBwdLayers[kNumBwdLayers - 1].nt == 8 && kBwdLayers[kNumBwdLayers - 1].nks == 16,
+                      "the chain's last layer is L2^T");
+        u32x4 wf[16];
+        {
+            const uint8_t* wsrc = wt + ((size_t)(bwd_layer_start(kNumBwdLayers - 1, NERFHIP_BF16) + wave * 16)) * kPieceBytes + lane * 16;
+#pragma unroll
+            for (int ks = 0; ks < 16; ++ks) wf[ks] = *reinterpret_cast<const u32x4*>(wsrc + (size_t)ks * kPieceBytes);
+#pragma unroll
+            for (int ks = 0; ks < 16; ++ks) asm volatile("" : "+v"(wf[ks]));
+        }
+        auto stage_tile = [&](int64_t it) {
+            int64_t T = t_first + (it < my_tiles ? it : my_tiles - 1);
+            if (T >= ntiles) T = ntiles - 1;
+            if (T < 0) T = 0;
+            return T;
+        };
+        const uint8_t* a0p = nullptr;
+        const uint8_t* a1p = nullptr;
+        const uint8_t* d1p = nullptr;
+        unsigned slot0 = 0, slot1 = 0;
+        int s_iss = D - 1, s_use = 0;
+        auto advance = [&](int64_t g) {
+            a0p = a1p;
+            slot0 = slot1;
+            const int64_t T = stage_tile(g + 1);
+            a1p = acts_base + tile_block_off(T, act_tile_bytes(PREC), IL);
+            d1p = dys_base + tile_block_off(T, kDySlabs * 64 * 16, IL);
+            s_iss = (s_iss + 1 == D) ? 0 : s_iss + 1;
+            slot1 = lds_base + (unsigned)(s_iss * STAGE);
+        };
+        auto issue_piece = [&](int i, bool opening) {
+            if (i < 2) {
+                const int sl = wave + 8 * i;
+                const unsigned dst = (unsigned)__builtin_amdgcn_readfirstlane((int)(slot1 + (unsigned)((O_DY2 + sl) * kPieceBytes)));
+                glds16_nt(d1p + (size_t)(dy_h(2) + sl) * kPieceBytes * IL + lane * 16, dst);
+            } else if (!opening && wave < kXyzSlabs) {
+                const unsigned dst = (unsigned)__builtin_amdgcn_readfirstlane((int)(slot0 + (unsigned)((O_ENC + wave) * kPieceBytes)));
+                glds16_nt(a0p + (size_t)(kActEncX + wave) * kPieceBytes * IL + ((wave & 1) ? dma_off_odd : dma_off_even), dst);
+            } else {
+                const unsigned dst = (unsigned)__builtin_amdgcn_readfirstlane((int)(slot1 + (unsigned)(O_GATE * kPieceBytes)));
+                const uint8_t* g = a1p + (size_t)(act_mask_off(PREC) + mask_piece_h(1) * kPieceBytes) * IL + lane * 16;
+                if (wave == kXyzSlabs) glds16_nt(g, dst);
+                else glds16_nt_masked(g, dst, 1ull);
+            }
+        };
+        constexpr int FR = 6;
+        auto dy2_frag = [&](const char* sb, int ks) { return *reinterpret_cast<const bf16x8*>(sb + (O_DY2 + ks) * kPieceBytes + lane * 16); };
+        auto form_ahead = [&](const char* sb, bf16x8 (&fb)[FR]) {
+#pragma unroll
+            for (int ks = 0; ks < FR; ++ks) fb[ks] = dy2_frag(sb, ks);
+        };
+        auto form = [&](char* sb, bf16x8 (&fb)[FR]) {
+            f32x16 c;
+#pragma unroll
+            for (int r = 0; r < 16; ++r) c[r] = 0.0f;
+            __builtin_amdgcn_sched_barrier(0);
+#pragma unroll
+            for (int ks = 0; ks < 16; ++ks) {
+                c = __builtin_amdgcn_mfma_f32_32x32x16_bf16(__builtin_bit_cast(bf16x8, wf[ks]), fb[ks % FR], c, 0, 0, 0);
+                if (ks + FR < 16) fb[ks % FR] = dy2_frag(sb, ks + FR);
+                __builtin_amdgcn_sched_barrier(0);
+            }
+            const u32x4 gates = *reinterpret_cast<const u32x4*>(sb + O_GATE * kPieceBytes + lane * 16);
+            const int gw = wave >> 1;
+            const unsigned gword = gw == 0 ? gates[0] : (gw == 1 ? gates[1] : (gw == 2 ? gates[2] : gates[3]));
+            const short sh0 = (short)(8 * (wave & 1));
+            bf16x8 o[2];
+#pragma unroll
+            for (int p = 0; p < 8; ++p) {
+                typedef __attribute__((ext_vector_type(2))) float f32x2v;
+                const f32x2v xv = {c[2 * p], c[2 * p + 1]};
+                const bf16x2 pk = __builtin_convertvector(xv, bf16x2);
+                s16x2 gm = __builtin_bit_cast(s16x2, gword);
+                gm = (gm << (short)(sh0 + p)) >> (short)15;
+                const unsigned d = __builtin_bit_cast(unsigned, pk) & __builtin_bit_cast(unsigned, gm);
+                const bf16x2 gated = __builtin_bit_cast(bf16x2, d);
+                o[p >> 2][2 * (p & 3)] = gated[0];
+                o[p >> 2][2 * (p & 3) + 1] = gated[1];
+            }
+            const int unit = 2 * (lane & 31) + (lane >> 5);
+            *reinterpret_cast<bf16x8*>(sb + (2 * wave) * SLAB_BYTES + unit * 16) = o[0];
+            *reinterpret_cast<bf16x8*>(sb + (2 * wave + 1) * SLAB_BYTES + (unit ^ 8) * 16) = o[1];
+        };
+        advance(-1);
+#pragma unroll
+        for (int i = 0; i < LPW; ++i) issue_piece(i, true);
+#pragma unroll
+        for (int g = 0; g < D - 1; ++g) {
+            advance(g);
+#pragma unroll
+            for (int i = 0; i < LPW; ++i) issue_piece(i, false);
+        }
+        wait_vm_barrier<(D - 1) * LPW>();
+        bf16x8 fb[FR];
+        form_ahead(ring, fb);
+        form(ring, fb);
+        for (int64_t it = 0; it < my_tiles; ++it) {
+            wait_vm_barrier<(D - 2) * LPW>();
+            advance(it + D - 1);
+            char* st_base = ring + s_use * STAGE;
+            s_use = (s_use + 1 == D) ? 0 : s_use + 1;
+            const char* dy_base = st_base + (2 * wave) * SLAB_BYTES;
+            const char* x_base = st_base + O_ENC * SLAB_BYTES;
+            const bf16x8 a0 = load_frag(dy_base, 0);
+            bf16x8 b[4];
+#pragma unroll
+            for (int m = 0; m < 4; ++m) b[m] = load_frag(x_base + 2 * (m % 2) * SLAB_BYTES, m / 2);
+            const bf16x8 a1 = load_frag(dy_base, 1);
+            form_ahead(ring + s_use * STAGE, fb);
+            __builtin_amdgcn_sched_barrier(0);
+#pragma unroll
+            for (int m = 0; m < 4; ++m) {
+                acc[m % 2] = __builtin_amdgcn_mfma_f32_32x32x16_bf16(m < 2 ? a0 : a1, b[m], acc[m % 2], 0, 0, 0);
+                __builtin_amdgcn_sched_barrier(0);
+                if (m == 1) dw_bias_sum(a0, dbacc, dbacc2);
+                if (m == 3) dw_bias_sum(a1, dbacc, dbacc2);
+                if (m < LPW) {
+                    issue_piece(m, false);
+                    __builtin_amdgcn_sched_barrier(0);
+                }
+            }
+            form(ring + s_use * STAGE, fb);
+        }
+        asm volatile("s_waitcnt vmcnt(0)" ::: "memory");
+        float* sl = slabs + (size_t)blockIdx.x * kDwSlabFloats;
+        dbacc += dbacc2;
+#pragma unroll
+        for (int x = 0; x < 2; ++x) dw_store_block(sl + (size_t)(wave * kDwMaxXTiles + x) * 1024, acc[x], lane);
+        sl[8 * kDwMaxXTiles * 64 * 16 + wave * 64 + lane] = dbacc;
+    };
     using std::integral_constant;
     using std::false_type;
     using std::true_type;
@@ -410,6 +544,7 @@
         case 2:
             if constexpr (PREC == NERFHIP_BF16) {
                 if (regen) { run(integral_constant<int, 2>{}, integral_constant<int, 20>{}, true_type{}); break; }
+                if (const uint8_t* wt = jobs.dy1_wt[jid / kNumDwJobs]) { run_dy1(wt); break; }
             }
             run(integral_constant<int, 2>{}, integral_constant<int, 20>{}, false_type{});
             break;
diff --git a/nerf_pl_amd/csrc/mlp_dw_plan.h b/nerf_pl_amd/csrc/mlp_dw_plan.h
--- a/nerf_pl_amd/csrc/mlp_dw_plan.h
+++ b/nerf_pl_amd/csrc/mlp_dw_plan.h
@@ -11,9 +11,14 @@
 }
 
 constexpr int kDwCostA = 150, kDwCostB = 45;
+#ifndef NERFHIP_DW_COST_DY1
+#define NERFHIP_DW_COST_DY1 500
+#endif
+constexpr int kDwCostDy1 = NERFHIP_DW_COST_DY1;
+constexpr int kPlanDy1InDw = 1;
 constexpr int kDwMinIters = 48;
 static int dw_target_wgs(int dtype) { return dtype == kPlanBf16F8 ? kDwWgsF8 : dtype == kPlanBf16 ? kDwWgsBf16 : kDwWgsF32; }
-static int dw_plan(const int64_t* n_points, int n_models, int dtype, nerfhip::DwJobTable* jt) {
+static int dw_plan(const int64_t* n_points, int n_models, int dtype, nerfhip::DwJobTable* jt, int flags = 0) {
     using namespace nerfhip;
     using namespace nerfhip::mlp;
     const int njobs = n_models * kNumDwJobs;
@@ -28,6 +33,7 @@
         const int ca = dtype == kPlanBf16 ? kDwCostA : 1;
         const int cb = dtype == kPlanBf16 ? kDwCostB : 0;
         cost[j] = ca + (int64_t)cb * (jb.dy_slabs + jb.x1_slabs + jb.x2_slabs + (j % kNumDwJobs == kDwJobDir ? 2 : 0));
+        if (dtype == kPlanBf16 && (flags & kPlanDy1InDw) && j % kNumDwJobs == 0) cost[j] = ca + (int64_t)cb * kDwDy1FetchSlabs + kDwCostDy1;
         units[j] = tiles / (dtype == kPlanBf16F8 ? 2 : 1);
         cap[j] = units[j] / kDwMinIters;
         if (cap[j] < 1) cap[j] = 1;
diff --git a/nerf_pl_amd/models/train_step.py b/nerf_pl_amd/models/train_step.py
--- a/nerf_pl_amd/models/train_step.py
+++ b/nerf_pl_amd/models/train_step.py
@@ -48,6 +48,19 @@
     return prev
 
 
+_dy1_in_dw = os.environ.get("NERFHIP_DY1_IN_DW", "1") != "0"
+
+
+def dy1_in_dw_enabled():
+    return _dy1_in_dw
+
+
+def set_dy1_in_dw(on):
+    global _dy1_in_dw
+    prev, _dy1_in_dw = _dy1_in_dw, bool(on)
+    return prev
+
+
 class _TrainRender(torch.autograd.Function):
     @staticmethod
     def forward(ctx, cfg, rays, rgbs, *params):
@@ -85,6 +98,7 @@
                                                     white_back, u, gscale, packs, acts_c, dev)
         ctx.models = [models[1], models[0]] if N > 0 else [models[0]]
         ctx.entries, ctx.dtype, ctx.adam = entries, dtype, adam
+        ctx.dy1_in_dw = dy1_in_dw_enabled() and ops.mlp_dtype_code(dtype) == ops.BF16 and all(len(e) == 4 for e in entries)
         ctx.n_params = [len(m.flat_params()) for m in models]
         ctx.serials = [m.pack_serial() for m in ctx.models]
         ctx.mark_non_differentiable(out3, *outs)
@@ -109,8 +123,9 @@
             adam = ctx.adam.handle(models) if ctx.adam is not None else None
         groups = [[k] for k in range(n_models)] if hooked and joint_hook is None else [list(range(n_models))]
         grads = []
+        mode = {"dy1_in_dw": True} if getattr(ctx, "dy1_in_dw", False) else {}
         for group in groups:
-            got = ops.mlp_bwd_multi([entries[k] for k in group], dtype, adam=adam, g_scale=g_scale)
+            got = ops.mlp_bwd_multi([entries[k] for k in group], dtype, adam=adam, g_scale=g_scale, **mode)
             grads_ready([models[k] for k in group], [g[2] for g in got])
             grads += got
         if adam is not None:
diff --git a/nerf_pl_amd/ops.py b/nerf_pl_amd/ops.py
--- a/nerf_pl_amd/ops.py
+++ b/nerf_pl_amd/ops.py
@@ -640,13 +640,16 @@
     return bufs
 
 
-def mlp_bwd_multi(entries, dtype, adam=None, phases=7, workspace=None, g_scale=None):
+def mlp_bwd_multi(entries, dtype, adam=None, phases=7, workspace=None, g_scale=None, dy1_in_dw=False, accumulate_into=None):
     code = mlp_dtype_code(dtype)
     lib = _lib.load()
     M = len(entries)
     dev = entries[0][1].device
     gs, outs, ns, dys, grads = [], [], [], [], []
     enc, keep_enc = None, []
+    flags = _lib.BWD_DY1_IN_DW if dy1_in_dw else 0
+    if accumulate_into is not None and adam is not None:
+        raise ValueError("mlp_bwd_multi: the fused Adam update cannot follow an accumulating backward")
     for m, e in enumerate(entries):
         g_out, out = e[0], e[1]
         if len(e) > 4 and e[4] is not None:
@@ -666,17 +669,20 @@
         ns.append(out.shape[0])
     with torch.cuda.device(dev):
         n_arr = (ctypes.c_int64 * M)(*ns)
-        key = ("multi", tuple(ns), code)
+        key = ("multi", tuple(ns), code, flags)
         if workspace is not None and key in workspace:
             dys, ws = workspace[key]
         else:
             dys = [torch.empty(int(lib.nerfhip_mlp_dy_bytes(n, code)), device=dev, dtype=torch.uint8) for n in ns]
-            ws = torch.empty(int(lib.nerfhip_mlp_dw_workspace_bytes_multi(n_arr, M, code)), device=dev, dtype=torch.uint8)
+            ws = torch.empty(int(lib.nerfhip_mlp_dw_workspace_bytes_multi_flags(n_arr, M, code, flags)), device=dev, dtype=torch.uint8)
             if workspace is not None:
                 workspace[key] = (dys, ws)
-        joint = torch.empty(M * FLAT_GRAD_FLOATS, device=dev, dtype=torch.float32)
-        for m, n in enumerate(ns):
-            grads.append(flat_grad_views(n, dev, out=joint[m * FLAT_GRAD_FLOATS:(m + 1) * FLAT_GRAD_FLOATS]))
+        if accumulate_into is not None:
+            grads = list(accumulate_into)
+        else:
+            joint = torch.empty(M * FLAT_GRAD_FLOATS, device=dev, dtype=torch.float32)
+            for m, n in enumerate(ns):
+                grads.append(flat_grad_views(n, dev, out=joint[m * FLAT_GRAD_FLOATS:(m + 1) * FLAT_GRAD_FLOATS]))
         vp = ctypes.c_void_p
         G = (vp * M)(*[t.data_ptr() for t in gs])
         O = (vp * M)(*[t.data_ptr() for t in outs])
@@ -690,9 +696,10 @@
                 adam.grad_flat[m] = grads[m][2].data_ptr()
         if g_scale is not None:
             require_gpu(g_scale)
-        check(lib.nerfhip_mlp_bwd_multi_rays(M, G, O, n_arr, PB, AC, DY, ptr(ws), GW, GB, 0, code, int(phases), ptr(g_scale),
-                                             ctypes.addressof(adam) if adam is not None else None,
-                                             ctypes.addressof(enc) if enc is not None else None, stream_ptr()), "nerfhip_mlp_bwd_multi_rays")
+        check(lib.nerfhip_mlp_bwd_multi_flags(M, G, O, n_arr, PB, AC, DY, ptr(ws), GW, GB, int(accumulate_into is not None), code, int(phases),
+                                              ptr(g_scale), ctypes.addressof(adam) if adam is not None else None,
+                                              ctypes.addressof(enc) if enc is not None else None, flags, stream_ptr()),
+              "nerfhip_mlp_bwd_multi_flags")
     return grads
 
 
```

After: 962,600. 0.89x the previous value.
